# kkahatapitiya/Coarse-Fine-Networks

Hardware: AMD Instinct MI355X
Metric: clips/sec (fwd+bwd+SGD) x3d_fine X3D-M T=256x224x224 (higher is better)
Workload: dtype f32; 1 GPU; x3d_fine X3D-M train step (fwd+loss+bwd+SGD), 8x3x256x224x224 clips per GPU, random-init weights; clips_per_gpu=8, frames=256, parallelism=dp1, launch=eager

## Files before the change

coarse-fine-networks_amd/cfn_hip/ops.py:

```python
import torch
from torch.autograd import Function
from torch.autograd.function import once_differentiable

import ctypes
import threading

from . import call, call_try, check, query, ACT_NONE, ACT_RELU, ACT_SWISH, ACT_SIGMOID


_scratch_epoch = [0]


class _ZeroArena(object):
    CHUNK = 1 << 20

    def __init__(self):
        self.buf, self.off, self.epoch = {}, {}, _scratch_epoch[0]

    def take(self, numel, dev):
        if self.epoch != _scratch_epoch[0]:
            self.buf, self.off, self.epoch = {}, {}, _scratch_epoch[0]
        numel_al = (numel + 1) & ~1
        key = (dev.type, dev.index)
        if key not in self.buf or self.off[key] + numel_al > self.buf[key].numel():
            self.buf[key] = torch.zeros(max(self.CHUNK, numel_al), dtype=torch.float64, device=dev)
            self.off[key] = 0
        o = self.off[key]
        self.off[key] = o + numel_al
        return self.buf[key][o:o + numel]


class _GradCast(object):

    def __init__(self):
        self._reset()
        self.last_total = 0

    def _reset(self):
        self.cur, self.live, self.scheduled, self.seen, self.task = {}, [], False, set(), None

    def begin(self):
        tid = torch._C._current_graph_task_id()
        if tid != self.task:
            if self.live:
                self.flush()
            self._reset()
            self.task = tid

    def first_use(self, w):
        if id(w) in self.seen:
            return False
        self.seen.add(id(w))
        return True

    def take(self, numel, shape, dev):
        al = (numel + 3) & ~3
        key = (dev.type, dev.index)
        ch = self.cur.get(key)
        if ch is None or ch['off'] + al > ch['f64'].numel():
            size = max(int(self.last_total * 1.05) + 1024, al, 1 << 16)
            ch = {'f64': torch.zeros(size, dtype=torch.float64, device=dev),
                  'f32': torch.empty(size, dtype=torch.float32, device=dev), 'off': 0, 'done': 0}
            self.cur[key] = ch
            self.live.append(ch)
        o = ch['off']
        ch['off'] = o + al
        if not self.scheduled:
            torch.autograd.Variable._execution_engine.queue_callback(self._end_of_backward)
            self.scheduled = True
        return ch['f64'][o:o + numel], ch['f32'][o:o + numel].view(shape)

    def flush(self):
        for ch in self.live:
            if ch['off'] > ch['done']:
                ch['f32'][ch['done']:ch['off']].copy_(ch['f64'][ch['done']:ch['off']])
                ch['done'] = ch['off']

    def _end_of_backward(self):
        self.flush()
        self.last_total = max(sum(ch['off'] for ch in self.live), 1)
        self._reset()


class _PerThread(threading.local):

    def __init__(self):
        self.arena = _ZeroArena()
        self.gradcast = _GradCast()


_tls = _PerThread()
LAZY_GRAD_CAST = True


def _f64(n, c, dev):
    return _tls.arena.take(n * c, dev).view(n, c)


def _f64pair(n, c, dev):
    t = _tls.arena.take(2 * n * c, dev).view(2, n, c)
    return t, t[0], t[1]


def reset_scratch():
    _scratch_epoch[0] += 1


def flush_grad_casts():
    _tls.gradcast.flush()


def allow_lazy_grad_cast(params, ok=True):
    for p in params:
        p._cfn_lazy_grad_ok = bool(ok)


def _lazy_ok(w):
    if not LAZY_GRAD_CAST or w is None or not w.is_leaf or w.grad is not None or torch.is_grad_enabled():
        return False
    if not getattr(w, '_cfn_lazy_grad_ok', False):
        return False
    if w._backward_hooks:
        return False
    hooks = getattr(w, '_post_accumulate_grad_hooks', None)
    if hooks:
        from .dist import _BucketHook
        if not all(isinstance(h, _BucketHook) for h in hooks.values()):
            return False
    return True


def _lazy_ok_probe(w):
    with torch.no_grad():
        return _lazy_ok(w)


def _grad_owner(w):
    if w is not None and not w.is_leaf and w._is_view():
        base = w._base
        if base is not None and base.is_leaf and base.numel() == w.numel() and w.is_contiguous() and base.is_contiguous():
            return base
    return w


def _gw_buffers(w, rows, cols, dev):
    gc = _tls.gradcast
    owner = _grad_owner(w)
    if _lazy_ok(owner):
        gc.begin()
        if gc.first_use(owner):
            g64, g32 = gc.take(rows * cols, tuple(w.shape), dev)
            return g64.view(rows, cols), (lambda: g32)
        gc.flush()
    g64 = _f64(rows, cols, dev)
    return g64, (lambda: g64.float().view(tuple(w.shape)))


def _opt(t):
    return None if t is None else t.contiguous()


def _coef(t, rows=None, cols=None):
    if t is None:
        return None
    if rows is not None and t.numel() != rows * cols:
        raise RuntimeError('per-sample coefficients of %d x %d channels expected, got a tensor of shape %s' % (rows, cols, tuple(t.shape)))
    return t.to(torch.float64).contiguous()


class ShortcutToken(object):

    def __init__(self):
        self.acc, self.acc_stride, self.main_done = None, 1, False


class TailLink(object):

    def __init__(self):
        self.y_scale = self.res_scale = None
        self.done = False


def _bf(t):
    return t is not None and t.dtype in (torch.bfloat16, torch.float16)


def subsample_hw(x, s):
    N, C, T, H, W = x.shape
    out = torch.empty(N, C, T, (H - 1) // s + 1, (W - 1) // s + 1, dtype=x.dtype, device=x.device)
    call('cfn_subsample_hw' + _sfx(x), x, out, N * C * T, H, W, s)
    return out


class _PwConv(Function):

    @staticmethod
    def forward(ctx, x, A, B, w, act, stride, want_stats, token, role, tail=None, tail_role=None):
        x = check(x).contiguous()
        N, Cin, T, H, W = x.shape
        Cout = w.shape[0]
        Ho, Wo = (H - 1) // stride + 1, (W - 1) // stride + 1
        y = torch.empty(N, Cout, T, Ho, Wo, dtype=x.dtype, device=x.device)
        s = q = None
        if want_stats:
            s, q = _f64(N, Cout, x.device), _f64(N, Cout, x.device)
        w2 = w.reshape(Cout, Cin).contiguous()
        A, B = _coef(A, N, Cin), _coef(B, N, Cin)
        xs = None
        if _bf(x):
            xs = subsample_hw(x, stride) if stride > 1 else x
            call('cfn_pwconv_fwd' + _sfx(x), xs, A, B, act, w2, y, s, q, N, Cin, Cout, T * Ho * Wo)
        else:
            call('cfn_pwconv_fwd', x, A, B, act, w2, y, s, q, N, Cin, Cout, T, H, W, stride)
        ctx.save_for_backward(x, A, B, w2, y, xs if stride > 1 else None)
        ctx.meta = (act, stride, tuple(w.shape))
        ctx.wparam = w
        ctx.token, ctx.role = token, role
        ctx.tail, ctx.tail_role = tail, tail_role
        if not want_stats:
            return y, None, None
        return y, s, q

    @staticmethod
    @once_differentiable
    def backward(ctx, gy, gs, gq):
        x, A, B, w2, y, xs = ctx.saved_tensors
        act, stride, wshape = ctx.meta
        token, role = ctx.token, ctx.role
        N, Cin, T, H, W = x.shape
        Cout = w2.shape[0]
        gy = torch.zeros_like(y) if gy is None else gy.contiguous()
        gs, gq = _opt(gs), _opt(gq)
        gsc = None
        if ctx.tail is not None and ctx.tail.done:
            gsc = ctx.tail.y_scale if ctx.tail_role == 'y' else ctx.tail.res_scale
        if _bf(x):
            return _PwConv._backward_bf16(ctx, gy, gs, gq, gsc)
        gx = gA = gB = gw = None
        g64 = fin = None
        fused = False
        if ctx.needs_input_grad[0] or (A is not None and ctx.needs_input_grad[1]):
            if token is not None and role == 'short' and stride > 1 and not token.main_done:
                Ho, Wo = y.shape[3], y.shape[4]
                da = torch.empty(N, Cin, T, Ho, Wo, dtype=torch.float32, device=x.device)
                if ctx.needs_input_grad[3]:
                    g64, fin = _gw_buffers(ctx.wparam, Cout, Cin, x.device)
                    fused = call_try('cfn_pwconv_short_bwd', gy, y, gs, gq, gsc, w2, x, A, B, act, da, g64, N, Cin, Cout, T, H, W,
                                     stride)
                if not fused:
                    call('cfn_pwconv_bwd_data_acc', gy, y, gs, gq, w2, None, None, None, ACT_NONE, da, None, None, N, Cin, Cout, T,
                         Ho, Wo, 1, None, 1, gsc)
                token.acc, token.acc_stride = da, stride
            else:
                gx = torch.zeros_like(x) if stride != 1 else torch.empty_like(x)
                ab = a64 = b64 = None
                if A is not None:
                    ab, a64, b64 = _f64pair(N, Cin, x.device)
                acc, acc_stride = None, 1
                if token is not None and role == 'main':
                    if token.acc is not None:
                        acc, acc_stride, token.acc = token.acc, token.acc_stride, None
                    else:
                        token.main_done = True
                if stride == 1 and ctx.needs_input_grad[3]:
                    g64, fin = _gw_buffers(ctx.wparam, Cout, Cin, x.device)
                    fused = call_try('cfn_pwconv_bwd_fused', gy, y, gs, gq, w2, x, A, B, act, gx, a64, b64, g64, N, Cin, Cout,
                                     T, H, W, acc, acc_stride, gsc)
                if not fused:
                    call('cfn_pwconv_bwd_data_acc', gy, y, gs, gq, w2, x, A, B, act, gx, a64, b64, N, Cin, Cout, T, H, W, stride,
                         acc, acc_stride, gsc)
                if A is not None:
                    gA, gB = ab[0], ab[1]
        if ctx.needs_input_grad[3]:
            if g64 is None:
                g64, fin = _gw_buffers(ctx.wparam, Cout, Cin, x.device)
            if not fused:
                call('cfn_pwconv_bwd_weight', gy, y, gs, gq, x, A, B, act, g64, N, Cin, Cout, T, H, W, stride, gsc)
            gw = fin()
        return gx, gA, gB, gw, None, None, None, None, None, None, None

    @staticmethod
    def _backward_bf16(ctx, gy, gs, gq, gsc):
        x, A, B, w2, y, xs = ctx.saved_tensors
        act, stride, wshape = ctx.meta
        token, role = ctx.token, ctx.role
        N, Cin, T, H, W = x.shape
        Cout = w2.shape[0]
        Ho, Wo = y.shape[3], y.shape[4]
        xin = xs if stride > 1 else x
        gx = gA = gB = gw = None
        if ctx.needs_input_grad[0] or (A is not None and ctx.needs_input_grad[1]):
            if token is not None and role == 'short' and stride > 1 and not token.main_done:
                da = torch.empty(N, Cin, T, Ho, Wo, dtype=x.dtype, device=x.device)
                call('cfn_pwconv_bwd_data' + _sfx(gy), gy, y, gs, gq, w2, None, None, None, ACT_NONE, da, None, None, N, Cin, Cout, T,
                     Ho, Wo, None, 1, gsc)
                token.acc, token.acc_stride = da, stride
            else:
                ab = a64 = b64 = None
                if A is not None:
                    ab, a64, b64 = _f64pair(N, Cin, x.device)
                acc, acc_stride = None, 1
                if token is not None and role == 'main':
                    if token.acc is not None:
                        acc, acc_stride, token.acc = token.acc, token.acc_stride, None
                    else:
                        token.main_done = True
                gxc = torch.empty_like(xin)
                call('cfn_pwconv_bwd_data' + _sfx(gy), gy, y, gs, gq, w2, xin, A, B, act, gxc, a64, b64, N, Cin, Cout, T, Ho, Wo,
                     acc, acc_stride, gsc)
                if stride > 1:
                    gx = torch.zeros_like(x)
                    gx[:, :, :, ::stride, ::stride] = gxc
                else:
                    gx = gxc
                if A is not None:
                    gA, gB = ab[0], ab[1]
        if ctx.needs_input_grad[3]:
            g64, fin = _gw_buffers(ctx.wparam, Cout, Cin, x.device)
            call('cfn_pwconv_bwd_weight' + _sfx(gy), gy, y, gs, gq, xin, A, B, act, g64, N, Cin, Cout, T * Ho * Wo, gsc)
            gw = fin()
        return gx, gA, gB, gw, None, None, None, None, None, None, None


def pwconv(x, w, A=None, B=None, act=ACT_NONE, stride=1, stats=True, token=None, role=None, tail=None, tail_role=None):
    N, Cin, T, H, W = x.shape
    Ho, Wo = (H - 1) // stride + 1, (W - 1) // stride + 1
    es = x.element_size()
    lim = (1 << 31) if es == 4 else (1 << 30)
    span = max(Cin * H * W, w.shape[0] * H * W, w.shape[0] * Ho * Wo, Cin * Ho * Wo) * es
    needs_grad = torch.is_grad_enabled() and any(t is not None and t.requires_grad for t in (x, w, A, B))
    if span * T < lim or needs_grad or T == 1:
        return _PwConv.apply(x, A, B, w, act, stride, stats, token, role, tail, tail_role)
    step = max((lim - 1) // span, 1)
    odd_plane = es == 2 and (Ho * Wo) % 2 == 1
    if odd_plane:
        if 2 * span >= lim:
            raise RuntimeError('pwconv: two frames of %d x %d x %d bf16 elements exceed the 1 GiB buffer range the frame-range '
                               'chunking has to respect (odd plane: frames travel in pairs)' % (max(Cin, w.shape[0]), H, W))
        step = max(step & ~1, 2)
    y = torch.empty(N, w.shape[0], T, Ho, Wo, dtype=x.dtype, device=x.device)
    s = q = None
    t0 = 0
    while t0 < T:
        t1 = min(t0 + step, T)
        if odd_plane and (t1 - t0) % 2 and t1 - t0 > 1:
            t1 -= 1
        pad = odd_plane and (t1 - t0) % 2 == 1
        xc = x[:, :, t0:t1].contiguous()
        if pad:
            xc = torch.cat([xc, torch.zeros_like(xc)], 2)
        yc, sc, qc = _PwConv.apply(xc, A, B, w, act, stride, False if pad else stats, None, None)
        if pad:
            yc = yc[:, :, :1]
            if stats:
                sc, qc = yc.double().sum((2, 3, 4)), (yc.double() ** 2).sum((2, 3, 4))
        y[:, :, t0:t1] = yc
        if stats:
            s, q = (sc, qc) if s is None else (s + sc, q + qc)
        t0 = t1
    return y, s, q


def _sfx(t):
    return '_bf16' if t.dtype == torch.bfloat16 else ('_f16' if t.dtype == torch.float16 else '')


class _DwConv3d(Function):

    @staticmethod
    def forward(ctx, x, A, B, w, act, stride, want_stats):
        x = check(x).contiguous()
        N, C, T, H, W = x.shape
        Ho, Wo = (H + 2 - 3) // stride + 1, (W + 2 - 3) // stride + 1
        y = torch.empty(N, C, T, Ho, Wo, dtype=x.dtype, device=x.device)
        s = q = None
        if want_stats:
            s, q = _f64(N, C, x.device), _f64(N, C, x.device)
        w2 = w.reshape(C, 27).contiguous()
        A, B = _coef(A, N, C), _coef(B, N, C)
        call('cfn_dwconv3d_fwd' + _sfx(x), x, A, B, act, w2, y, s, q, N, C, T, H, W, stride)
        ctx.save_for_backward(x, A, B, w2, y)
        ctx.meta = (act, stride, tuple(w.shape))
        ctx.wparam = w
        if not want_stats:
            return y, None, None
        return y, s, q

    @staticmethod
    @once_differentiable
    def backward(ctx, gy, gs, gq):
        x, A, B, w2, y = ctx.saved_tensors
        act, stride, wshape = ctx.meta
        N, C, T, H, W = x.shape
        gy = torch.zeros_like(y) if gy is None else gy.contiguous()
        gs, gq = _opt(gs), _opt(gq)
        gx = gA = gB = gw = None
        want_x = ctx.needs_input_grad[0] or (A is not None and ctx.needs_input_grad[1])
        want_w = ctx.needs_input_grad[3]
        ab = a64 = b64 = g64 = fin = None
        if want_x:
            gx = torch.empty_like(x)
            if A is not None:
                ab, a64, b64 = _f64pair(N, C, x.device)
        if want_w:
            g64, fin = _gw_buffers(ctx.wparam, C, 27, x.device)
        sfx = _sfx(x)
        fused = want_x and want_w and stride == 1 and call_try('cfn_dwconv3d_bwd_fused' + sfx, gy, y, gs, gq, w2, x, A, B, act,
                                                             gx, a64, b64, g64, N, C, T, H, W)
        if not fused and want_x and want_w and stride == 2:
            fused = call_try('cfn_dwconv3d_bwd_fused_s2' + sfx, gy, y, gs, gq, w2, x, A, B, act, gx, a64, b64, g64, N, C, T, H, W)
        if not fused:
            if want_x:
                call('cfn_dwconv3d_bwd_data' + sfx, gy, y, gs, gq, w2, x, A, B, act, gx, a64, b64, N, C, T, H, W, stride)
            if want_w:
                call('cfn_dwconv3d_bwd_weight' + sfx, gy, y, gs, gq, x, A, B, act, g64, N, C, T, H, W, stride)
        if want_x and A is not None:
            gA, gB = ab[0], ab[1]
        if want_w:
            gw = fin()
        return gx, gA, gB, gw, None, None, None


def dwconv3d(x, w, A=None, B=None, act=ACT_NONE, stride=1, stats=True):
    return _DwConv3d.apply(x, A, B, w, act, stride, stats)


class _DwConvT5(Function):

    @staticmethod
    def forward(ctx, x, w, want_stats, out_dtype=None):
        x = check(x, torch.float32).contiguous()
        N, C, T, H, W = x.shape
        y = torch.empty_like(x, dtype=out_dtype or x.dtype)
        s = q = None
        if want_stats:
            s, q = _f64(N, C, x.device), _f64(N, C, x.device)
        w2 = w.reshape(C, 5).contiguous()
        call('cfn_dwconv_t5_fwd' + _sfx(y), x, w2, y, s, q, N, C, T, H * W)
        ctx.save_for_backward(x, w2, y)
        ctx.wshape = tuple(w.shape)
        ctx.wparam = w
        if not want_stats:
            return y, None, None
        return y, s, q

    @staticmethod
    @once_differentiable
    def backward(ctx, gy, gs, gq):
        x, w2, y = ctx.saved_tensors
        N, C, T, H, W = x.shape
        gy = torch.zeros_like(y) if gy is None else gy.contiguous()
        gs, gq = _opt(gs), _opt(gq)
        gx = gw = None
        want_x, want_w = ctx.needs_input_grad[0], ctx.needs_input_grad[1]
        if want_x:
            gx = torch.empty_like(x)
        if want_w:
            g64, fin = _gw_buffers(ctx.wparam, C, 5, x.device)
        fused = want_x and want_w and call_try('cfn_dwconv_t5_bwd_fused' + _sfx(y), gy, y, gs, gq, w2, x, gx, g64, N, C, T, H * W)
        if not fused:
            if want_x:
                call('cfn_dwconv_t5_bwd_data' + _sfx(y), gy, y, gs, gq, w2, gx, N, C, T, H * W)
            if want_w:
                call('cfn_dwconv_t5_bwd_weight' + _sfx(y), gy, y, gs, gq, x, g64, N, C, T, H * W)
        if want_w:
            gw = fin()
        return gx, gw, None, None


def dwconv_t5(x, w, stats=True, out_dtype=None):
    return _DwConvT5.apply(x, w, stats, out_dtype)


class _StemConv(Function):

    @staticmethod
    def forward(ctx, x, w):
        x = check(x).contiguous()
        N, Ci, T, H, W = x.shape
        Co = w.shape[0]
        Ho, Wo = (H + 2 - 3) // 2 + 1, (W + 2 - 3) // 2 + 1
        y = torch.empty(N, Co, T, Ho, Wo, dtype=torch.float32, device=x.device)
        w2 = w.reshape(Co, Ci * 9).contiguous()
        call('cfn_stem_conv_fwd', x, w2, y, N, Ci, Co, T, H, W)
        ctx.save_for_backward(x)
        ctx.wshape = tuple(w.shape)
        ctx.wparam = w
        return y

    @staticmethod
    @once_differentiable
    def backward(ctx, gy):
        (x,) = ctx.saved_tensors
        N, Ci, T, H, W = x.shape
        Co = ctx.wshape[0]
        gw = None
        if ctx.needs_input_grad[1]:
            g64, fin = _gw_buffers(ctx.wparam, Co, Ci * 9, x.device)
            call('cfn_stem_conv_bwd_weight', gy.contiguous(), x, g64, N, Ci, Co, T, H, W)
            gw = fin()
        return None, gw


def stem_conv(x, w):
    return _StemConv.apply(x, w)


from .u8clips import clip_lut


def _u8_args(frames, lengths, lut):
    if frames.dtype != torch.uint8 or frames.dim() != 5 or frames.shape[4] != 3:
        raise RuntimeError('uint8 frames of shape (N, T, H, W, 3) expected, got %s %s' % (frames.dtype, tuple(frames.shape)))
    if lut.dtype != torch.float32 or lut.numel() != 3 * 256:
        raise RuntimeError('a (3, 256) fp32 table expected (ops.clip_lut), got %s %s' % (lut.dtype, tuple(lut.shape)))
    if lengths is not None:
        if lengths.numel() != frames.shape[0]:
            raise RuntimeError('one length per clip expected: %d clips, lengths %s' % (frames.shape[0], tuple(lengths.shape)))
        lengths = lengths.to(torch.int32).contiguous()
    return frames.contiguous(), lengths, lut.contiguous()


def clip_u8_to_f32(frames, lut, lengths=None):
    frames, lengths, lut = _u8_args(frames, lengths, lut)
    N, T, H, W, _ = frames.shape
    x = torch.empty(N, 3, T, H, W, dtype=torch.float32, device=frames.device)
    call('cfn_clip_u8_to_f32', frames, lut, lengths, x, N, T, H, W)
    return x


class _StemConvU8(Function):

    @staticmethod
    def forward(ctx, frames, lengths, lut, w):
        frames, lengths, lut = _u8_args(frames, lengths, lut)
        N, T, H, W, Ci = frames.shape
        Co = w.shape[0]
        Ho, Wo = (H + 2 - 3) // 2 + 1, (W + 2 - 3) // 2 + 1
        y = torch.empty(N, Co, T, Ho, Wo, dtype=torch.float32, device=frames.device)
        w2 = w.reshape(Co, Ci * 9).contiguous()
        if not call_try('cfn_stem_conv_u8_fwd', frames, lut, lengths, w2, y, N, Ci, Co, T, H, W):
            call('cfn_stem_conv_fwd', clip_u8_to_f32(frames, lut, lengths), w2, y, N, Ci, Co, T, H, W)
        ctx.save_for_backward(frames, lengths, lut)
        ctx.wshape = tuple(w.shape)
        ctx.wparam = w
        return y

    @staticmethod
    @once_differentiable
    def backward(ctx, gy):
        frames, lengths, lut = ctx.saved_tensors
        N, T, H, W, Ci = frames.shape
        Co = ctx.wshape[0]
        gw = None
        if ctx.needs_input_grad[3]:
            g64, fin = _gw_buffers(ctx.wparam, Co, Ci * 9, frames.device)
            gy = gy.contiguous()
            if not call_try('cfn_stem_conv_u8_bwd_weight', gy, frames, lut, lengths, g64, N, Ci, Co, T, H, W):
                call('cfn_stem_conv_bwd_weight', gy, clip_u8_to_f32(frames, lut, lengths), g64, N, Ci, Co, T, H, W)
            gw = fin()
        return None, None, None, gw


def stem_conv_u8(frames, lengths, lut, w):
    return _StemConvU8.apply(frames, lengths, lut, w)


from . import u8aug

_AUG_TABLES = {}
_AUG_TABLES_MAX = 256


def aug_tables(box, size, device):
    cs = tuple(int(v) for v in box.detach().reshape(-1, 4)[:, 2].cpu().tolist())
    device = torch.device(device)
    key = (cs, int(size), device.type, device.index)
    hit = _AUG_TABLES.get(key)
    if hit is None:
        if any(c <= 0 or c > 4 * int(size) for c in cs):
            raise RuntimeError('crop_resize_flip_u8: crop extents %s into %d: 1 <= c <= 4 * size expected (the kernel takes tables of up '
                               'to %d taps; there is no CPU fallback)' % (sorted(set(cs)), size, u8aug.MAX_TAPS))
        bounds, coef = u8aug.batch_tables(cs, size)
        hit = (bounds.to(device), coef.to(device))
        if len(_AUG_TABLES) >= _AUG_TABLES_MAX:
            _AUG_TABLES.clear()
        _AUG_TABLES[key] = hit
    return hit


def crop_resize_flip_u8(frames, lengths, box, size, out=None, tables=None):
    if frames.dtype != torch.uint8 or frames.dim() != 5 or frames.shape[4] != 3:
        raise RuntimeError('uint8 frames of shape (N, T, Hs, Ws, 3) expected, got %s %s' % (frames.dtype, tuple(frames.shape)))
    N, T, Hs, Ws, _ = frames.shape
    S = int(size)
    if box.numel() != 4 * N:
        raise RuntimeError('one box (x1, y1, c, flip) per clip expected: %d clips, box %s' % (N, tuple(box.shape)))
    if lengths is not None:
        if lengths.numel() != N:
            raise RuntimeError('one length per clip expected: %d clips, lengths %s' % (N, tuple(lengths.shape)))
        lengths = lengths.to(torch.int32).contiguous()
    bounds, coef = tables if tables is not None else aug_tables(box, S, frames.device)
    if tuple(bounds.shape) != (N, S, 2) or coef.dim() != 3 or tuple(coef.shape[:2]) != (N, S):
        raise RuntimeError('tables of %d clips into %d expected, got bounds %s coef %s' % (N, S, tuple(bounds.shape), tuple(coef.shape)))
    box = box.reshape(N, 4).to(device=frames.device, dtype=torch.int32).contiguous()
    if out is None:
        out = torch.empty(N, T, S, S, 3, dtype=torch.uint8, device=frames.device)
    elif out.dtype != torch.uint8 or tuple(out.shape) != (N, T, S, S, 3) or not out.is_contiguous():
        raise RuntimeError('out: a contiguous uint8 tensor of shape %s expected, got %s %s' % ((N, T, S, S, 3), out.dtype, tuple(out.shape)))
    if not call_try('cfn_crop_resize_flip_u8', frames.contiguous(), lengths, box, bounds.contiguous(), coef.contiguous(), out, N, T, Hs, Ws,
                    S, int(coef.shape[2])):
        raise RuntimeError('crop_resize_flip_u8: %d taps into size %d is beyond what the kernel was built for (c <= 4 * size, size <= 312 '
                           'at 9 taps); there is no CPU fallback' % (int(coef.shape[2]), S))
    return out


AP_SORT_TILE = 8192
AP_FLAG_NONBINARY, AP_FLAG_OVERFLOW = 1, 2


def _ap_stores(scores, targets, count, what):
    for name, x in (('scores', scores), ('targets', targets), ('count', count)):
        if not torch.is_tensor(x) or not x.is_cuda:
            raise RuntimeError('%s: %s must be a device tensor; there is no CPU path' % (what, name))
    if scores.dtype != torch.float32 or scores.dim() != 2 or targets.dtype != torch.uint8 or tuple(targets.shape) != tuple(scores.shape):
        raise RuntimeError('%s: class-major stores expected, scores (K, cap) fp32 and targets (K, cap) uint8; got %s %s, %s %s'
                           % (what, scores.dtype, tuple(scores.shape), targets.dtype, tuple(targets.shape)))
    if count.dtype != torch.int32 or count.numel() != 1:
        raise RuntimeError('%s: count must be one int32 on the device, got %s %s' % (what, count.dtype, tuple(count.shape)))
    if scores.shape[0] < 1 or scores.shape[1] < 1:
        raise RuntimeError('%s: empty stores %s' % (what, tuple(scores.shape)))
    return int(scores.shape[0]), int(scores.shape[1])


def ap_append(probs, labels, valid, scores, targets, count, flags):
    K, cap = _ap_stores(scores, targets, count, 'ap_append')
    for name, x in (('probs', probs), ('labels', labels), ('flags', flags)):
        if not torch.is_tensor(x) or not x.is_cuda:
            raise RuntimeError('ap_append: %s must be a device tensor; there is no CPU path' % name)
    if probs.dim() != 3 or probs.shape[1] != K or tuple(labels.shape) != tuple(probs.shape):
        raise RuntimeError('ap_append: probs and labels (B, %d, TL) expected, got %s and %s' % (K, tuple(probs.shape), tuple(labels.shape)))
    if flags.dtype != torch.int32 or flags.numel() != 1:
        raise RuntimeError('ap_append: flags must be one int32 on the device')
    B, _, TL = probs.shape
    if valid is not None:
        if valid.numel() != B:
            raise RuntimeError('ap_append: one valid length per video expected: %d videos, valid %s' % (B, tuple(valid.shape)))
        valid = valid.to(torch.int32).contiguous()
    call('cfn_ap_append', probs.float().contiguous(), labels.float().contiguous(), valid, scores, targets, count, flags, B, K, TL, cap)


def ap_sort(scores, targets, count, out=None):
    K, cap = _ap_stores(scores, targets, count, 'ap_sort')
    if out is None:
        out = (torch.empty_like(scores), torch.empty_like(targets), torch.empty(K, cap, dtype=torch.int32, device=scores.device),
               torch.empty_like(targets))
    ss, st, tk, tt = out
    for x, ref, dt in ((ss, scores, torch.float32), (st, targets, torch.uint8), (tk, scores, torch.int32), (tt, targets, torch.uint8)):
        if tuple(x.shape) != tuple(ref.shape) or x.dtype != dt or x.device != ref.device:
            raise RuntimeError('ap_sort: out buffers of shape %s (fp32, uint8, int32, uint8) on %s expected' % (tuple(ref.shape), ref.device))
    call('cfn_ap_sort', scores, targets, count, ss, st, tk, tt, K, cap)
    return ss, st


def ap_reduce(sorted_targets, count):
    if not sorted_targets.is_cuda or not count.is_cuda:
        raise RuntimeError('ap_reduce: device tensors only; there is no CPU path')
    if sorted_targets.dtype != torch.uint8 or sorted_targets.dim() != 2 or count.dtype != torch.int32 or count.numel() != 1:
        raise RuntimeError('ap_reduce: sorted targets (K, cap) uint8 and one int32 count expected')
    K, cap = sorted_targets.shape
    ap = torch.empty(K, dtype=torch.float32, device=sorted_targets.device)
    call('cfn_ap_reduce', sorted_targets, count, ap, K, cap)
    return ap


def average_precision(scores, targets, count, out=None):
    _, st = ap_sort(scores, targets, count, out=out)
    return ap_reduce(st, count)


class _BnFold(Function):

    @staticmethod
    def forward(ctx, s, q, gamma, beta, w1, b1, w2, b2, bufs, cfg):
        training, N, C, S, count, eps, momentum, pool_count = cfg
        run_mean, run_var, nbt = bufs
        dev = run_mean.device
        Wd = w1.shape[0] if w1 is not None else 0
        Se = S if training else 1
        A = torch.empty(N, C, dtype=torch.float64, device=dev)
        B = torch.empty_like(A)
        mean = torch.empty(Se, C, dtype=torch.float64, device=dev)
        rstd = torch.empty_like(mean)
        A0 = B0 = gate = hbuf = pooled = None
        w1c = w2c = None
        if Wd:
            A0, B0, gate, pooled = (torch.empty(N, C, dtype=torch.float32, device=dev) for _ in range(4))
            hbuf = torch.empty(N, Wd, dtype=torch.float32, device=dev)
            w1c, w2c = w1.reshape(Wd, C).contiguous(), w2.reshape(C, Wd).contiguous()
        s, q = _opt(s), _opt(q)
        call('cfn_bn_fold_fwd', s, q, gamma, beta, run_mean, run_var, nbt if training else None, int(training), N, C, S,
             float(count), float(eps), float(momentum), w1c, b1, w2c, b2, Wd, float(pool_count), A, B, mean, rstd,
             A0, B0, gate, hbuf, pooled)
        ctx.save_for_backward(s, gamma, mean, rstd, A0, B0, gate, hbuf, pooled, w1c, w2c)
        ctx.cfg = (training, N, C, S, Wd, count, pool_count, None if w1 is None else tuple(w1.shape),
                   None if w2 is None else tuple(w2.shape))
        return A, B

    @staticmethod
    @once_differentiable
    def backward(ctx, gA, gB):
        s, gamma, mean, rstd, A0, B0, gate, hbuf, pooled, w1c, w2c = ctx.saved_tensors
        training, N, C, S, Wd, count, pool_count, w1s, w2s = ctx.cfg
        dev = mean.device
        gA = torch.zeros(N, C, dtype=torch.float64, device=dev) if gA is None else gA.contiguous()
        gB = torch.zeros(N, C, dtype=torch.float64, device=dev) if gB is None else gB.contiguous()
        gs = gq = None
        if training:
            gs = torch.empty(N, C, dtype=torch.float64, device=dev)
            gq = torch.empty_like(gs)
        elif Wd:
            gs = torch.empty(N, C, dtype=torch.float64, device=dev)
        gg = gbt = None
        if gamma is not None:
            gg, gbt = torch.empty(C, device=dev), torch.empty(C, device=dev)
        gw1 = gb1 = gw2 = gb2 = tA = tB = None
        if Wd:
            gw1, gb1 = torch.empty(Wd, C, device=dev), torch.empty(Wd, device=dev)
            gw2, gb2 = torch.empty(C, Wd, device=dev), torch.empty(C, device=dev)
            tA, tB = (torch.empty(N, C, dtype=torch.float64, device=dev) for _ in range(2))
        call('cfn_bn_fold_bwd', gA, gB, s, gamma, mean, rstd, A0, B0, gate, hbuf, pooled, w1c, w2c, int(training), N, C, S,
             Wd, float(count), float(pool_count), gs, gq, gg, gbt, gw1, gb1, gw2, gb2, tA, tB)
        if Wd:
            gw1, gw2 = gw1.view(w1s), gw2.view(w2s)
        return gs, gq, gg, gbt, gw1, gb1, gw2, gb2, None, None


def bn_fold(s, q, gamma, beta, bufs, training, N, C, S, count, eps, momentum, se=None, pool_count=1.0):
    w1, b1, w2, b2 = se if se is not None else (None, None, None, None)
    return _BnFold.apply(s, q, gamma, beta, w1, b1, w2, b2, bufs, (training, N, C, S, count, eps, momentum, pool_count))


class _BnAddRelu(Function):

    @staticmethod
    def forward(ctx, y, A, B, res, Ar, Br, split, link):
        y, res = check(y).contiguous(), check(res).contiguous()
        N, C = y.shape[:2]
        vol = y[0, 0].numel()
        if tuple(res.shape) != tuple(y.shape):
            raise RuntimeError('bn_add_relu: residual %s does not match y %s' % (tuple(res.shape), tuple(y.shape)))
        out = torch.empty_like(y)
        A, B, Ar, Br = _coef(A, N, C), _coef(B, N, C), _coef(Ar, N, C), _coef(Br, N, C)
        mask = None
        sfx = _sfx(y)
        if link is not None:
            words = query('cfn_bn_add_relu_mask_words' + sfx, N * C, vol)
            if words > 0:
                mask = torch.empty(words, dtype=torch.int32, device=y.device)
        call('cfn_bn_add_relu_fwd' + sfx, y, A, B, res, Ar, Br, out, mask, N * C, vol)
        ctx.link, ctx.has_mask = link, mask is not None
        ctx.save_for_backward(y, A, res, Ar, mask if mask is not None else out)
        if not split:
            return out
        alias = torch.empty(0, dtype=out.dtype, device=out.device).set_(out.untyped_storage(), out.storage_offset(),
                                                                         out.shape, out.stride())
        return out, alias

    @staticmethod
    @once_differentiable
    def backward(ctx, gout, gout2=None):
        y, A, res, Ar, out = ctx.saved_tensors
        N, C = y.shape[:2]
        vol = y[0, 0].numel()
        if gout is None:
            gout, gout2 = gout2, None
        if gout is None:
            gout = torch.zeros_like(y)
        gout2 = None if gout2 is None else gout2.contiguous()
        t3 = _tls.arena.take(3 * N * C, y.device).view(3, N, C)
        gA, gB = t3[0], t3[1]
        gAr = t3[2] if Ar is not None else None
        gBr = gB if Ar is not None else None
        link = ctx.link
        if link is not None:
            g = torch.empty_like(y)
            mask = out if ctx.has_mask else None
            call('cfn_bn_add_relu_bwd_g' + _sfx(y), gout.contiguous(), gout2, None if ctx.has_mask else out, mask, y,
                 res if Ar is not None else None, g, gA, gB, gAr, N * C, vol)
            link.y_scale, link.res_scale, link.done = A.detach(), (None if Ar is None else Ar.detach()), True
            g2 = torch.empty(0, dtype=g.dtype, device=g.device).set_(g.untyped_storage(), g.storage_offset(), g.shape, g.stride())
            return g, gA, gB, g2, gAr, gBr, None, None
        if _bf(y):
            g = torch.empty_like(y)
            call('cfn_bn_add_relu_bwd_g' + _sfx(y), gout.contiguous(), gout2, out, None, y, res if Ar is not None else None, g, gA, gB,
                 gAr, N * C, vol)
            shp = (N, C) + (1,) * (y.dim() - 2)
            gres = g if Ar is None else (g.float() * Ar.float().view(shp)).to(y.dtype)
            return (g.float() * A.float().view(shp)).to(y.dtype), gA, gB, gres, gAr, gBr, None, None
        gy, gres = torch.empty_like(y), torch.empty_like(res)
        call('cfn_bn_add_relu_bwd', gout.contiguous(), gout2, out, y, A, res, Ar, gy, gres, gA, gB, gAr, N * C, vol)
        return gy, gA, gB, gres, gAr, gBr, None, None


def bn_add_relu(y, A, B, res, Ar=None, Br=None, split=False, link=None):
    return _BnAddRelu.apply(y, A, B, res, Ar, Br, split, link)


class _AffineAct(Function):
    @staticmethod
    def forward(ctx, x, A, B, act):
        x = check(x).contiguous()
        N, C = x.shape[:2]
        out = torch.empty_like(x)
        A, B = _coef(A, N, C), _coef(B, N, C)
        call('cfn_affine_act_fwd', x, A, B, act, out, N * C, x[0, 0].numel())
        ctx.save_for_backward(x, A, B)
        ctx.act = act
        return out

    @staticmethod
    @once_differentiable
    def backward(ctx, gout):
        x, A, B = ctx.saved_tensors
        N, C = x.shape[:2]
        gx = torch.empty_like(x)
        a64, b64 = _f64(N, C, x.device), _f64(N, C, x.device)
        call('cfn_affine_act_bwd', gout.contiguous(), x, A, B, ctx.act, gx, a64, b64, N * C, x[0, 0].numel())
        return gx, a64, b64, None


def affine_act(x, A, B, act=ACT_NONE):
    return _AffineAct.apply(x, A, B, act)


class _ChannelStats(Function):

    @staticmethod
    def forward(ctx, x):
        x = check(x).contiguous()
        N, C = x.shape[:2]
        s, q = _f64(N, C, x.device), _f64(N, C, x.device)
        call('cfn_channel_stats', x, s, q, N * C, x[0, 0].numel())
        ctx.save_for_backward(x)
        return s, q

    @staticmethod
    @once_differentiable
    def backward(ctx, gs, gq):
        (x,) = ctx.saved_tensors
        N, C = x.shape[:2]
        gx = torch.zeros_like(x)
        shp = (N, C) + (1,) * (x.dim() - 2)
        if gs is not None:
            gx = gx + gs.float().view(shp)
        if gq is not None:
            gx = gx + 2.0 * gq.float().view(shp) * x
        return gx


def channel_stats(x):
    return _ChannelStats.apply(x)


class _PoolHW(Function):

    @staticmethod
    def forward(ctx, x, A, B, act, OH, OW):
        x = check(x).contiguous()
        N, C, T, H, W = x.shape
        out = torch.empty(N, C, T, OH, OW, dtype=torch.float32, device=x.device)
        A, B = _coef(A, N, C), _coef(B, N, C)
        call('cfn_pool_hw_fwd' + _sfx(x), x, A, B, act, out, N * C, T, H, W, OH, OW)
        ctx.save_for_backward(x, A, B)
        ctx.meta = (act, OH, OW)
        return out

    @staticmethod
    @once_differentiable
    def backward(ctx, gout):
        x, A, B = ctx.saved_tensors
        act, OH, OW = ctx.meta
        N, C, T, H, W = x.shape
        gx = torch.empty_like(x)
        a64 = b64 = None
        if A is not None:
            a64, b64 = _f64(N, C, x.device), _f64(N, C, x.device)
        call('cfn_pool_hw_bwd' + _sfx(x), gout.contiguous(), x, A, B, act, gx, a64, b64, N * C, T, H, W, OH, OW)
        if A is None:
            return gx, None, None, None, None, None
        return gx, a64, b64, None, None, None


def pool_hw(x, OH, OW, A=None, B=None, act=ACT_NONE):
    return _PoolHW.apply(x, A, B, act, OH, OW)


class _Film(Function):

    @staticmethod
    def forward(ctx, x, m, c, f):
        x, m, c = check(x).contiguous(), check(m).contiguous(), check(c).contiguous()
        N, C, T, H, W = x.shape
        want = (N, C, T, H // f if f > 0 else -1, W // f if f > 0 else -1)
        if f <= 0 or H % f or W % f or tuple(m.shape) != want or tuple(c.shape) != want:
            raise RuntimeError('film: coefficients %s / %s do not tile x %s with %d x %d blocks (expected %s)'
                               % (tuple(m.shape), tuple(c.shape), tuple(x.shape), f, f, want))
        out = torch.empty_like(x)
        call('cfn_film_fwd', x, m, c, out, N * C, T, H, W, f)
        ctx.save_for_backward(x, m)
        ctx.f = f
        return out

    @staticmethod
    @once_differentiable
    def backward(ctx, g):
        x, m = ctx.saved_tensors
        N, C, T, H, W = x.shape
        gx, gm, gc = torch.empty_like(x), torch.empty_like(m), torch.empty_like(m)
        call('cfn_film_bwd', g.contiguous(), x, m, gx, gm, gc, N * C, T, H, W, ctx.f)
        return gx, gm, gc, None


def film(x, m, c, f):
    return _Film.apply(x, m, c, f)


class _TimeSample(Function):

    @staticmethod
    def forward(ctx, x, cdf):
        x, cdf = check(x).contiguous(), check(cdf).contiguous()
        B, C, Tin = x.shape[:3]
        K = cdf.shape[1]
        P = x[0, 0, 0].numel()
        out = torch.empty((B, C, K) + tuple(x.shape[3:]), dtype=torch.float32, device=x.device)
        call('cfn_time_sample_fwd', x, cdf, out, B, C, Tin, K, P)
        ctx.save_for_backward(x, cdf)
        return out

    @staticmethod
    @once_differentiable
    def backward(ctx, g):
        x, cdf = ctx.saved_tensors
        B, C, Tin = x.shape[:3]
        K = cdf.shape[1]
        P = x[0, 0, 0].numel()
        gx = torch.empty_like(x) if ctx.needs_input_grad[0] else None
        g64 = torch.zeros(B, K, dtype=torch.float64, device=x.device) if ctx.needs_input_grad[1] else None
        call('cfn_time_sample_bwd', g.contiguous(), x, cdf, gx, g64, B, C, Tin, K, P)
        return gx, (g64.float() if g64 is not None else None)


def time_sample(x, cdf):
    return _TimeSample.apply(x, cdf)


class _TimePool(Function):

    @staticmethod
    def forward(ctx, x, mode, R):
        x = check(x, torch.float32).contiguous()
        B, C, T = x.shape[:3]
        P = x[0, 0, 0].numel()
        out = torch.empty((B, C, T // R) + tuple(x.shape[3:]), dtype=torch.float32, device=x.device)
        call('cfn_time_pool_fwd', x, out, mode, B * C, T, R, P)
        ctx.save_for_backward(x)
        ctx.meta = (mode, R)
        return out

    @staticmethod
    @once_differentiable
    def backward(ctx, g):
        (x,) = ctx.saved_tensors
        mode, R = ctx.meta
        B, C, T = x.shape[:3]
        gx = torch.empty_like(x)
        call('cfn_time_pool_bwd', g.contiguous(), x, gx, mode, B * C, T, R, x[0, 0, 0].numel())
        return gx, None, None


def time_pool(x, mode, R=4):
    return _TimePool.apply(x, {'avg': 0, 'max': 1}[mode], R)


def grid_time_index(cdf, Tin):
    cdf = check(cdf).contiguous()
    i0 = torch.empty(cdf.shape, dtype=torch.int32, device=cdf.device)
    w1 = torch.empty(cdf.shape, dtype=torch.float32, device=cdf.device)
    call('cfn_grid_time_index', cdf, cdf.numel(), Tin, i0, w1)
    return i0, w1


class _Interp1d(Function):
    @staticmethod
    def forward(ctx, x, y, xnew):
        x, y, xnew = check(x).contiguous(), check(y).contiguous(), check(xnew).contiguous()
        B = max(x.shape[0], y.shape[0], xnew.shape[0])
        N, Pq = x.shape[1], xnew.shape[1]
        rows = (int(x.shape[0] > 1), int(y.shape[0] > 1), int(xnew.shape[0] > 1))
        ynew = torch.empty(B, Pq, dtype=torch.float32, device=x.device)
        ind = torch.empty(B, Pq, dtype=torch.int64, device=x.device)
        call('cfn_interp1d_fwd', x, y, xnew, ynew, ind, B, N, Pq, *rows)
        ctx.save_for_backward(x, y, xnew, ind)
        ctx.rows = rows
        ctx.mark_non_differentiable(ind)
        return ynew, ind

    @staticmethod
    @once_differentiable
    def backward(ctx, g, _gind):
        x, y, xnew, ind = ctx.saved_tensors
        B, Pq = ind.shape
        N = x.shape[1]
        gx = torch.zeros_like(x) if ctx.needs_input_grad[0] else None
        gy = torch.zeros_like(y) if ctx.needs_input_grad[1] else None
        gq = torch.zeros_like(xnew) if ctx.needs_input_grad[2] else None
        call('cfn_interp1d_bwd', g.contiguous(), x, y, xnew, ind, gx, gy, gq, B, N, Pq, *ctx.rows)
        return gx, gy, gq


def interp1d(x, y, xnew):
    return _Interp1d.apply(x, y, xnew)


class _TimeResize(Function):

    @staticmethod
    def forward(ctx, x, L, align_corners):
        x = check(x).contiguous()
        BC = x.shape[0] * x.shape[1]
        Kin = x.shape[2]
        P = x[0, 0, 0].numel()
        out = torch.empty(tuple(x.shape[:2]) + (L,) + tuple(x.shape[3:]), dtype=torch.float32, device=x.device)
        call('cfn_time_resize_fwd', x, out, BC, Kin, L, P, int(bool(align_corners)))
        ctx.meta = (tuple(x.shape), L, int(bool(align_corners)))
        return out

    @staticmethod
    @once_differentiable
    def backward(ctx, g):
        shape, L, ac = ctx.meta
        gx = torch.empty(shape, dtype=torch.float32, device=g.device)
        P = 1
        for d in shape[3:]:
            P *= d
        call('cfn_time_resize_bwd', g.contiguous(), gx, shape[0] * shape[1], shape[2], L, P, ac)
        return gx, None, None


def time_resize(x, L, align_corners=True):
    return _TimeResize.apply(x, L, align_corners)


def _detloss_args(logits, labels, masks, crops):
    for name, v in (('logits', logits), ('labels', labels), ('masks', masks)):
        if not v.is_cuda or v.dtype != torch.float32:
            raise RuntimeError('detection_loss: %s must be a device fp32 tensor, got %s on %s (there is no CPU path)' % (name, v.dtype, v.device))
        if v.device != logits.device:
            raise RuntimeError('detection_loss: %s lives on %s, the logits on %s' % (name, v.device, logits.device))
    crops = int(crops)
    if logits.dim() != 3 or labels.dim() != 3 or masks.dim() != 2 or crops < 1:
        raise RuntimeError('detection_loss: logits (B*crops, C, T), labels (B, C, TL), masks (B, TL), crops >= 1')
    B, C, TL = labels.shape
    if logits.shape[0] != B * crops or logits.shape[1] != C or tuple(masks.shape) != (B, TL) or 0 in logits.shape or 0 in labels.shape:
        raise RuntimeError('detection_loss: logits %s, labels %s, masks %s do not belong together at %d crop(s)'
                           % (tuple(logits.shape), tuple(labels.shape), tuple(masks.shape), crops))
    return logits.contiguous(), labels.contiguous(), masks.contiguous(), B, C, logits.shape[2], TL


def detection_loss_fwd(logits, labels, masks, align_corners=True, crops=1, norm=None, world=1.0, want_probs=True):
    logits, labels, masks, B, C, T, TL = _detloss_args(logits, labels, masks, crops)
    dev = logits.device
    if norm is not None:
        if not norm.is_cuda or norm.device != dev or norm.numel() != 1:
            raise RuntimeError('detection_loss: norm must be a one-element tensor on the device of the logits')
        norm = norm.detach().to(torch.float32).reshape(1)
    cls = torch.empty((), dtype=torch.float32, device=dev)
    loc = torch.empty((), dtype=torch.float32, device=dev)
    probs = torch.empty(B, C, TL, dtype=torch.float32, device=dev) if want_probs else None
    jstar = torch.empty(B * C, dtype=torch.int32, device=dev)
    ymax = torch.empty(B * C, dtype=torch.float32, device=dev)
    rows = torch.empty(2 * B * C, dtype=torch.float64, device=dev)
    norm_used = torch.empty(1, dtype=torch.float64, device=dev)
    call('cfn_detloss_fwd', logits, labels, masks, norm, float(world), probs, cls, loc, jstar, ymax, rows, norm_used, B, C, T, TL, int(crops),
         int(bool(align_corners)))
    return cls, loc, probs, jstar, ymax, norm_used


def detection_loss_bwd(g_cls, g_loc, logits, labels, masks, jstar, ymax, norm_used, align_corners=True, crops=1, world=1.0):
    logits, labels, masks, B, C, T, TL = _detloss_args(logits, labels, masks, crops)
    if jstar.numel() != B * C or ymax.numel() != B * C or norm_used.numel() != 1:
        raise RuntimeError('detection_loss_bwd: jstar / ymax / norm_used are not the ones the forward returned for these shapes')
    g_cls, g_loc = (g.detach().to(torch.float32).reshape(1) for g in (g_cls, g_loc))
    gx = torch.empty_like(logits)
    call('cfn_detloss_bwd', g_cls, g_loc, logits, labels, masks, jstar.contiguous(), ymax.contiguous(), norm_used, float(world), gx, B, C, T, TL,
         int(crops), int(bool(align_corners)))
    return gx


class _DetectionLoss(Function):

    @staticmethod
    def forward(ctx, logits, labels, masks, align_corners, crops, norm, world, want_probs):
        cls, loc, probs, jstar, ymax, norm_used = detection_loss_fwd(logits, labels, masks, align_corners, crops, norm, world, want_probs)
        ctx.save_for_backward(logits, labels, masks, jstar, ymax, norm_used)
        ctx.meta = (bool(align_corners), int(crops), float(world))
        if probs is not None:
            ctx.mark_non_differentiable(probs)
        return cls, loc, probs

    @staticmethod
    @once_differentiable
    def backward(ctx, g_cls, g_loc, _g_probs):
        gx = detection_loss_bwd(g_cls, g_loc, *ctx.saved_tensors, *ctx.meta) if ctx.needs_input_grad[0] else None
        return gx, None, None, None, None, None, None, None


def detection_loss(logits, labels, masks, align_corners, crops=1, norm=None, world=1.0, want_probs=True):
    return _DetectionLoss.apply(logits, labels, masks, align_corners, crops, norm, world, want_probs)


def _geom(kernel, stride, padding):
    return (ctypes.c_int * 9)(*(tuple(kernel) + tuple(stride) + tuple(padding)))


class _ConvDense(Function):

    @staticmethod
    def forward(ctx, x, A, B, w, act, kernel, stride, padding, want_stats):
        x = check(x).contiguous()
        N, Ci, T, H, W = x.shape
        Co = w.shape[0]
        g = _geom(kernel, stride, padding)
        To = (T + 2 * padding[0] - kernel[0]) // stride[0] + 1
        Ho = (H + 2 * padding[1] - kernel[1]) // stride[1] + 1
        Wo = (W + 2 * padding[2] - kernel[2]) // stride[2] + 1
        y = torch.empty(N, Co, To, Ho, Wo, dtype=torch.float32, device=x.device)
        s = q = None
        if want_stats:
            s, q = _f64(N, Co, x.device), _f64(N, Co, x.device)
        w2 = w.reshape(Co, -1).contiguous()
        A, B = _coef(A, N, Ci), _coef(B, N, Ci)
        call('cfn_conv3d_dense_fwd', x, A, B, act, w2, y, s, q, N, Ci, Co, T, H, W, g)
        ctx.save_for_backward(x, A, B, w2, y)
        ctx.meta = (act, tuple(kernel), tuple(stride), tuple(padding), tuple(w.shape))
        ctx.wparam = w
        if not want_stats:
            return y, None, None
        return y, s, q

    @staticmethod
    @once_differentiable
    def backward(ctx, gy, gs, gq):
        x, A, B, w2, y = ctx.saved_tensors
        act, kernel, stride, padding, wshape = ctx.meta
        N, Ci, T, H, W = x.shape
        Co = w2.shape[0]
        g = _geom(kernel, stride, padding)
        gy = torch.zeros_like(y) if gy is None else gy.contiguous()
        gs, gq = _opt(gs), _opt(gq)
        gx = gA = gB = gw = None
        if ctx.needs_input_grad[0] or (A is not None and ctx.needs_input_grad[1]):
            gx = torch.empty_like(x)
            ab = a64 = b64 = None
            if A is not None:
                ab, a64, b64 = _f64pair(N, Ci, x.device)
            call('cfn_conv3d_dense_bwd_data', gy, y, gs, gq, w2, x, A, B, act, gx, a64, b64, N, Ci, Co, T, H, W, g)
            if A is not None:
                gA, gB = ab[0], ab[1]
        if ctx.needs_input_grad[3]:
            g64, fin = _gw_buffers(ctx.wparam, Co, w2.shape[1], x.device)
            call('cfn_conv3d_dense_bwd_weight', gy, y, gs, gq, x, A, B, act, g64, N, Ci, Co, T, H, W, g)
            gw = fin()
        return gx, gA, gB, gw, None, None, None, None, None


def conv3d_dense(x, w, kernel, stride, padding, A=None, B=None, act=ACT_NONE, stats=True):
    return _ConvDense.apply(x, A, B, w, act, kernel, stride, padding, stats)


class _FusionGather(Function):

    @staticmethod
    def forward(ctx, x, at_raw, at_bias, GX, mask, crops):
        x, at_raw, GX, mask = check(x).contiguous(), check(at_raw).contiguous(), check(GX).contiguous(), check(mask).contiguous()
        B, C, Tf, P = x.shape
        K = GX.shape[2]
        if GX.shape[0] != B * crops or GX.shape[1] != Tf or tuple(mask.shape) != (B, Tf) or tuple(at_raw.shape) != (B, Tf, P):
            raise RuntimeError('fusion_gather: inconsistent shapes x %s at %s GX %s mask %s crops %d'
                               % (tuple(x.shape), tuple(at_raw.shape), tuple(GX.shape), tuple(mask.shape), crops))
        z = torch.empty(B * crops, C, K, P, dtype=torch.float32, device=x.device)
        den = torch.empty(B * crops, K, P, dtype=torch.float32, device=x.device)
        call('cfn_fusion_gather_fwd', x, at_raw, at_bias, GX, mask, z, den, B, crops, C, Tf, K, P)
        ctx.save_for_backward(x, at_raw, at_bias, GX, mask, z, den)
        ctx.crops = crops
        return z

    @staticmethod
    @once_differentiable
    def backward(ctx, gz):
        x, at_raw, at_bias, GX, mask, z, den = ctx.saved_tensors
        B, C, Tf, P = x.shape
        K, crops = GX.shape[2], ctx.crops
        need = ctx.needs_input_grad
        gx = torch.empty_like(x) if need[0] else None
        want_at = need[1] or (at_bias is not None and need[2])
        gat = torch.empty_like(at_raw) if want_at else None
        gGX = torch.empty_like(GX) if need[3] else None
        dw = torch.empty(B * crops, Tf, K, P, dtype=torch.float32, device=x.device)
        call('cfn_fusion_gather_bwd', gz.contiguous(), z, den, x, at_raw, at_bias, GX, mask, gx, gat, gGX, dw, B, crops, C, Tf, K, P)
        gb = gat.sum().view(at_bias.shape) if (at_bias is not None and need[2]) else None
        return gx, (gat if need[1] else None), gb, gGX, None, None


def fusion_gather(x, at_raw, at_bias, GX, mask, crops=1):
    return _FusionGather.apply(x, at_raw, at_bias, GX, mask, crops)


class _GaussAlign(Function):

    @staticmethod
    def forward(ctx, meta, mask, gx, tx, ratio, crops, K):
        meta, mask = meta.contiguous(), check(mask).contiguous()
        if meta.dtype != torch.int64:
            meta = meta.to(torch.int64)
        B, Tf = mask.shape
        if gx is not None:
            gx = check(gx).contiguous()
        GX = torch.empty(B * crops, Tf, K, dtype=torch.float32, device=mask.device)
        call('cfn_gauss_align_fwd', meta, mask, gx, float(tx), float(ratio), GX, B, crops, Tf, K)
        ctx.save_for_backward(meta, mask, gx)
        ctx.cfg = (float(tx), float(ratio), crops, K)
        return GX

    @staticmethod
    @once_differentiable
    def backward(ctx, gGX):
        meta, mask, gx = ctx.saved_tensors
        tx, ratio, crops, K = ctx.cfg
        ggx = None
        if gx is not None and ctx.needs_input_grad[2]:
            B, Tf = mask.shape
            ggx = torch.empty_like(gx)
            call('cfn_gauss_align_bwd', gGX.contiguous(), meta, mask, gx, tx, ratio, ggx, B, crops, Tf, K)
        return None, None, ggx, None, None, None, None


def gauss_align(meta, mask, gx, tx, ratio, crops, K):
    return _GaussAlign.apply(meta, mask, gx, 1.0 if tx is None else tx, ratio, crops, K)


class _GridCdf(Function):

    @staticmethod
    def forward(ctx, g, bias):
        g = check(g).contiguous()
        B, Kin = g.shape
        cdf = torch.empty(B, Kin + 1, dtype=torch.float32, device=g.device)
        call('cfn_grid_cdf_fwd', g, bias, cdf, B, Kin)
        ctx.save_for_backward(g, bias)
        return cdf

    @staticmethod
    @once_differentiable
    def backward(ctx, gcdf):
        g, bias = ctx.saved_tensors
        B, Kin = g.shape
        gg = torch.empty_like(g)
        call('cfn_grid_cdf_bwd', gcdf.contiguous(), g, bias, gg, B, Kin)
        gb = gg.sum().view(bias.shape) if (bias is not None and ctx.needs_input_grad[1]) else None
        return gg, gb


def grid_cdf(g, bias=None):
    return _GridCdf.apply(g, bias)


FEAT_POSITIONS = 49


def _feat_channels(channels, what):
    channels = tuple(int(c) for c in channels)
    if len(channels) != 5 or any(c <= 0 or c % 8 for c in channels):
        raise RuntimeError('%s: five channel counts that are positive multiples of 8 expected, got %s' % (what, channels))
    return channels


def _feat_sfx(dtype, what):
    if dtype not in (torch.float16, torch.bfloat16):
        raise RuntimeError('%s: fp16 or bf16 data expected, got %s' % (what, dtype))
    return '_f16' if dtype == torch.float16 else '_bf16'


def feat_unpack(data, offsets, lengths, channels, t_max, out=None):
    channels = _feat_channels(channels, 'feat_unpack')
    sfx = _feat_sfx(data.dtype, 'feat_unpack')
    t_max = int(t_max)
    if data.dim() != 1 or not data.is_contiguous():
        raise RuntimeError('feat_unpack: a flat contiguous buffer expected, got %s' % (tuple(data.shape),))
    if offsets.dtype != torch.int64 or offsets.dim() != 2 or offsets.shape[1] != 5 or offsets.shape[0] < 1:
        raise RuntimeError('feat_unpack: offsets (B, 5) int64 expected, got %s %s' % (offsets.dtype, tuple(offsets.shape)))
    B = int(offsets.shape[0])
    if lengths.dtype != torch.int32 or lengths.numel() != B:
        raise RuntimeError('feat_unpack: lengths (%d,) int32 expected, got %s %s' % (B, lengths.dtype, tuple(lengths.shape)))
    if t_max < 1:
        raise RuntimeError('feat_unpack: t_max >= 1 expected, got %d' % t_max)
    if out is None:
        out = [torch.empty(B, c, t_max, 7, 7, dtype=torch.float32, device=data.device) for c in channels]
    else:
        out = list(out)
        if len(out) != 5:
            raise RuntimeError('feat_unpack: out: five maps expected, got %d' % len(out))
        for y, c in zip(out, channels):
            if y.dtype != torch.float32 or tuple(y.shape) != (B, c, t_max, 7, 7) or not y.is_contiguous():
                raise RuntimeError('feat_unpack: out: five contiguous fp32 maps (%d, C_k, %d, 7, 7) with C_k = %s expected, got %s %s'
                                   % (B, t_max, channels, y.dtype, tuple(y.shape)))
    call('cfn_feat_unpack' + sfx, data, offsets.contiguous(), lengths.contiguous(), *out, B, t_max, *channels, int(data.numel()))
    return out


def feat_pack(feat, dtype, out=None):
    sfx = _feat_sfx(dtype, 'feat_pack')
    xs = []
    for x in feat:
        if x.dim() == 5 and x.shape[0] == 1:
            x = x[0]
        if x.dtype != torch.float32 or x.dim() != 4 or x.shape[2] * x.shape[3] != FEAT_POSITIONS:
            raise RuntimeError('feat_pack: fp32 maps (C, T, 7, 7) expected, got %s %s' % (x.dtype, tuple(x.shape)))
        xs.append(x.contiguous())
    if len(xs) != 5 or any(x.shape[1] != xs[0].shape[1] for x in xs):
        raise RuntimeError('feat_pack: five maps of one frame count expected, got %s' % [tuple(x.shape) for x in xs])
    channels = _feat_channels([x.shape[0] for x in xs], 'feat_pack')
    T = int(xs[0].shape[1])
    n = T * sum(channels) * FEAT_POSITIONS
    if out is None:
        out = torch.empty(n, dtype=dtype, device=xs[0].device)
    elif out.dtype != dtype or out.dim() != 1 or out.numel() != n or not out.is_contiguous():
        raise RuntimeError('feat_pack: out: a flat %s tensor of %d elements expected, got %s %s' % (dtype, n, out.dtype, tuple(out.shape)))
    call('cfn_feat_pack' + sfx, *xs, out, T, *channels)
    return out


def jpeg_workspace_bytes(rows, slots, lanes, blocks_max):
    n = int(query('cfn_jpeg_workspace_bytes', int(rows), int(slots), int(lanes), int(blocks_max)))
    if n < 0:
        raise RuntimeError('jpeg_decode_u8: bad sizes (%d frames, %d slots, %d lanes, %d blocks)' % (rows, slots, lanes, blocks_max))
    return n


def jpeg_decode_u8(jpeg_clips, out=None, status=None, workspace=None):
    jc = jpeg_clips
    if not (hasattr(jc, '_fields') and jc._fields[:6] == ('data', 'frames', 'tables', 'geom', 'lengths', 'box')):
        raise RuntimeError('jpeg_decode_u8: a JpegClips batch expected, got %s' % type(jc).__name__)
    data, frames, tables = jc.data, jc.frames, jc.tables
    geom, lengths = jc.geom.reshape(-1, 4), jc.lengths.reshape(-1)
    T, H, W, lanes, blocks_max = (int(d) for d in jc.dims)
    if data.dtype != torch.uint8 or data.dim() != 1 or data.numel() < 1:
        raise RuntimeError('jpeg_decode_u8: data: a flat uint8 buffer expected, got %s %s' % (data.dtype, tuple(data.shape)))
    if frames.dim() != 2 or frames.shape[1] != 8 or frames.shape[0] < 1:
        raise RuntimeError('jpeg_decode_u8: frames (R, 8) int32 expected, got %s %s' % (frames.dtype, tuple(frames.shape)))
    if tables.dim() != 2 or tables.shape[1] != 3456 or tables.shape[0] < 1:
        raise RuntimeError('jpeg_decode_u8: tables (S, 3456) int32 expected, got %s %s' % (tables.dtype, tuple(tables.shape)))
    N, R = int(lengths.numel()), int(frames.shape[0])
    if geom.shape[0] != N:
        raise RuntimeError('jpeg_decode_u8: one geometry per clip expected: %d clips, geom %s' % (N, tuple(jc.geom.shape)))
    dev = data.device
    if out is None:
        out = torch.empty(N, T, H, W, 3, dtype=torch.uint8, device=dev)
    elif out.dtype != torch.uint8 or out.numel() != N * T * H * W * 3 or tuple(out.shape[-4:]) != (T, H, W, 3) or not out.is_contiguous():
        raise RuntimeError('jpeg_decode_u8: out: a contiguous uint8 tensor (..., %d, %d, %d, 3) of %d clips expected, got %s %s'
                           % (T, H, W, N, out.dtype, tuple(out.shape)))
    if status is None:
        status = torch.empty(R, dtype=torch.int32, device=dev)
    elif status.dtype != torch.int32 or status.numel() != R or not status.is_contiguous():
        raise RuntimeError('jpeg_decode_u8: status: %d contiguous int32 words expected, got %s %s' % (R, status.dtype, tuple(status.shape)))
    need = jpeg_workspace_bytes(R, N * T, lanes, blocks_max)
    if workspace is None:
        workspace = torch.empty(need, dtype=torch.uint8, device=dev)
    elif workspace.dtype != torch.uint8 or workspace.numel() < need or not workspace.is_contiguous():
        raise RuntimeError('jpeg_decode_u8: workspace: a contiguous uint8 buffer of at least %d bytes expected, got %s %s'
                           % (need, workspace.dtype, tuple(workspace.shape)))
    call('cfn_jpeg_decode_u8', data.contiguous(), frames.contiguous(), tables.contiguous(), geom.contiguous(), lengths.contiguous(), out, status,
         workspace, int(workspace.numel()), int(data.numel()), R, int(tables.shape[0]), N, T, H, W, lanes, blocks_max)
    return out.view(N, T, H, W, 3)
```

coarse-fine-networks_amd/csrc/bnfold.hip:

```cpp
#include "cfn_common.h"
#include <stdlib.h>

struct BnFoldArgs {
    const double* s; const double* q;
    const float* gamma; const float* beta;
    float* run_mean; float* run_var;
    long* nbt;
    int training, N, C, S, Wd;
    int stage;
    double count, pool_count, eps, momentum;
    const float* w1; const float* b1; const float* w2; const float* b2;
    double* A; double* B;
    double* mean; double* rstd;
    float* A0; float* B0; float* gate; float* hbuf; float* pooled;
};

#define BNF_NB 8

__device__ __forceinline__ void bnf_stage_se(const float* w1, const float* w2, float* w1s, float* w2s, int C, int Wd) {
    for (int e = threadIdx.x; e < C * Wd; e += blockDim.x) {
        w1s[e] = w1[e];
        const int c = e / Wd, j = e - c * Wd;
        w2s[c * (Wd + 1) + j] = w2[e];
    }
}

__global__ __launch_bounds__(1024) void bn_fold_fwd_kernel(const BnFoldArgs a) {
    const int tid = threadIdx.x, nthr = blockDim.x, N = a.N, C = a.C, S = a.training ? a.S : 1, G = N / S, Wd = a.Wd;
    extern __shared__ float sh[];
    const bool st = Wd > 0 && a.stage;
    float* sp = sh + (st ? Wd * C + C * (Wd + 1) : 0);
    float* shh = sp + BNF_NB * C;
    const float* w1s = st ? sh : a.w1;
    const float* w2s = st ? sh + Wd * C : a.w2;
    const int w2p = st ? Wd + 1 : Wd;
    if (st) bnf_stage_se(a.w1, a.w2, sh, sh + Wd * C, C, Wd);
    const bool ps = Wd > 0 && gridDim.x > 1;
    const int gown = ps ? (int)(blockIdx.x % S) : 0;
    const int gtid = Wd > 0 ? tid : (int)(blockIdx.x * blockDim.x) + tid, gn = Wd > 0 ? nthr : (int)(gridDim.x * blockDim.x);
    for (int e = ps ? gown * C + tid : gtid; e < (ps ? (gown + 1) * C : S * C); e += gn) {
        const bool wr = !ps || (int)blockIdx.x == gown;
        const int g = e / C, c = e - g * C;
        double mean, var;
        if (a.training) {
            double ss = 0.0, qq = 0.0;
            for (int i = 0; i < G; ++i) { ss += a.s[(long)(i * S + g) * C + c]; qq += a.q[(long)(i * S + g) * C + c]; }
            const double cnt = a.count * G;
            mean = ss / cnt;
            var = qq / cnt - mean * mean;
            if (var < 0.0) var = 0.0;
            const double unb = var * (cnt / (cnt > 1.0 ? cnt - 1.0 : 1.0));
            if (wr) {
                a.run_mean[e] = (float)((1.0 - a.momentum) * (double)a.run_mean[e] + a.momentum * mean);
                a.run_var[e] = (float)((1.0 - a.momentum) * (double)a.run_var[e] + a.momentum * unb);
            }
        } else {
            mean = (double)a.run_mean[c];
            var = (double)a.run_var[c];
        }
        const double rstd = 1.0 / sqrt(var + a.eps);
        if (wr) { a.mean[e] = mean; a.rstd[e] = rstd; }
        const double ga = a.gamma ? (double)a.gamma[c] : 1.0, be = a.beta ? (double)a.beta[c] : 0.0;
        const float av = (float)(ga * rstd), bv = (float)(be - mean * ga * rstd);
        for (int i = 0; i < G; ++i) {
            if (ps && i * S + g != (int)blockIdx.x) continue;
            const long o = (long)(i * S + g) * C + c;
            if (Wd > 0) { a.A0[o] = av; a.B0[o] = bv; } else { a.A[o] = av; a.B[o] = bv; }
        }
    }
    if (a.training && a.nbt && gtid == 0 && (!ps || blockIdx.x == 0)) a.nbt[0] += 1;
    if (Wd <= 0) return;
    __syncthreads();
    const int wave = tid >> 6, lane = tid & 63, nwaves = nthr >> 6;
    for (int n0 = ps ? (int)blockIdx.x : 0; n0 < (ps ? (int)blockIdx.x + 1 : N); n0 += BNF_NB) {
        const int nb = ps ? 1 : min(BNF_NB, N - n0);
        for (int e = tid; e < nb * C; e += nthr) {
            const long o = (long)n0 * C + e;
            const float pv = (float)(a.s[o] / a.pool_count) * a.A0[o] + a.B0[o];
            sp[e] = pv;
            a.pooled[o] = pv;
        }
        __syncthreads();
        for (int p = wave; p < nb * Wd; p += nwaves) {
            const int nl = p / Wd, j = p - nl * Wd;
            float acc = 0.0f;
            for (int c = lane; c < C; c += 64) acc = fmaf(w1s[j * C + c], sp[nl * C + c], acc);
            acc = cfn_wave_sum(acc);
            if (lane == 0) {
                acc = fmaxf(acc + a.b1[j], 0.0f);
                shh[p] = acc;
                a.hbuf[(long)(n0 + nl) * Wd + j] = acc;
            }
        }
        __syncthreads();
        for (int e = tid; e < nb * C; e += nthr) {
            const int nl = e / C, c = e - nl * C;
            float acc = a.b2[c];
            for (int j = 0; j < Wd; ++j) acc = fmaf(w2s[c * w2p + j], shh[nl * Wd + j], acc);
            const float gt = 1.0f / (1.0f + expf(-acc));
            const long o = (long)n0 * C + e;
            a.gate[o] = gt;
            a.A[o] = a.A0[o] * gt;
            a.B[o] = a.B0[o] * gt;
        }
        __syncthreads();
    }
}

struct BnFoldBwdArgs {
    const double* gA; const double* gB;
    const double* s;
    const float* gamma;
    const double* mean; const double* rstd;
    const float* A0; const float* B0; const float* gate; const float* hbuf; const float* pooled;
    const float* w1; const float* w2;
    int training, N, C, S, Wd;
    int stage;
    double count, pool_count;
    double* gs; double* gq;
    float* ggamma; float* gbeta;
    float* gw1; float* gb1; float* gw2; float* gb2;
    double* tA; double* tB;
};

__global__ __launch_bounds__(1024) void bn_fold_bwd_kernel(const BnFoldBwdArgs a) {
    const int tid = threadIdx.x, nthr = blockDim.x, N = a.N, C = a.C, S = a.training ? a.S : 1, G = N / S, Wd = a.Wd;
    extern __shared__ float sh[];
    if (Wd > 0) {
        const bool st = a.stage != 0;
        const float* w1s = st ? sh : a.w1;
        const float* w2s = st ? sh + Wd * C : a.w2;
        const int w2p = st ? Wd + 1 : Wd;
        float* gz2 = sh + (st ? Wd * C + C * (Wd + 1) : 0);
        float* pl = gz2 + BNF_NB * C;
        float* gz1 = pl + BNF_NB * C;
        float* shh = gz1 + BNF_NB * Wd;
        if (st) bnf_stage_se(a.w1, a.w2, sh, sh + Wd * C, C, Wd);
        const int wave = tid >> 6, lane = tid & 63, nwaves = nthr >> 6;
        for (int n0 = 0; n0 < N; n0 += BNF_NB) {
            const int nb = min(BNF_NB, N - n0);
            const bool first = n0 == 0;
            for (int e = tid; e < nb * Wd; e += nthr) shh[e] = a.hbuf[(long)n0 * Wd + e];
            for (int e = tid; e < nb * C; e += nthr) {
                const long o = (long)n0 * C + e;
                const float gt = a.gate[o];
                const float ggate = a.gA[o] * a.A0[o] + a.gB[o] * a.B0[o];
                gz2[e] = ggate * gt * (1.0f - gt);
                pl[e] = a.pooled[o];
                a.tA[o] = a.gA[o] * gt;
                a.tB[o] = a.gB[o] * gt;
            }
            __syncthreads();
            for (int e = tid; e < C * Wd; e += nthr) {
                const int c = e / Wd, j = e - c * Wd;
                float acc = 0.0f;
                for (int nl = 0; nl < nb; ++nl) acc = fmaf(gz2[nl * C + c], shh[nl * Wd + j], acc);
                a.gw2[e] = first ? acc : a.gw2[e] + acc;
            }
            for (int c = tid; c < C; c += nthr) {
                float acc = 0.0f;
                for (int nl = 0; nl < nb; ++nl) acc += gz2[nl * C + c];
                a.gb2[c] = first ? acc : a.gb2[c] + acc;
            }
            for (int p = wave; p < nb * Wd; p += nwaves) {
                const int nl = p / Wd, j = p - nl * Wd;
                float acc = 0.0f;
                for (int c = lane; c < C; c += 64) acc = fmaf(gz2[nl * C + c], w2s[c * w2p + j], acc);
                acc = cfn_wave_sum(acc);
                if (lane == 0) gz1[p] = shh[p] > 0.0f ? acc : 0.0f;
            }
            __syncthreads();
            for (int e = tid; e < Wd * C; e += nthr) {
                const int j = e / C, c = e - j * C;
                float acc = 0.0f;
                for (int nl = 0; nl < nb; ++nl) acc = fmaf(gz1[nl * Wd + j], pl[nl * C + c], acc);
                a.gw1[e] = first ? acc : a.gw1[e] + acc;
            }
            for (int j = tid; j < Wd; j += nthr) {
                float acc = 0.0f;
                for (int nl = 0; nl < nb; ++nl) acc += gz1[nl * Wd + j];
                a.gb1[j] = first ? acc : a.gb1[j] + acc;
            }
            for (int e = tid; e < nb * C; e += nthr) {
                const int nl = e / C, c = e - nl * C;
                float gp = 0.0f;
                for (int j = 0; j < Wd; ++j) gp = fmaf(gz1[nl * Wd + j], w1s[j * C + c], gp);
                const long o = (long)n0 * C + e;
                const float sm = (float)(a.s[o] / a.pool_count);
                a.tA[o] += gp * sm;
                a.tB[o] += gp;
                if (a.gs) a.gs[o] = (double)(gp * a.A0[o]) / a.pool_count;
            }
            __syncthreads();
        }
    }
    const double* dA = Wd > 0 ? a.tA : a.gA;
    const double* dB = Wd > 0 ? a.tB : a.gB;
    const int gtid = Wd > 0 ? tid : (int)(blockIdx.x * blockDim.x) + tid, gn = Wd > 0 ? nthr : (int)(gridDim.x * blockDim.x);
    for (int c = gtid; c < C; c += gn) {
        double ggam = 0.0, gbet = 0.0;
        for (int g = 0; g < S; ++g) {
            double ga = 0.0, gb = 0.0;
            for (int i = 0; i < G; ++i) { ga += dA[(long)(i * S + g) * C + c]; gb += dB[(long)(i * S + g) * C + c]; }
            const double mean = a.mean[g * C + c], rstd = a.rstd[g * C + c];
            const double gam = a.gamma ? (double)a.gamma[c] : 1.0;
            ggam += (ga - gb * mean) * rstd;
            gbet += gb;
            if (a.training && a.gs) {
                const double cnt = a.count * G;
                const double g_rstd = (ga - gb * mean) * gam;
                const double g_var = g_rstd * (-0.5 * rstd * rstd * rstd);
                const double g_mean = -gb * gam * rstd - 2.0 * mean * g_var;
                for (int i = 0; i < G; ++i) {
                    const long o = (long)(i * S + g) * C + c;
                    a.gs[o] = (Wd > 0 ? a.gs[o] : 0.0) + g_mean / cnt;
                    a.gq[o] = g_var / cnt;
                }
            }
        }
        if (a.ggamma) { a.ggamma[c] = (float)ggam; a.gbeta[c] = (float)gbet; }
    }
}

extern "C" int cfn_bn_fold_fwd(const double* s, const double* q, const float* gamma, const float* beta, float* run_mean,
                               float* run_var, long* nbt, int training, int N, int C, int S, double count, double eps,
                               double momentum, const float* w1, const float* b1, const float* w2, const float* b2, int Wd,
                               double pool_count, double* A, double* B, double* mean, double* rstd, float* A0, float* B0,
                               float* gate, float* hbuf, float* pooled, void* stream) {
    CFN_REQUIRE(A && B && mean && rstd && run_mean && run_var, "cfn_bn_fold_fwd: null tensor");
    CFN_REQUIRE(!training || (s && q), "cfn_bn_fold_fwd: training needs sum / sumsq");
    CFN_REQUIRE(N > 0 && C > 0 && S > 0, "cfn_bn_fold_fwd: bad sizes");
    CFN_REQUIRE(!training || N % S == 0, "cfn_bn_fold_fwd: batch %d not divisible by %d splits", N, S);
    CFN_REQUIRE(Wd <= 0 || (w1 && b1 && w2 && b2 && s && A0 && B0 && gate && hbuf && pooled), "cfn_bn_fold_fwd: SE needs its tensors");
    const size_t lds_small = Wd > 0 ? BNF_NB * (size_t)(C + Wd) * sizeof(float) : 0;
    const size_t lds_full = Wd > 0 ? lds_small + ((size_t)Wd * C + (size_t)C * (Wd + 1)) * sizeof(float) : 0;
    const int stage = lds_full <= 150 * 1024;
    const size_t lds = stage ? lds_full : lds_small;
    BnFoldArgs a = {s, q, gamma, beta, run_mean, run_var, nbt, training, N, C, S, Wd, stage, count, pool_count, eps, momentum,
                    w1, b1, w2, b2, A, B, mean, rstd, A0, B0, gate, hbuf, pooled};
    CFN_REQUIRE(lds <= 150 * 1024, "cfn_bn_fold_fwd: per-sample SE tables (C=%d, width=%d) exceed LDS", C, Wd);
    if (lds > 48 * 1024) (void)hipFuncSetAttribute((const void*)bn_fold_fwd_kernel, hipFuncAttributeMaxDynamicSharedMemorySize, (int)lds);
    const int Se = training ? S : 1;
    static const int per_sample = getenv("CFN_BNFOLD_PS") ? atoi(getenv("CFN_BNFOLD_PS")) : 1;
    hipLaunchKernelGGL(bn_fold_fwd_kernel, dim3(Wd > 0 ? (per_sample ? N : 1) : cfn_cdiv((long)Se * C, 64)), dim3(Wd > 0 ? 1024 : 64), lds, (hipStream_t)stream, a);
    return cfn_check_launch("bn_fold_fwd");
}

extern "C" int cfn_bn_fold_bwd(const double* gA, const double* gB, const double* s, const float* gamma, const double* mean,
                               const double* rstd, const float* A0, const float* B0, const float* gate, const float* hbuf,
                               const float* pooled, const float* w1, const float* w2, int training, int N, int C, int S,
                               int Wd, double count, double pool_count, double* gs, double* gq, float* ggamma, float* gbeta,
                               float* gw1, float* gb1, float* gw2, float* gb2, double* tA, double* tB, void* stream) {
    CFN_REQUIRE(gA && gB && mean && rstd, "cfn_bn_fold_bwd: null tensor");
    CFN_REQUIRE(Wd <= 0 || (s && A0 && B0 && gate && hbuf && pooled && w1 && w2 && gw1 && gb1 && gw2 && gb2 && tA && tB),
                "cfn_bn_fold_bwd: SE needs its tensors");
    CFN_REQUIRE(!training || ((gs == nullptr) == (gq == nullptr)), "cfn_bn_fold_bwd: gs/gq mismatch");
    const size_t lds_small = Wd > 0 ? 2 * BNF_NB * (size_t)(C + Wd) * sizeof(float) : 0;
    const size_t lds_full = Wd > 0 ? lds_small + ((size_t)Wd * C + (size_t)C * (Wd + 1)) * sizeof(float) : 0;
    const int stage = lds_full <= 150 * 1024;
    const size_t lds = stage ? lds_full : lds_small;
    BnFoldBwdArgs a = {gA, gB, s, gamma, mean, rstd, A0, B0, gate, hbuf, pooled, w1, w2, training, N, C, S, Wd, stage, count,
                       pool_count, gs, gq, ggamma, gbeta, gw1, gb1, gw2, gb2, tA, tB};
    CFN_REQUIRE(lds <= 150 * 1024, "cfn_bn_fold_bwd: per-sample SE tables (C=%d, width=%d) exceed LDS", C, Wd);
    if (lds > 48 * 1024) (void)hipFuncSetAttribute((const void*)bn_fold_bwd_kernel, hipFuncAttributeMaxDynamicSharedMemorySize, (int)lds);
    hipLaunchKernelGGL(bn_fold_bwd_kernel, dim3(Wd > 0 ? 1 : cfn_cdiv(C, 64)), dim3(Wd > 0 ? 1024 : 64), lds, (hipStream_t)stream, a);
    return cfn_check_launch("bn_fold_bwd");
}
```

coarse-fine-networks_amd/csrc/cfn_common.h:

```cpp
#pragma once
#include <hip/hip_runtime.h>
#include <stdint.h>
#include <stdio.h>
#include <stdarg.h>

#define CFN_OK 0
#define CFN_ERR_ARG 1
#define CFN_ERR_LAUNCH 2
#define CFN_ERR_UNSUPPORTED 3

enum { CFN_ACT_NONE = 0, CFN_ACT_RELU = 1, CFN_ACT_SWISH = 2, CFN_ACT_SIGMOID = 3 };

extern "C" const char* cfn_last_error(void);
int cfn_fail(int code, const char* fmt, ...);
int cfn_check_launch(const char* what);

#define CFN_REQUIRE(cond, ...) \
    do { if (!(cond)) return cfn_fail(CFN_ERR_ARG, __VA_ARGS__); } while (0)

enum { CFN_K_DWCONV_FWD = 0, CFN_K_DWCONV_BWD = 1, CFN_K_PWCONV_FWD = 2, CFN_K_PWCONV_BWD = 3,
       CFN_K_GRIDPOOL = 4, CFN_K_ELEMWISE = 5, CFN_K_STEM = 6, CFN_K_FUSION = 7, CFN_K_PWCONV_WGRAD = 8,
       CFN_K_DWCONV_WGRAD = 9, CFN_K_DENSE_FWD = 10, CFN_K_GRIDPOOL_BWD = 11, CFN_K_COUNT = 12 };
struct CfnProfScope {
    int fam; hipStream_t s; hipEvent_t e0; bool on;
    CfnProfScope(int family, hipStream_t stream, double bytes);
    ~CfnProfScope();
};

struct CfnDetState { unsigned long long* keys; unsigned long long* vals; unsigned long long* count; unsigned long long cap; };
static __constant__ CfnDetState cfn_det_dev;
int cfn_det_register(void (*set)(const CfnDetState*));
static void cfn_det_tu_set(const CfnDetState* st) {
    if (hipMemcpyToSymbol(HIP_SYMBOL(cfn_det_dev), st, sizeof(*st)) != hipSuccess) (void)hipGetLastError();
}
static const int cfn_det_tu_registered = cfn_det_register(&cfn_det_tu_set);
__device__ __forceinline__ unsigned long long* cfn_det_keys() { return cfn_det_dev.keys; }
__device__ __forceinline__ void cfn_add64(double* p, double v, unsigned long long* keys);
__device__ __forceinline__ void cfn_add64(double* p, double v) { cfn_add64(p, v, cfn_det_dev.keys); }
__device__ __forceinline__ void cfn_add64(double* p, double v, unsigned long long* const keys) {
    if (__builtin_expect(keys != nullptr, 0)) {
        const unsigned long long i = atomicAdd(cfn_det_dev.count, 1ull);
        if (i < cfn_det_dev.cap) { keys[i] = (unsigned long long)(uintptr_t)p; cfn_det_dev.vals[i] = __builtin_bit_cast(unsigned long long, v); }
    } else {
        atomicAdd(p, v);
    }
}

static inline int cfn_cdiv(long a, long b) { return (int)((a + b - 1) / b); }

static inline bool cfn_split_nc(long NC, unsigned& gy, unsigned& gz) {
    gy = (unsigned)NC; gz = 1;
    if (NC <= 65535) return NC > 0;
    for (long d = 65535; d >= 1; --d)
        if (NC % d == 0) { gy = (unsigned)d; gz = (unsigned)(NC / d); return gz <= 65535; }
    return false;
}
static inline bool cfn_split_nc_ok(long NC) { unsigned a, b; return cfn_split_nc(NC, a, b); }

__device__ __forceinline__ int cfn_uni(int v) { return __builtin_amdgcn_readfirstlane(v); }
__device__ __forceinline__ unsigned cfn_uni(unsigned v) { return (unsigned)__builtin_amdgcn_readfirstlane((int)v); }
__device__ __forceinline__ long cfn_uni(long v) {
    const unsigned lo = cfn_uni((unsigned)v), hi = cfn_uni((unsigned)((unsigned long)v >> 32));
    return (long)(((unsigned long)hi << 32) | lo);
}
__device__ __forceinline__ float cfn_uni(float v) { return __builtin_bit_cast(float, __builtin_amdgcn_readfirstlane(__builtin_bit_cast(int, v))); }
template <class T> __device__ __forceinline__ T* cfn_uni(T* p) { return (T*)cfn_uni((long)p); }

template <class T> __device__ __forceinline__ __amdgpu_buffer_rsrc_t cfn_rsrc(T* p, unsigned bytes) {
    return __builtin_amdgcn_make_buffer_rsrc((void*)cfn_uni((long)p), 0, cfn_uni(bytes), 0x00020000);
}

__device__ __forceinline__ void cfn_bst128(unsigned __attribute__((ext_vector_type(4))) data, __amdgpu_buffer_rsrc_t r, int vo, int so) {
    __builtin_amdgcn_raw_buffer_store_b128(data, r, vo, so, 0);
    asm volatile("s_nop 1" : "+v"(data));
}

__device__ __forceinline__ float cfn_sigmoid(float v) { return __builtin_amdgcn_rcpf(1.0f + __expf(-v)); }

template <int ACT>
__device__ __forceinline__ float cfn_act(float z) {
    if (ACT == CFN_ACT_RELU) return fmaxf(z, 0.0f);
    if (ACT == CFN_ACT_SWISH) return z * cfn_sigmoid(z);
    return z;
}
template <int ACT>
__device__ __forceinline__ float cfn_act_grad(float z) {
    if (ACT == CFN_ACT_RELU) return z > 0.0f ? 1.0f : 0.0f;
    if (ACT == CFN_ACT_SWISH) { float s = cfn_sigmoid(z); return s * (1.0f + z * (1.0f - s)); }
    return 1.0f;
}
__device__ __forceinline__ float cfn_act_rt(float z, int act) {
    if (act == CFN_ACT_RELU) return fmaxf(z, 0.0f);
    if (act == CFN_ACT_SWISH) return z * cfn_sigmoid(z);
    if (act == CFN_ACT_SIGMOID) return cfn_sigmoid(z);
    return z;
}
__device__ __forceinline__ float cfn_act_grad_rt(float z, int act) {
    if (act == CFN_ACT_RELU) return z > 0.0f ? 1.0f : 0.0f;
    if (act == CFN_ACT_SWISH) { float s = cfn_sigmoid(z); return s * (1.0f + z * (1.0f - s)); }
    if (act == CFN_ACT_SIGMOID) { float s = cfn_sigmoid(z); return s * (1.0f - s); }
    return 1.0f;
}

__device__ __forceinline__ float cfn_settle(float v) {
    float o;
    asm volatile("v_mov_b32 %0, %1" : "=v"(o) : "v"(v));
    return o;
}
__device__ __forceinline__ float2 cfn_settle(float2 v) { return float2{cfn_settle(v.x), cfn_settle(v.y)}; }
__device__ __forceinline__ float4 cfn_settle3(float4 v) { return float4{cfn_settle(v.x), cfn_settle(v.y), cfn_settle(v.z), 0.0f}; }

__device__ __forceinline__ float cfn_wave_sum(float v) {
#pragma unroll
    for (int o = 32; o > 0; o >>= 1) v += __shfl_xor(v, o, 64);
    return v;
}
__device__ __forceinline__ double cfn_wave_sum_d(double v) {
#pragma unroll
    for (int o = 32; o > 0; o >>= 1) v += __shfl_xor(v, o, 64);
    return v;
}

__device__ __forceinline__ unsigned cfn_xcd_remap(unsigned b, unsigned total) {
    const unsigned q = total >> 3, r = total & 7u;
    const unsigned xcd = b & 7u, i = b >> 3;
#ifdef CFN_XCD_REVERSE
    return total - 1u - (xcd * q + (xcd < r ? xcd : r) + i);
#else
    return xcd * q + (xcd < r ? xcd : r) + i;
#endif
}
```

coarse-fine-networks_amd/csrc/elementwise.hip:

```cpp
#include "cfn_common.h"
#include <stdlib.h>

typedef float __attribute__((ext_vector_type(4))) f4v;

template <int NV>
__device__ __forceinline__ void block_sum(float (&v)[NV], float* sh ) {
#pragma unroll
    for (int i = 0; i < NV; ++i) v[i] = cfn_wave_sum(v[i]);
    const int wave = threadIdx.x >> 6;
    if ((threadIdx.x & 63) == 0)
#pragma unroll
        for (int i = 0; i < NV; ++i) sh[i * 4 + wave] = v[i];
    __syncthreads();
    if (threadIdx.x == 0)
#pragma unroll
        for (int i = 0; i < NV; ++i) v[i] = sh[i * 4] + sh[i * 4 + 1] + sh[i * 4 + 2] + sh[i * 4 + 3];
}

#define EW_ITEMS 8

template <int VEC>
__global__ __launch_bounds__(256) void bn_add_relu_fwd_kernel(const float* __restrict__ y, const double* __restrict__ A,
                                                              const double* __restrict__ B, const float* __restrict__ res,
                                                              const double* __restrict__ Ar, const double* __restrict__ Br,
                                                              float* __restrict__ out, unsigned* __restrict__ mask, long vol) {
    const long nc = blockIdx.y + (long)blockIdx.z * gridDim.y;
    const float a = A[nc], b = B[nc] + (Br ? Br[nc] : 0.0f), ar = Ar ? Ar[nc] : 1.0f;
    const long base = nc * vol;
    long i = ((long)blockIdx.x * 256 * EW_ITEMS + threadIdx.x) * VEC;
    unsigned mw = 0;
#pragma unroll
    for (int k = 0; k < EW_ITEMS; ++k, i += 256 * VEC) {
        if (i >= vol) break;
        if (VEC == 4) {
            const f4v yv = *reinterpret_cast<const f4v*>(y + base + i);
            const f4v rv = *reinterpret_cast<const f4v*>(res + base + i);
            f4v o;
            o.x = fmaxf(fmaf(yv.x, a, fmaf(rv.x, ar, b)), 0.f); o.y = fmaxf(fmaf(yv.y, a, fmaf(rv.y, ar, b)), 0.f);
            o.z = fmaxf(fmaf(yv.z, a, fmaf(rv.z, ar, b)), 0.f); o.w = fmaxf(fmaf(yv.w, a, fmaf(rv.w, ar, b)), 0.f);
            *reinterpret_cast<f4v*>(out + base + i) = o;
            mw |= ((o.x > 0.f ? 1u : 0u) | (o.y > 0.f ? 2u : 0u) | (o.z > 0.f ? 4u : 0u) | (o.w > 0.f ? 8u : 0u)) << (4 * k);
        } else {
            out[base + i] = fmaxf(fmaf(y[base + i], a, fmaf(res[base + i], ar, b)), 0.f);
        }
    }
    if (VEC == 4 && mask) mask[(nc * gridDim.x + blockIdx.x) * 256 + threadIdx.x] = mw;
}

template <int VEC>
__global__ __launch_bounds__(256) void bn_add_relu_bwd_g_kernel(const float* __restrict__ gout, const float* __restrict__ gout2,
                                                                const float* __restrict__ out, const unsigned* __restrict__ mask,
                                                                const float* __restrict__ y, const float* __restrict__ res,
                                                                float* __restrict__ g_out, double* __restrict__ gA,
                                                                double* __restrict__ gB, double* __restrict__ gAr, long vol) {
    __shared__ float sh[12];
    const long nc = blockIdx.y + (long)blockIdx.z * gridDim.y;
    const long base = nc * vol;
    float acc[3] = {0.f, 0.f, 0.f};
    long i = ((long)blockIdx.x * 256 * EW_ITEMS + threadIdx.x) * VEC;
    const unsigned mw = (VEC == 4 && mask) ? mask[(nc * gridDim.x + blockIdx.x) * 256 + threadIdx.x] : 0u;
#pragma unroll
    for (int k = 0; k < EW_ITEMS; ++k, i += 256 * VEC) {
        if (i >= vol) break;
        if (VEC == 4) {
            f4v go = *reinterpret_cast<const f4v*>(gout + base + i);
            if (gout2) go += *reinterpret_cast<const f4v*>(gout2 + base + i);
            const f4v yv = *reinterpret_cast<const f4v*>(y + base + i);
            unsigned m4;
            if (mask) m4 = (mw >> (4 * k)) & 15u;
            else {
                const f4v ov = *reinterpret_cast<const f4v*>(out + base + i);
                m4 = (ov.x > 0.f ? 1u : 0u) | (ov.y > 0.f ? 2u : 0u) | (ov.z > 0.f ? 4u : 0u) | (ov.w > 0.f ? 8u : 0u);
            }
            f4v g;
            g.x = (m4 & 1u) ? go.x : 0.f; g.y = (m4 & 2u) ? go.y : 0.f;
            g.z = (m4 & 4u) ? go.z : 0.f; g.w = (m4 & 8u) ? go.w : 0.f;
            acc[0] += g.x * yv.x + g.y * yv.y + g.z * yv.z + g.w * yv.w;
            acc[1] += g.x + g.y + g.z + g.w;
            if (gAr) {
                const f4v rv = *reinterpret_cast<const f4v*>(res + base + i);
                acc[2] += g.x * rv.x + g.y * rv.y + g.z * rv.z + g.w * rv.w;
            }
            *reinterpret_cast<f4v*>(g_out + base + i) = g;
        } else {
            const float g = out[base + i] > 0.f ? gout[base + i] + (gout2 ? gout2[base + i] : 0.f) : 0.f;
            acc[0] = fmaf(g, y[base + i], acc[0]);
            acc[1] += g;
            if (gAr) acc[2] = fmaf(g, res[base + i], acc[2]);
            g_out[base + i] = g;
        }
    }
    block_sum<3>(acc, sh);
    if (threadIdx.x == 0) {
        cfn_add64(&gA[nc], (double)acc[0]);
        cfn_add64(&gB[nc], (double)acc[1]);
        if (gAr) cfn_add64(&gAr[nc], (double)acc[2]);
    }
}

struct EwFlatArgs {
    const float* y; const double* A; const double* B; const float* res; const double* Ar; const double* Br; float* out; unsigned* mask;
    const float* gout; const float* gout2; const float* outr; const unsigned* maskr; float* g; double* gA; double* gB; double* gAr;
    long vol; unsigned nchunks;
};

__global__ __launch_bounds__(256) void bn_add_relu_fwd_flat_kernel(const EwFlatArgs a) {
    constexpr int OOB = 0x7ffffff0;
    const unsigned L = cfn_xcd_remap(blockIdx.x, gridDim.x);
    const long nc = cfn_uni((int)(L / a.nchunks));
    const unsigned chunk = cfn_uni(L - (unsigned)nc * a.nchunks);
    const float ca = a.A[nc], cb = a.B[nc] + (a.Br ? a.Br[nc] : 0.0f), car = a.Ar ? a.Ar[nc] : 1.0f;
    const unsigned bytes = (unsigned)(a.vol * 4);
    __amdgpu_buffer_rsrc_t ry = cfn_rsrc(a.y + nc * a.vol, bytes), rr = cfn_rsrc(a.res + nc * a.vol, bytes), ro = cfn_rsrc(a.out + nc * a.vol, bytes);
    const long i0 = ((long)chunk * 256 * EW_ITEMS + threadIdx.x) * 4;
    f4v yv[EW_ITEMS], rv[EW_ITEMS];
    int off[EW_ITEMS];
#pragma unroll
    for (int k = 0; k < EW_ITEMS; ++k) {
        const long i = i0 + (long)k * 1024;
        off[k] = i < a.vol ? (int)(i * 4) : OOB;
        yv[k] = __builtin_bit_cast(f4v, __builtin_amdgcn_raw_buffer_load_b128(ry, off[k], 0, 0));
        rv[k] = __builtin_bit_cast(f4v, __builtin_amdgcn_raw_buffer_load_b128(rr, off[k], 0, 0));
    }
    unsigned mw = 0;
#pragma unroll
    for (int k = 0; k < EW_ITEMS; ++k) {
        f4v o;
        o.x = fmaxf(fmaf(yv[k].x, ca, fmaf(rv[k].x, car, cb)), 0.f); o.y = fmaxf(fmaf(yv[k].y, ca, fmaf(rv[k].y, car, cb)), 0.f);
        o.z = fmaxf(fmaf(yv[k].z, ca, fmaf(rv[k].z, car, cb)), 0.f); o.w = fmaxf(fmaf(yv[k].w, ca, fmaf(rv[k].w, car, cb)), 0.f);
        cfn_bst128(__builtin_bit_cast(unsigned __attribute__((ext_vector_type(4))), o), ro, off[k], 0);
        if (off[k] != OOB) mw |= ((o.x > 0.f ? 1u : 0u) | (o.y > 0.f ? 2u : 0u) | (o.z > 0.f ? 4u : 0u) | (o.w > 0.f ? 8u : 0u)) << (4 * k);
    }
    if (a.mask) a.mask[((unsigned long)nc * a.nchunks + chunk) * 256 + threadIdx.x] = mw;
}

__global__ __launch_bounds__(256) void bn_add_relu_bwd_g_flat_kernel(const EwFlatArgs a) {
    constexpr int OOB = 0x7ffffff0;
    __shared__ float sh[12];
    const unsigned L = cfn_xcd_remap(blockIdx.x, gridDim.x);
    const long nc = cfn_uni((int)(L / a.nchunks));
    const unsigned chunk = cfn_uni(L - (unsigned)nc * a.nchunks);
    const unsigned bytes = (unsigned)(a.vol * 4);
    const bool has2 = a.gout2 != nullptr, hasm = a.maskr != nullptr, hasr = a.gAr != nullptr;
    __amdgpu_buffer_rsrc_t rg = cfn_rsrc(a.gout + nc * a.vol, bytes), rg2 = cfn_rsrc((has2 ? a.gout2 : a.gout) + nc * a.vol, has2 ? bytes : 0u);
    __amdgpu_buffer_rsrc_t ry = cfn_rsrc(a.y + nc * a.vol, bytes), ro = cfn_rsrc((hasm ? a.gout : a.outr) + nc * a.vol, bytes);
    __amdgpu_buffer_rsrc_t rr = cfn_rsrc((hasr ? a.res : a.gout) + nc * a.vol, bytes), rd = cfn_rsrc(a.g + nc * a.vol, bytes);
    const long i0 = ((long)chunk * 256 * EW_ITEMS + threadIdx.x) * 4;
    const unsigned mw = hasm ? a.maskr[((unsigned long)nc * a.nchunks + chunk) * 256 + threadIdx.x] : 0u;
    f4v go[EW_ITEMS], g2v[EW_ITEMS], yv[EW_ITEMS];
    int off[EW_ITEMS];
#pragma unroll
    for (int k = 0; k < EW_ITEMS; ++k) {
        const long i = i0 + (long)k * 1024;
        off[k] = i < a.vol ? (int)(i * 4) : OOB;
        go[k] = __builtin_bit_cast(f4v, __builtin_amdgcn_raw_buffer_load_b128(rg, off[k], 0, 0));
        g2v[k] = __builtin_bit_cast(f4v, __builtin_amdgcn_raw_buffer_load_b128(rg2, off[k], 0, 0));
        yv[k] = __builtin_bit_cast(f4v, __builtin_amdgcn_raw_buffer_load_b128(ry, off[k], 0, 0));
    }
    float acc[3] = {0.f, 0.f, 0.f};
#pragma unroll
    for (int k = 0; k < EW_ITEMS; ++k) {
        f4v ov, rv;
        const f4v g2 = g2v[k];
        if (!hasm) ov = __builtin_bit_cast(f4v, __builtin_amdgcn_raw_buffer_load_b128(ro, off[k], 0, 0));
        if (hasr) rv = __builtin_bit_cast(f4v, __builtin_amdgcn_raw_buffer_load_b128(rr, off[k], 0, 0));
        const f4v gs = go[k] + g2;
        unsigned m4;
        if (hasm) m4 = (mw >> (4 * k)) & 15u;
        else m4 = (ov.x > 0.f ? 1u : 0u) | (ov.y > 0.f ? 2u : 0u) | (ov.z > 0.f ? 4u : 0u) | (ov.w > 0.f ? 8u : 0u);
        f4v g;
        g.x = (m4 & 1u) ? gs.x : 0.f; g.y = (m4 & 2u) ? gs.y : 0.f;
        g.z = (m4 & 4u) ? gs.z : 0.f; g.w = (m4 & 8u) ? gs.w : 0.f;
        acc[0] += g.x * yv[k].x + g.y * yv[k].y + g.z * yv[k].z + g.w * yv[k].w;
        acc[1] += g.x + g.y + g.z + g.w;
        if (hasr) acc[2] += g.x * rv.x + g.y * rv.y + g.z * rv.z + g.w * rv.w;
        cfn_bst128(__builtin_bit_cast(unsigned __attribute__((ext_vector_type(4))), g), rd, off[k], 0);
    }
    block_sum<3>(acc, sh);
    if (threadIdx.x == 0) {
        cfn_add64(&a.gA[nc], (double)acc[0]);
        cfn_add64(&a.gB[nc], (double)acc[1]);
        if (hasr) cfn_add64(&a.gAr[nc], (double)acc[2]);
    }
}

template <int VEC>
__global__ __launch_bounds__(256) void bn_add_relu_bwd_kernel(const float* __restrict__ gout, const float* __restrict__ gout2,
                                                              const float* __restrict__ out,
                                                              const float* __restrict__ y, const double* __restrict__ A,
                                                              const float* __restrict__ res, const double* __restrict__ Ar,
                                                              float* __restrict__ gy, float* __restrict__ gres,
                                                              double* __restrict__ gA, double* __restrict__ gB,
                                                              double* __restrict__ gAr, long vol) {
    __shared__ float sh[12];
    const long nc = blockIdx.y + (long)blockIdx.z * gridDim.y;
    const float a = A[nc], ar = Ar ? Ar[nc] : 1.0f;
    const long base = nc * vol;
    float acc[3] = {0.f, 0.f, 0.f};
    long i = ((long)blockIdx.x * 256 * EW_ITEMS + threadIdx.x) * VEC;
#pragma unroll
    for (int k = 0; k < EW_ITEMS; ++k, i += 256 * VEC) {
        if (i >= vol) break;
        if (VEC == 4) {
            f4v go = *reinterpret_cast<const f4v*>(gout + base + i);
            if (gout2) go += *reinterpret_cast<const f4v*>(gout2 + base + i);
            const f4v ov = *reinterpret_cast<const f4v*>(out + base + i);
            const f4v yv = *reinterpret_cast<const f4v*>(y + base + i);
            f4v g;
            g.x = ov.x > 0.f ? go.x : 0.f; g.y = ov.y > 0.f ? go.y : 0.f;
            g.z = ov.z > 0.f ? go.z : 0.f; g.w = ov.w > 0.f ? go.w : 0.f;
            acc[0] += g.x * yv.x + g.y * yv.y + g.z * yv.z + g.w * yv.w;
            acc[1] += g.x + g.y + g.z + g.w;
            if (Ar) {
                const f4v rv = *reinterpret_cast<const f4v*>(res + base + i);
                acc[2] += g.x * rv.x + g.y * rv.y + g.z * rv.z + g.w * rv.w;
            }
            *reinterpret_cast<f4v*>(gy + base + i) = g * a;
            *reinterpret_cast<f4v*>(gres + base + i) = g * ar;
        } else {
            const float g = out[base + i] > 0.f ? gout[base + i] + (gout2 ? gout2[base + i] : 0.f) : 0.f;
            acc[0] = fmaf(g, y[base + i], acc[0]);
            acc[1] += g;
            if (Ar) acc[2] = fmaf(g, res[base + i], acc[2]);
            gy[base + i] = g * a;
            gres[base + i] = g * ar;
        }
    }
    block_sum<3>(acc, sh);
    if (threadIdx.x == 0) {
        cfn_add64(&gA[nc], (double)acc[0]);
        cfn_add64(&gB[nc], (double)acc[1]);
        if (gAr) cfn_add64(&gAr[nc], (double)acc[2]);
    }
}

template <int VEC>
__global__ __launch_bounds__(256) void affine_act_fwd_kernel(const float* __restrict__ x, const double* __restrict__ A,
                                                             const double* __restrict__ B, int act, float* __restrict__ out,
                                                             long vol) {
    const long nc = blockIdx.y + (long)blockIdx.z * gridDim.y;
    const float a = A[nc], b = B[nc];
    const long base = nc * vol;
    long i = ((long)blockIdx.x * 256 * EW_ITEMS + threadIdx.x) * VEC;
#pragma unroll
    for (int k = 0; k < EW_ITEMS; ++k, i += 256 * VEC) {
        if (i >= vol) break;
        if (VEC == 4) {
            const f4v v = *reinterpret_cast<const f4v*>(x + base + i);
            f4v o;
            o.x = cfn_act_rt(fmaf(v.x, a, b), act); o.y = cfn_act_rt(fmaf(v.y, a, b), act);
            o.z = cfn_act_rt(fmaf(v.z, a, b), act); o.w = cfn_act_rt(fmaf(v.w, a, b), act);
            *reinterpret_cast<f4v*>(out + base + i) = o;
        } else {
            out[base + i] = cfn_act_rt(fmaf(x[base + i], a, b), act);
        }
    }
}

template <int VEC>
__global__ __launch_bounds__(256) void affine_act_bwd_kernel(const float* __restrict__ gout, const float* __restrict__ x,
                                                             const double* __restrict__ A, const double* __restrict__ B, int act,
                                                             float* __restrict__ gx, double* __restrict__ gA,
                                                             double* __restrict__ gB, long vol) {
    __shared__ float sh[8];
    const long nc = blockIdx.y + (long)blockIdx.z * gridDim.y;
    const float a = A[nc], b = B[nc];
    const long base = nc * vol;
    float acc[2] = {0.f, 0.f};
    long i = ((long)blockIdx.x * 256 * EW_ITEMS + threadIdx.x) * VEC;
#pragma unroll
    for (int k = 0; k < EW_ITEMS; ++k, i += 256 * VEC) {
        if (i >= vol) break;
#pragma unroll
        for (int u = 0; u < VEC; ++u) {
            const float xv = x[base + i + u];
            const float dz = gout[base + i + u] * cfn_act_grad_rt(fmaf(xv, a, b), act);
            acc[0] = fmaf(dz, xv, acc[0]);
            acc[1] += dz;
            gx[base + i + u] = dz * a;
        }
    }
    block_sum<2>(acc, sh);
    if (threadIdx.x == 0) { cfn_add64(&gA[nc], (double)acc[0]); cfn_add64(&gB[nc], (double)acc[1]); }
}

template <int VEC>
__global__ __launch_bounds__(256) void channel_stats_kernel(const float* __restrict__ x, double* __restrict__ sum,
                                                            double* __restrict__ sumsq, long vol) {
    __shared__ float sh[8];
    const long nc = blockIdx.y + (long)blockIdx.z * gridDim.y;
    const long base = nc * vol;
    float acc[2] = {0.f, 0.f};
    long i = ((long)blockIdx.x * 256 * EW_ITEMS + threadIdx.x) * VEC;
#pragma unroll
    for (int k = 0; k < EW_ITEMS; ++k, i += 256 * VEC) {
        if (i >= vol) break;
        if (VEC == 4) {
            const f4v v = *reinterpret_cast<const f4v*>(x + base + i);
            acc[0] += v.x + v.y + v.z + v.w;
            acc[1] += v.x * v.x + v.y * v.y + v.z * v.z + v.w * v.w;
        } else {
            const float v = x[base + i];
            acc[0] += v;
            acc[1] = fmaf(v, v, acc[1]);
        }
    }
    block_sum<2>(acc, sh);
    if (threadIdx.x == 0) { cfn_add64(&sum[nc], (double)acc[0]); cfn_add64(&sumsq[nc], (double)acc[1]); }
}

__device__ __forceinline__ int ap_start(int o, int O, int S) { return (o * S) / O; }
__device__ __forceinline__ int ap_end(int o, int O, int S) { return ((o + 1) * S + O - 1) / O; }

__global__ __launch_bounds__(256) void pool_hw_fwd_kernel(const float* __restrict__ x, const double* __restrict__ A,
                                                          const double* __restrict__ B, int act, float* __restrict__ out,
                                                          int T, int H, int W, int OH, int OW) {
    const long nc = blockIdx.y + (long)blockIdx.z * gridDim.y;
    const long ovol = (long)T * OH * OW;
    const long o = (long)blockIdx.x * 256 + threadIdx.x;
    if (o >= ovol) return;
    const float a = A ? A[nc] : 1.0f, b = A ? B[nc] : 0.0f;
    const int ow = (int)(o % OW), oh = (int)((o / OW) % OH), t = (int)(o / ((long)OW * OH));
    const int h0 = ap_start(oh, OH, H), h1 = ap_end(oh, OH, H), w0 = ap_start(ow, OW, W), w1 = ap_end(ow, OW, W);
    const float* p = x + (nc * T + t) * (long)H * W;
    float s = 0.f;
    for (int i = h0; i < h1; ++i)
        for (int j = w0; j < w1; ++j) s += cfn_act_rt(fmaf(p[i * W + j], a, b), act);
    out[nc * ovol + o] = s / (float)((h1 - h0) * (w1 - w0));
}

__global__ __launch_bounds__(256) void pool_hw_bwd_kernel(const float* __restrict__ gout, const float* __restrict__ x,
                                                          const double* __restrict__ A, const double* __restrict__ B, int act,
                                                          float* __restrict__ gx, double* __restrict__ gA,
                                                          double* __restrict__ gB, int T, int H, int W, int OH, int OW) {
    __shared__ float sh[8];
    const long nc = blockIdx.y + (long)blockIdx.z * gridDim.y;
    const long vol = (long)T * H * W;
    const long i = (long)blockIdx.x * 256 + threadIdx.x;
    float acc[2] = {0.f, 0.f};
    if (i < vol) {
        const float a = A ? A[nc] : 1.0f, b = A ? B[nc] : 0.0f;
        const int w = (int)(i % W), h = (int)((i / W) % H), t = (int)(i / ((long)W * H));
        const float* gp = gout + (nc * T + t) * (long)OH * OW;
        float g = 0.f;
        for (int oh = 0; oh < OH; ++oh) {
            const int hs = ap_start(oh, OH, H), he = ap_end(oh, OH, H);
            if (h < hs || h >= he) continue;
            for (int ow = 0; ow < OW; ++ow) {
                const int ws = ap_start(ow, OW, W), we = ap_end(ow, OW, W);
                if (w >= ws && w < we) g += gp[oh * OW + ow] / (float)((he - hs) * (we - ws));
            }
        }
        const float xv = x[nc * vol + i];
        const float dz = g * cfn_act_grad_rt(fmaf(xv, a, b), act);
        acc[0] = dz * xv;
        acc[1] = dz;
        gx[nc * vol + i] = dz * a;
    }
    if (gA) {
        block_sum<2>(acc, sh);
        if (threadIdx.x == 0) { cfn_add64(&gA[nc], (double)acc[0]); cfn_add64(&gB[nc], (double)acc[1]); }
    }
}

__global__ __launch_bounds__(256) void pool_hw1_fwd_kernel(const float* __restrict__ x, const double* __restrict__ A,
                                                           const double* __restrict__ B, int act, float* __restrict__ out,
                                                           int T, int HW) {
    const long nc = blockIdx.y + (long)blockIdx.z * gridDim.y;
    const int lane = threadIdx.x & 63, wv = threadIdx.x >> 6;
    const float a = A ? (float)A[nc] : 1.0f, b = A ? (float)B[nc] : 0.0f;
    const float inv = 1.0f / (float)HW;
    const float* p = x + nc * (long)T * HW;
    for (int t0 = (blockIdx.x * 4 + wv) * 8; t0 < T; t0 += gridDim.x * 32) {
        float v[8];
#pragma unroll
        for (int u = 0; u < 8; ++u) v[u] = (lane < HW && t0 + u < T) ? p[(long)(t0 + u) * HW + lane] : 0.0f;
#pragma unroll
        for (int u = 0; u < 8; ++u) {
            float s = (lane < HW && t0 + u < T) ? cfn_act_rt(fmaf(v[u], a, b), act) : 0.0f;
            s = cfn_wave_sum(s);
            if (lane == 0 && t0 + u < T) out[nc * T + t0 + u] = s * inv;
        }
    }
}

__global__ __launch_bounds__(256) void pool_hw1_bwd_kernel(const float* __restrict__ gout, const float* __restrict__ x,
                                                           const double* __restrict__ A, const double* __restrict__ B, int act,
                                                           float* __restrict__ gx, double* __restrict__ gA,
                                                           double* __restrict__ gB, int T, int HW) {
    __shared__ float sh[8];
    const long nc = blockIdx.y + (long)blockIdx.z * gridDim.y;
    const float a = A ? (float)A[nc] : 1.0f, b = A ? (float)B[nc] : 0.0f;
    const float inv = 1.0f / (float)HW;
    const long vol = (long)T * HW;
    const float* xp = x + nc * vol;
    const float* gp = gout + nc * T;
    float* op = gx + nc * vol;
    float acc[2] = {0.f, 0.f};
    for (long i = threadIdx.x; i < vol; i += 256) {
        const int t = (int)(i / HW);
        const float xv = xp[i];
        const float dz = gp[t] * inv * cfn_act_grad_rt(fmaf(xv, a, b), act);
        acc[0] = fmaf(dz, xv, acc[0]);
        acc[1] += dz;
        op[i] = dz * a;
    }
    if (gA) {
        block_sum<2>(acc, sh);
        if (threadIdx.x == 0) { cfn_add64(&gA[nc], (double)acc[0]); cfn_add64(&gB[nc], (double)acc[1]); }
    }
}

__global__ __launch_bounds__(256) void film_fwd_kernel(const float* __restrict__ x, const float* __restrict__ m,
                                                       const float* __restrict__ c, float* __restrict__ out, int T, int H,
                                                       int W, int f) {
    const long nc = blockIdx.y + (long)blockIdx.z * gridDim.y;
    const long vol = (long)T * H * W;
    const long i = (long)blockIdx.x * 256 + threadIdx.x;
    if (i >= vol) return;
    const int Hs = H / f, Ws = W / f;
    const int w = (int)(i % W), h = (int)((i / W) % H), t = (int)(i / ((long)W * H));
    const long s = (nc * T + t) * (long)Hs * Ws + (long)(h / f) * Ws + w / f;
    out[nc * vol + i] = fmaf(x[nc * vol + i], m[s], c[s]);
}

__global__ __launch_bounds__(256) void film_bwd_kernel(const float* __restrict__ g, const float* __restrict__ x,
                                                       const float* __restrict__ m, float* __restrict__ gx,
                                                       float* __restrict__ gm, float* __restrict__ gc, int T, int H, int W,
                                                       int f) {
    const long nc = blockIdx.y + (long)blockIdx.z * gridDim.y;
    const int Hs = H / f, Ws = W / f;
    const long svol = (long)T * Hs * Ws;
    const long s = (long)blockIdx.x * 256 + threadIdx.x;
    if (s >= svol) return;
    const int ws = (int)(s % Ws), hs = (int)((s / Ws) % Hs), t = (int)(s / ((long)Ws * Hs));
    const long base = (nc * T + t) * (long)H * W + (long)hs * f * W + ws * f;
    const float mv = m[nc * svol + s];
    float a0 = 0.f, a1 = 0.f;
    for (int i = 0; i < f; ++i)
        for (int j = 0; j < f; ++j) {
            const float gv = g[base + i * W + j];
            a0 = fmaf(gv, x[base + i * W + j], a0);
            a1 += gv;
            gx[base + i * W + j] = gv * mv;
        }
    gm[nc * svol + s] = a0;
    gc[nc * svol + s] = a1;
}

static inline dim3 ew_grid(long vol, long NC, int vec) { unsigned gy, gz; cfn_split_nc(NC, gy, gz); return dim3(cfn_cdiv(vol, 256L * EW_ITEMS * vec), gy, gz); }
static inline dim3 nc_grid(long xblocks, long NC) { unsigned gy, gz; cfn_split_nc(NC, gy, gz); return dim3((unsigned)xblocks, gy, gz); }
static inline bool ew_vec4(long vol, const void* p0, const void* p1 = nullptr, const void* p2 = nullptr,
                           const void* p3 = nullptr, const void* p4 = nullptr, const void* p5 = nullptr) {
    auto al = [](const void* p) { return p == nullptr || ((uintptr_t)p & 15) == 0; };
    return vol % 4 == 0 && al(p0) && al(p1) && al(p2) && al(p3) && al(p4) && al(p5);
}
static inline bool ew_flat_ok(long vol, long NC) {
    return vol * 4 < 0x7ffffff0L && NC * (long)cfn_cdiv(vol, 256L * EW_ITEMS * 4) < 0x7fffffffL && NC < 0x7fffffffL;
}
#define CFN_NC_CHECK(NC) CFN_REQUIRE((NC) > 0 && cfn_split_nc_ok(NC), "N*C = %ld has no grid factorisation", (long)(NC))

extern "C" long cfn_bn_add_relu_mask_words(long NC, long vol) {
    if (NC <= 0 || vol <= 0 || vol % 4 != 0) return 0;
    return NC * (long)cfn_cdiv(vol, 256L * EW_ITEMS * 4) * 256;
}

extern "C" int cfn_bn_add_relu_fwd(const float* y, const double* A, const double* B, const float* res, const double* Ar,
                                   const double* Br, float* out, int* mask, long NC, long vol, void* stream) {
    CFN_REQUIRE(y && A && B && res && out, "cfn_bn_add_relu_fwd: null tensor");
    CFN_REQUIRE((Ar == nullptr) == (Br == nullptr), "cfn_bn_add_relu_fwd: Ar/Br mismatch");
    CFN_NC_CHECK(NC);
    hipStream_t st = (hipStream_t)stream;
    CfnProfScope prof(CFN_K_ELEMWISE, st, 12.0 * NC * vol);
    const bool v4 = ew_vec4(vol, y, res, out);
    CFN_REQUIRE(mask == nullptr || v4, "cfn_bn_add_relu_fwd: the bit mask needs vol %% 4 == 0 and 16-byte aligned tensors");
    if (v4 && ew_flat_ok(vol, NC)) {
        EwFlatArgs a = {};
        a.y = y; a.A = A; a.B = B; a.res = res; a.Ar = Ar; a.Br = Br; a.out = out; a.mask = (unsigned*)mask; a.vol = vol;
        a.nchunks = (unsigned)cfn_cdiv(vol, 256L * EW_ITEMS * 4);
        hipLaunchKernelGGL(bn_add_relu_fwd_flat_kernel, dim3((unsigned)(NC * a.nchunks)), dim3(256), 0, st, a);
    } else if (v4) hipLaunchKernelGGL(bn_add_relu_fwd_kernel<4>, ew_grid(vol, NC, 4), dim3(256), 0, st, y, A, B, res, Ar, Br, out, (unsigned*)mask, vol);
    else hipLaunchKernelGGL(bn_add_relu_fwd_kernel<1>, ew_grid(vol, NC, 1), dim3(256), 0, st, y, A, B, res, Ar, Br, out, (unsigned*)nullptr, vol);
    return cfn_check_launch("bn_add_relu_fwd");
}

extern "C" int cfn_bn_add_relu_bwd_g(const float* gout, const float* gout2, const float* out, const int* mask, const float* y,
                                     const float* res, float* g, double* gA, double* gB, double* gAr, long NC, long vol,
                                     void* stream) {
    CFN_REQUIRE(gout && y && g && gA && gB, "cfn_bn_add_relu_bwd_g: null tensor");
    CFN_REQUIRE((out != nullptr) != (mask != nullptr), "cfn_bn_add_relu_bwd_g: exactly one of out / mask");
    CFN_REQUIRE(gAr == nullptr || res != nullptr, "cfn_bn_add_relu_bwd_g: gAr needs res");
    CFN_NC_CHECK(NC);
    hipStream_t st = (hipStream_t)stream;
    CfnProfScope prof(CFN_K_ELEMWISE, st, (12.0 + (gout2 ? 4.0 : 0.0) + (out ? 4.0 : 0.125) + (gAr ? 4.0 : 0.0)) * NC * vol);
    const bool v4 = ew_vec4(vol, gout, out, y, gAr ? res : nullptr, g) && (((uintptr_t)gout2) & 15) == 0;
    CFN_REQUIRE(mask == nullptr || v4, "cfn_bn_add_relu_bwd_g: the bit mask needs vol %% 4 == 0 and 16-byte aligned tensors");
    if (v4 && ew_flat_ok(vol, NC)) {
        EwFlatArgs a = {};
        a.gout = gout; a.gout2 = gout2; a.outr = out; a.maskr = (const unsigned*)mask; a.y = y; a.res = res; a.g = g; a.gA = gA; a.gB = gB; a.gAr = gAr;
        a.vol = vol; a.nchunks = (unsigned)cfn_cdiv(vol, 256L * EW_ITEMS * 4);
        hipLaunchKernelGGL(bn_add_relu_bwd_g_flat_kernel, dim3((unsigned)(NC * a.nchunks)), dim3(256), 0, st, a);
    } else if (v4)
        hipLaunchKernelGGL(bn_add_relu_bwd_g_kernel<4>, ew_grid(vol, NC, 4), dim3(256), 0, st, gout, gout2, out, (const unsigned*)mask, y, res, g, gA, gB, gAr, vol);
    else
        hipLaunchKernelGGL(bn_add_relu_bwd_g_kernel<1>, ew_grid(vol, NC, 1), dim3(256), 0, st, gout, gout2, out, (const unsigned*)nullptr, y, res, g, gA, gB, gAr, vol);
    return cfn_check_launch("bn_add_relu_bwd_g");
}

extern "C" int cfn_bn_add_relu_bwd(const float* gout, const float* gout2, const float* out, const float* y, const double* A, const float* res,
                                   const double* Ar, float* gy, float* gres, double* gA, double* gB, double* gAr, long NC,
                                   long vol, void* stream) {
    CFN_REQUIRE(gout && out && y && A && gy && gres && gA && gB, "cfn_bn_add_relu_bwd: null tensor");
    CFN_REQUIRE(Ar == nullptr || (res != nullptr && gAr != nullptr), "cfn_bn_add_relu_bwd: Ar needs res and gAr");
    CFN_NC_CHECK(NC);
    hipStream_t st = (hipStream_t)stream;
    CfnProfScope prof(CFN_K_ELEMWISE, st, ((Ar ? 24.0 : 20.0) + (gout2 ? 4.0 : 0.0)) * NC * vol);
    if (ew_vec4(vol, gout, out, y, res, gy, gres) && (((uintptr_t)gout2) & 15) == 0)
        hipLaunchKernelGGL(bn_add_relu_bwd_kernel<4>, ew_grid(vol, NC, 4), dim3(256), 0, st, gout, gout2, out, y, A, res, Ar, gy, gres, gA, gB, gAr, vol);
    else
        hipLaunchKernelGGL(bn_add_relu_bwd_kernel<1>, ew_grid(vol, NC, 1), dim3(256), 0, st, gout, gout2, out, y, A, res, Ar, gy, gres, gA, gB, gAr, vol);
    return cfn_check_launch("bn_add_relu_bwd");
}

extern "C" int cfn_affine_act_fwd(const float* x, const double* A, const double* B, int act, float* out, long NC, long vol,
                                  void* stream) {
    CFN_REQUIRE(x && A && B && out, "cfn_affine_act_fwd: null tensor");
    CFN_NC_CHECK(NC);
    hipStream_t st = (hipStream_t)stream;
    CfnProfScope prof(CFN_K_ELEMWISE, st, 8.0 * NC * vol);
    if (ew_vec4(vol, x, out)) hipLaunchKernelGGL(affine_act_fwd_kernel<4>, ew_grid(vol, NC, 4), dim3(256), 0, st, x, A, B, act, out, vol);
    else hipLaunchKernelGGL(affine_act_fwd_kernel<1>, ew_grid(vol, NC, 1), dim3(256), 0, st, x, A, B, act, out, vol);
    return cfn_check_launch("affine_act_fwd");
}

extern "C" int cfn_affine_act_bwd(const float* gout, const float* x, const double* A, const double* B, int act, float* gx,
                                  double* gA, double* gB, long NC, long vol, void* stream) {
    CFN_REQUIRE(gout && x && A && B && gx && gA && gB, "cfn_affine_act_bwd: null tensor");
    CFN_NC_CHECK(NC);
    hipStream_t st = (hipStream_t)stream;
    CfnProfScope prof(CFN_K_ELEMWISE, st, 12.0 * NC * vol);
    if (vol % 4 == 0) hipLaunchKernelGGL(affine_act_bwd_kernel<4>, ew_grid(vol, NC, 4), dim3(256), 0, st, gout, x, A, B, act, gx, gA, gB, vol);
    else hipLaunchKernelGGL(affine_act_bwd_kernel<1>, ew_grid(vol, NC, 1), dim3(256), 0, st, gout, x, A, B, act, gx, gA, gB, vol);
    return cfn_check_launch("affine_act_bwd");
}

extern "C" int cfn_channel_stats(const float* x, double* sum, double* sumsq, long NC, long vol, void* stream) {
    CFN_REQUIRE(x && sum && sumsq, "cfn_channel_stats: null tensor");
    CFN_NC_CHECK(NC);
    hipStream_t st = (hipStream_t)stream;
    CfnProfScope prof(CFN_K_ELEMWISE, st, 4.0 * NC * vol);
    if (ew_vec4(vol, x)) hipLaunchKernelGGL(channel_stats_kernel<4>, ew_grid(vol, NC, 4), dim3(256), 0, st, x, sum, sumsq, vol);
    else hipLaunchKernelGGL(channel_stats_kernel<1>, ew_grid(vol, NC, 1), dim3(256), 0, st, x, sum, sumsq, vol);
    return cfn_check_launch("channel_stats");
}

extern "C" int cfn_pool_hw_fwd(const float* x, const double* A, const double* B, int act, float* out, long NC, int T, int H,
                               int W, int OH, int OW, void* stream) {
    CFN_REQUIRE(x && out, "cfn_pool_hw_fwd: null tensor");
    CFN_REQUIRE((A == nullptr) == (B == nullptr), "cfn_pool_hw_fwd: A/B mismatch");
    CFN_REQUIRE(OH > 0 && OW > 0 && OH <= 64 && OW <= 64, "cfn_pool_hw_fwd: bad output size %dx%d", OH, OW);
    CFN_NC_CHECK(NC);
    hipStream_t st = (hipStream_t)stream;
    const long ovol = (long)T * OH * OW;
    if (OH == 1 && OW == 1 && H * W <= 64) {
        hipLaunchKernelGGL(pool_hw1_fwd_kernel, nc_grid(cfn_cdiv(T, 32) < 16 ? cfn_cdiv(T, 32) : 16, NC), dim3(256), 0, st, x, A, B, act, out, T, H * W);
        return cfn_check_launch("pool_hw_fwd(global mean)");
    }
    hipLaunchKernelGGL(pool_hw_fwd_kernel, nc_grid(cfn_cdiv(ovol, 256), NC), dim3(256), 0, st, x, A, B, act, out, T, H, W, OH, OW);
    return cfn_check_launch("pool_hw_fwd");
}

extern "C" int cfn_pool_hw_bwd(const float* gout, const float* x, const double* A, const double* B, int act, float* gx,
                               double* gA, double* gB, long NC, int T, int H, int W, int OH, int OW, void* stream) {
    CFN_REQUIRE(gout && x && gx, "cfn_pool_hw_bwd: null tensor");
    CFN_REQUIRE((A == nullptr) == (B == nullptr), "cfn_pool_hw_bwd: A/B mismatch");
    CFN_REQUIRE(A == nullptr || (gA && gB), "cfn_pool_hw_bwd: prologue needs gA, gB");
    CFN_REQUIRE(OH > 0 && OW > 0 && OH <= 64 && OW <= 64, "cfn_pool_hw_bwd: bad output size %dx%d", OH, OW);
    CFN_NC_CHECK(NC);
    hipStream_t st = (hipStream_t)stream;
    const long vol = (long)T * H * W;
    if (OH == 1 && OW == 1 && H * W <= 64) {
        hipLaunchKernelGGL(pool_hw1_bwd_kernel, nc_grid(1, NC), dim3(256), 0, st, gout, x, A, B, act, gx,
                           A ? gA : nullptr, A ? gB : nullptr, T, H * W);
        return cfn_check_launch("pool_hw_bwd(global mean)");
    }
    hipLaunchKernelGGL(pool_hw_bwd_kernel, nc_grid(cfn_cdiv(vol, 256), NC), dim3(256), 0, st, gout, x, A, B, act, gx,
                       A ? gA : nullptr, A ? gB : nullptr, T, H, W, OH, OW);
    return cfn_check_launch("pool_hw_bwd");
}

extern "C" int cfn_film_fwd(const float* x, const float* m, const float* c, float* out, long NC, int T, int H, int W, int f,
                            void* stream) {
    CFN_REQUIRE(x && m && c && out, "cfn_film_fwd: null tensor");
    CFN_REQUIRE(f > 0 && H % f == 0 && W % f == 0, "cfn_film_fwd: factor %d does not tile %dx%d", f, H, W);
    CFN_NC_CHECK(NC);
    hipStream_t st = (hipStream_t)stream;
    const long vol = (long)T * H * W;
    CfnProfScope prof(CFN_K_FUSION, st, 8.0 * NC * vol);
    hipLaunchKernelGGL(film_fwd_kernel, nc_grid(cfn_cdiv(vol, 256), NC), dim3(256), 0, st, x, m, c, out, T, H, W, f);
    return cfn_check_launch("film_fwd");
}

extern "C" int cfn_film_bwd(const float* g, const float* x, const float* m, float* gx, float* gm, float* gc, long NC, int T,
                            int H, int W, int f, void* stream) {
    CFN_REQUIRE(g && x && m && gx && gm && gc, "cfn_film_bwd: null tensor");
    CFN_REQUIRE(f > 0 && H % f == 0 && W % f == 0, "cfn_film_bwd: factor %d does not tile %dx%d", f, H, W);
    CFN_NC_CHECK(NC);
    hipStream_t st = (hipStream_t)stream;
    const long svol = (long)T * (H / f) * (W / f);
    CfnProfScope prof(CFN_K_FUSION, st, 12.0 * NC * T * H * W);
    hipLaunchKernelGGL(film_bwd_kernel, nc_grid(cfn_cdiv(svol, 256), NC), dim3(256), 0, st, g, x, m, gx, gm, gc, T, H, W, f);
    return cfn_check_launch("film_bwd");
}
```

coarse-fine-networks_amd/x3d_fine.py:

```python
import os

import torch
import torch.nn as nn
import torch.nn.functional as F

from cfn_hip import ops, ACT_NONE, ACT_RELU, ACT_SWISH
from cfn_hip.u8clips import U8Clips

USE_TORCH_OPS = os.environ.get('CFN_USE_TORCH_OPS', '0') == '1'


class Deferred(object):
    __slots__ = ('raw', 'A', 'B', 'act')

    def __init__(self, raw, A, B, act):
        self.raw, self.A, self.B, self.act = raw, A, B, act

    @property
    def shape(self):
        return self.raw.shape

    def materialize(self):
        return ops.affine_act(self.raw, self.A, self.B, self.act)


def _unpack(x):
    if isinstance(x, Deferred):
        return x.raw, x.A, x.B, x.act
    return x, None, None, ACT_NONE


class SubBatchNorm3d(nn.Module):

    def __init__(self, num_splits, **args):
        super(SubBatchNorm3d, self).__init__()
        self.num_splits = num_splits
        self.num_features = args['num_features']
        self.eps = args.get('eps', 1e-5)
        self.momentum = args.get('momentum', 0.1)
        if args.get('affine', True):
            self.affine = True
            self.weight = nn.Parameter(torch.ones(self.num_features))
            self.bias = nn.Parameter(torch.zeros(self.num_features))
        else:
            self.affine = False
        self.bn = nn.BatchNorm3d(self.num_features, eps=self.eps, momentum=self.momentum, affine=False)
        self.split_bn = nn.BatchNorm3d(self.num_features * self.num_splits, eps=self.eps, momentum=self.momentum,
                                       affine=False)

    def aggregate_stats(self):
        if self.split_bn.track_running_stats:
            n = self.num_splits
            means = self.split_bn.running_mean.view(n, -1)
            mean = means.sum(0) / n
            var = self.split_bn.running_var.view(n, -1).sum(0) / n + ((means - mean) ** 2).sum(0) / n
            self.bn.running_mean.data = mean.detach()
            self.bn.running_var.data = var.detach()

    def fold(self, s, q, count, n, se=None):
        if self.training:
            bufs = (self.split_bn.running_mean, self.split_bn.running_var, self.split_bn.num_batches_tracked)
        else:
            bufs = (self.bn.running_mean, self.bn.running_var, self.bn.num_batches_tracked)
        gamma, beta = (self.weight, self.bias) if self.affine else (None, None)
        return ops.bn_fold(s, q, gamma, beta, bufs, self.training, n, self.num_features, self.num_splits, count, self.eps,
                           self.momentum, se=se, pool_count=count)

    def fold_op(self, s, q, count, n, se=None):
        tr = self.training
        bn = self.split_bn if tr else self.bn
        gamma, beta = (self.weight, self.bias) if self.affine else (None, None)
        w1, b1, w2, b2 = se if se is not None else (None, None, None, None)
        out = torch.ops.cfn.bn_fold(s, q, gamma, beta, bn.running_mean, bn.running_var, bn.num_batches_tracked, tr, n,
                                    self.num_features, self.num_splits, float(count), self.eps, self.momentum, w1, b1, w2, b2, float(count))
        if tr:
            with torch.no_grad():
                bn.running_mean.copy_(out[9])
                bn.running_var.copy_(out[10])
                bn.num_batches_tracked.copy_(out[11])
        return out[0], out[1]

    def forward(self, x):
        n = x.shape[0]
        s = q = None
        if self.training:
            s, q = ops.channel_stats(x)
        A, B = self.fold(s, q, x[0, 0].numel(), n)
        return ops.affine_act(x, A, B, ACT_NONE)


class Swish(nn.Module):

    def forward(self, x):
        n, c = x.shape[:2]
        one = torch.ones(n, c, device=x.device)
        return ops.affine_act(x, one, torch.zeros_like(one), ACT_SWISH)


def conv3x3x3(in_planes, out_planes, stride=1, t_downsample=False):
    return nn.Conv3d(in_planes, out_planes, kernel_size=3, stride=stride if t_downsample else (1, stride, stride), padding=1,
                     bias=False, groups=in_planes)


def conv1x1x1(in_planes, out_planes, stride=1, t_downsample=False):
    return nn.Conv3d(in_planes, out_planes, kernel_size=1, stride=stride if t_downsample else (1, stride, stride), bias=False)


def _every(x, s):
    return x if s == 1 else x[:, :, ::s].contiguous()


def _count(y):
    return y.shape[2] * y.shape[3] * y.shape[4]


class Bottleneck(nn.Module):

    def __init__(self, in_planes, planes, stride=1, downsample=None, index=0, base_bn_splits=8, t_downsample=False):
        super(Bottleneck, self).__init__()
        self.index = index
        self.base_bn_splits = base_bn_splits
        self.conv1 = conv1x1x1(in_planes, planes[0])
        self.bn1 = SubBatchNorm3d(num_splits=base_bn_splits, num_features=planes[0], affine=True)
        self.conv2 = conv3x3x3(planes[0], planes[0], stride, t_downsample=t_downsample)
        self.bn2 = SubBatchNorm3d(num_splits=base_bn_splits, num_features=planes[0], affine=True)
        self.conv3 = conv1x1x1(planes[0], planes[1], t_downsample=t_downsample)
        self.bn3 = SubBatchNorm3d(num_splits=base_bn_splits, num_features=planes[1], affine=True)
        self.swish = Swish()
        self.relu = nn.ReLU(inplace=True)
        if self.index % 2 == 0:
            width = self.round_width(planes[0])
            self.global_pool = nn.AdaptiveAvgPool3d((1, 1, 1))
            self.fc1 = nn.Conv3d(planes[0], width, kernel_size=1, stride=1)
            self.fc2 = nn.Conv3d(width, planes[0], kernel_size=1, stride=1)
            self.sigmoid = nn.Sigmoid()
        self.downsample = downsample
        self.stride = stride
        self.t_stride = stride if t_downsample else 1
        self.split_out = False

    def round_width(self, width, multiplier=0.0625, min_width=8, divisor=8):
        if not multiplier:
            return width
        width *= multiplier
        min_width = min_width or divisor
        width_out = max(min_width, int(width + divisor / 2) // divisor * divisor)
        if width_out < 0.9 * width:
            width_out += divisor
        return int(width_out)

    def _forward_torch_ops(self, x):
        import cfn_hip.torchlib
        T = torch.ops.cfn
        if isinstance(x, tuple):
            x = x[0]
        if isinstance(x, Deferred):
            x = x.materialize()
        if self.t_stride != 1 or (self.downsample is not None and not isinstance(self.downsample, nn.Sequential)):
            raise NotImplementedError('CFN_USE_TORCH_OPS: t_downsample / shortcut type A run on the default path only')
        n = x.shape[0]
        has_se = self.index % 2 == 0
        y1, s1, q1 = T.pwconv(x, self.conv1.weight, None, None, ACT_NONE, 1)
        A1, B1 = self.bn1.fold_op(s1, q1, _count(y1), n)
        y2, s2, q2 = T.dwconv3d(y1, self.conv2.weight, A1, B1, ACT_RELU, self.stride)
        se = (self.fc1.weight, self.fc1.bias, self.fc2.weight, self.fc2.bias) if has_se else None
        A2, B2 = self.bn2.fold_op(s2, q2, _count(y2), n, se=se)
        y3, s3, q3 = T.pwconv(y2, self.conv3.weight, A2, B2, ACT_SWISH, 1)
        A3, B3 = self.bn3.fold_op(s3, q3, _count(y3), n)
        if self.downsample is not None:
            yd, sd, qd = T.pwconv(x, self.downsample[0].weight, None, None, ACT_NONE, self.stride)
            Ad, Bd = self.downsample[1].fold_op(sd, qd, _count(yd), n)
            return T.bn_add_relu(y3, A3, B3, yd, Ad, Bd)
        return T.bn_add_relu(y3, A3, B3, x)

    def forward(self, x):
        if USE_TORCH_OPS:
            return self._forward_torch_ops(x)
        x, x_res = x if isinstance(x, tuple) else (x, x)
        xr, xa, xb, xact = _unpack(x)
        n = xr.shape[0]
        tr = self.training
        has_se = self.index % 2 == 0

        ts = self.t_stride
        tok = ops.ShortcutToken() if (isinstance(self.downsample, nn.Sequential) and self.stride > 1 and ts == 1) else None
        y1, s1, q1 = ops.pwconv(xr, self.conv1.weight, xa, xb, xact, 1, stats=tr, token=tok, role='main')
        A1, B1 = self.bn1.fold(s1, q1, _count(y1), n)
        if ts == 1:
            y2, s2, q2 = ops.dwconv3d(y1, self.conv2.weight, A1, B1, ACT_RELU, self.stride, stats=tr or has_se)
        else:
            y2f, _, _ = ops.dwconv3d(y1, self.conv2.weight, A1, B1, ACT_RELU, self.stride, stats=False)
            y2 = _every(y2f, ts)
            s2, q2 = ops.channel_stats(y2) if (tr or has_se) else (None, None)
        se = (self.fc1.weight, self.fc1.bias, self.fc2.weight, self.fc2.bias) if has_se else None
        A2, B2 = self.bn2.fold(s2, q2, _count(y2), n, se=se)
        link = ops.TailLink() if torch.is_grad_enabled() else None
        y3, s3, q3 = ops.pwconv(y2, self.conv3.weight, A2, B2, ACT_SWISH, 1, stats=tr, tail=link, tail_role='y')
        A3, B3 = self.bn3.fold(s3, q3, _count(y3), n)

        if self.downsample is not None:
            if not isinstance(self.downsample, nn.Sequential):
                _, planes_out, s_ = self.downsample
                xm = x_res.materialize() if isinstance(x_res, Deferred) else x_res
                res = xm.detach()[:, :, ::s_, ::s_, ::s_]
                if planes_out > res.shape[1]:
                    res = torch.cat([res, res.new_zeros((res.shape[0], planes_out - res.shape[1]) + tuple(res.shape[2:]))], dim=1)
                return ops.bn_add_relu(y3, A3, B3, res.contiguous(), split=self.split_out, link=link)
            yd, sd, qd = ops.pwconv(_every(xr, ts), self.downsample[0].weight, xa, xb, xact, self.stride, stats=tr, token=tok, role='short',
                                    tail=link, tail_role='res')
            Ad, Bd = self.downsample[1].fold(sd, qd, _count(yd), n)
            return ops.bn_add_relu(y3, A3, B3, yd, Ad, Bd, split=self.split_out, link=link)
        res = x_res.materialize() if isinstance(x_res, Deferred) else x_res
        return ops.bn_add_relu(y3, A3, B3, res, split=self.split_out, link=link)


class ResNet(nn.Module):

    def __init__(self, block, layers, block_inplanes, n_input_channels=3, conv1_t_size=7, conv1_t_stride=1,
                 shortcut_type='B', widen_factor=1.0, dropout=0.5, n_classes=400, base_bn_splits=8, task='class',
                 extract_feat=False, global_tower=False, t_downsample=False, aux_losses=None, _skip_module_init=False,
                 act_dtype=None):
        if not _skip_module_init:
            super(ResNet, self).__init__()
        block_inplanes = [(int(x * widen_factor), int(y * widen_factor)) for x, y in block_inplanes]
        self.index = 0
        self.base_bn_splits = base_bn_splits
        self.task = task
        self.extract_feat = extract_feat
        self.global_tower = global_tower
        self.t_downsample = t_downsample
        self.act_dtype = {None: torch.float32, 'f32': torch.float32, 'fp32': torch.float32, torch.float32: torch.float32,
                          'bf16': torch.bfloat16, torch.bfloat16: torch.bfloat16,
                          'fp16': torch.float16, 'f16': torch.float16, torch.float16: torch.float16}[act_dtype]
        self.in_planes = block_inplanes[0][1]

        self.conv1_s = nn.Conv3d(n_input_channels, self.in_planes, kernel_size=(1, 3, 3), stride=(1, 2, 2),
                                 padding=(0, 1, 1), bias=False)
        self.conv1_t = nn.Conv3d(self.in_planes, self.in_planes, kernel_size=(5, 1, 1), stride=(1, 1, 1),
                                 padding=(2, 0, 0), bias=False, groups=self.in_planes)
        self.bn1 = SubBatchNorm3d(num_splits=base_bn_splits, num_features=self.in_planes, affine=True)
        self.relu = nn.ReLU(inplace=True)
        self.layer1 = self._make_layer(block, block_inplanes[0], layers[0], shortcut_type, stride=2)
        self.layer2 = self._make_layer(block, block_inplanes[1], layers[1], shortcut_type, stride=2)
        self.layer3 = self._make_layer(block, block_inplanes[2], layers[2], shortcut_type, stride=2)
        self.layer4 = self._make_layer(block, block_inplanes[3], layers[3], shortcut_type, stride=2)
        self.conv5 = nn.Conv3d(block_inplanes[3][1], block_inplanes[3][0], kernel_size=(1, 1, 1), stride=(1, 1, 1),
                               padding=(0, 0, 0), bias=False)
        self.bn5 = SubBatchNorm3d(num_splits=base_bn_splits, num_features=block_inplanes[3][0], affine=True)
        if task == 'class':
            self.avgpool = nn.AdaptiveAvgPool3d((1, 1, 1))
        elif task == 'loc':
            self.avgpool = nn.AdaptiveAvgPool3d((None, 1, 1))
        self.fc1 = nn.Conv3d(block_inplanes[3][0], 2048, bias=False, kernel_size=1, stride=1)
        self.fc2 = nn.Linear(2048, n_classes)
        self.dropout = nn.Dropout(dropout)

        for m in self.modules():
            if isinstance(m, nn.Conv3d):
                nn.init.kaiming_normal_(m.weight, mode='fan_out', nonlinearity='relu')

    def _make_layer(self, block, planes, blocks, shortcut_type, stride=1):
        downsample = None
        if stride != 1 or self.in_planes != planes[1]:
            if shortcut_type == 'A':
                downsample = ('A', planes[1], stride)
            else:
                downsample = nn.Sequential(
                    conv1x1x1(self.in_planes, planes[1], stride, t_downsample=self.t_downsample),
                    SubBatchNorm3d(num_splits=self.base_bn_splits, num_features=planes[1], affine=True))
        layers = [block(in_planes=self.in_planes, planes=planes, stride=stride, downsample=downsample,
                        index=self.index, base_bn_splits=self.base_bn_splits, t_downsample=self.t_downsample)]
        self.in_planes = planes[1]
        self.index += 1
        for _ in range(1, blocks):
            layers.append(block(self.in_planes, planes, index=self.index, base_bn_splits=self.base_bn_splits,
                                t_downsample=self.t_downsample))
            self.index += 1
        self.index = 0
        for blk in layers[:-1]:
            blk.split_out = True
        return nn.Sequential(*layers)

    def replace_logits(self, n_classes):
        self.fc2 = nn.Linear(2048, n_classes).to(self.fc1.weight.device)

    def update_bn_splits_long_cycle(self, long_cycle_bn_scale):
        for m in self.modules():
            if isinstance(m, SubBatchNorm3d):
                m.num_splits = self.base_bn_splits * long_cycle_bn_scale
                m.split_bn = nn.BatchNorm3d(num_features=m.num_features * m.num_splits, affine=False).to(m.weight.device)
        return self.base_bn_splits * long_cycle_bn_scale

    def aggregate_sub_bn_stats(self):
        count = 0
        for m in self.modules():
            if isinstance(m, SubBatchNorm3d):
                m.aggregate_stats()
                count += 1
        return count

    def set_input_norm(self, mean, std, norm_value=255):
        lut = ops.clip_lut(mean, std, norm_value).to(self.conv1_s.weight.device)
        self.register_buffer('input_lut', lut, persistent=False)
        return self

    def _conv1_s(self, x):
        if not isinstance(x, U8Clips):
            return ops.stem_conv(x, self.conv1_s.weight)
        lut = getattr(self, 'input_lut', None)
        if lut is None:
            raise RuntimeError('the model was handed uint8 frames (U8Clips) but does not know how to normalise them: call '
                               'set_input_norm(mean, std) first (e.g. CHARADES_MEAN / CHARADES_STD)')
        if x.frames.dim() != 5:
            raise RuntimeError('U8Clips of shape (N, T, H, W, 3) expected (flatten_crops() a collated batch), got %s'
                               % (tuple(x.frames.shape),))
        return ops.stem_conv_u8(x.frames, x.lengths, lut, self.conv1_s.weight)

    def _stem(self, x):
        y = self._conv1_s(x)
        y, s, q = ops.dwconv_t5(y, self.conv1_t.weight, stats=self.training, out_dtype=self.act_dtype)
        A, B = self.bn1.fold(s, q, _count(y), y.shape[0])
        return Deferred(y, A, B, ACT_RELU)

    def _head(self, x):
        n = x.shape[0]
        y5, s5, q5 = ops.pwconv(x, self.conv5.weight, stats=self.training)
        A5, B5 = self.bn5.fold(s5, q5, _count(y5), n)
        if self.task == 'class':
            pooled = ops.pool_hw(y5, 1, 1, A5, B5, ACT_RELU).mean(dim=2, keepdim=True)
        else:
            pooled = ops.pool_hw(y5, 1, 1, A5, B5, ACT_RELU)
        if self.extract_feat:
            return pooled
        f1, _, _ = ops.pwconv(pooled, self.fc1.weight, stats=False)
        one = torch.ones(n, f1.shape[1], device=f1.device)
        z = ops.affine_act(f1, one, torch.zeros_like(one), ACT_RELU)
        z = self.dropout(z)
        out, _, _ = ops.pwconv(z, self.fc2.weight.view(self.fc2.weight.shape[0], -1, 1, 1, 1), stats=False)
        out = out.squeeze(4).squeeze(3) + self.fc2.bias.view(1, -1, 1)
        return out

    def forward(self, inp):
        x, masks = inp
        x = self._stem(x)
        feat_g = {}
        for i, layer in enumerate((self.layer1, self.layer2, self.layer3, self.layer4), start=1):
            x = layer(x)
            if self.global_tower:
                feat_g['layer%d' % i] = ops.pool_hw(x, 7, 7)
        if self.global_tower:
            n = x.shape[0]
            y5, s5, q5 = ops.pwconv(x, self.conv5.weight, stats=self.training)
            A5, B5 = self.bn5.fold(s5, q5, _count(y5), n)
            feat_g['conv5'] = ops.pool_hw(y5, 7, 7, A5, B5, ACT_RELU)
            return feat_g, masks
        return self._head(x)


def replace_logits(self, n_classes):
    self.fc2 = nn.Linear(2048, n_classes)


def get_inplanes(version):
    planes = {'S': [(54, 24), (108, 48), (216, 96), (432, 192)],
              'M': [(54, 24), (108, 48), (216, 96), (432, 192)],
              'XL': [(72, 32), (162, 72), (306, 136), (630, 280)]}
    return planes[version]


def get_blocks(version):
    blocks = {'S': [3, 5, 11, 7], 'M': [3, 5, 11, 7], 'XL': [5, 10, 25, 15]}
    return blocks[version]


def generate_model(x3d_version, **kwargs):
    return ResNet(Bottleneck, get_blocks(x3d_version), get_inplanes(x3d_version), **kwargs)
```

include/cfn_hip.h:

```cpp
#ifndef CFN_HIP_H
#define CFN_HIP_H
#ifdef __cplusplus
extern "C" {
#endif

const char* cfn_last_error(void);
const char* cfn_version(void);
int cfn_device_info(int* cus, int* lds_per_cu, char* name, int name_len);

int cfn_prof_enable(int family, int on);
int cfn_prof_collect(int family, double* total_ms, long* launches, double* total_bytes);

int cfn_dwconv3d_fwd(const float* x, const double* A, const double* B, int act, const float* w, float* y, double* sum,
                     double* sumsq, int N, int C, int T, int Hi, int Wi, int stride, void* stream);
int cfn_dwconv3d_bwd_data(const float* gy, const float* y, const double* gsum, const double* gsumsq, const float* w,
                          const float* x, const double* A, const double* B, int act, float* gx, double* gA, double* gB,
                          int N, int C, int T, int Hi, int Wi, int stride, void* stream);
int cfn_dwconv3d_bwd_weight(const float* gy, const float* y, const double* gsum, const double* gsumsq, const float* x,
                            const double* A, const double* B, int act, double* gw, int N, int C, int T, int Hi, int Wi,
                            int stride, void* stream);
int cfn_dwconv3d_bwd_fused(const float* gy, const float* y, const double* gsum, const double* gsumsq, const float* w,
                           const float* x, const double* A, const double* B, int act, float* gx, double* gA, double* gB,
                           double* gw, int N, int C, int T, int H, int W, void* stream);
int cfn_dwconv3d_bwd_fused_s2(const float* gy, const float* y, const double* gsum, const double* gsumsq, const float* w,
                              const float* x, const double* A, const double* B, int act, float* gx, double* gA, double* gB,
                              double* gw, int N, int C, int T, int H, int W, void* stream);

int cfn_dwconv_t5_fwd(const float* x, const float* w, float* y, double* sum, double* sumsq, int N, int C, int T,
                      long plane, void* stream);
int cfn_dwconv_t5_bwd_data(const float* gy, const float* y, const double* gsum, const double* gsumsq, const float* w,
                           float* gx, int N, int C, int T, long plane, void* stream);
int cfn_dwconv_t5_bwd_weight(const float* gy, const float* y, const double* gsum, const double* gsumsq, const float* x,
                             double* gw, int N, int C, int T, long plane, void* stream);
int cfn_dwconv_t5_bwd_fused(const float* gy, const float* y, const double* gsum, const double* gsumsq, const float* w,
                            const float* x, float* gx, double* gw, int N, int C, int T, long plane, void* stream);

int cfn_pwconv_fwd(const float* x, const double* A, const double* B, int act, const float* w, float* y, double* sum,
                   double* sumsq, int N, int Cin, int Cout, int T, int Hi, int Wi, int stride, void* stream);
int cfn_pwconv_bwd_data(const float* gy, const float* y, const double* gsum, const double* gsumsq, const float* w,
                        const float* x, const double* A, const double* B, int act, float* gx, double* gA, double* gB, int N,
                        int Cin, int Cout, int T, int Hi, int Wi, int stride, void* stream);
int cfn_pwconv_bwd_data_acc(const float* gy, const float* y, const double* gsum, const double* gsumsq, const float* w,
                        const float* x, const double* A, const double* B, int act, float* gx, double* gA, double* gB, int N,
                        int Cin, int Cout, int T, int Hi, int Wi, int stride, const float* acc, int acc_stride,
                        const double* gscale, void* stream);
int cfn_pwconv_bwd_weight(const float* gy, const float* y, const double* gsum, const double* gsumsq, const float* x,
                          const double* A, const double* B, int act, double* gw, int N, int Cin, int Cout, int T, int Hi,
                          int Wi, int stride, const double* gscale, void* stream);

int cfn_pw_split_terms(int terms);

int cfn_deterministic(int on);

int cfn_pwconv_bwd_fused(const float* gy, const float* y, const double* gsum, const double* gsumsq, const float* w,
                         const float* x, const double* A, const double* B, int act, float* gx, double* gA, double* gB,
                         double* gw, int N, int Cin, int Cout, int T, int Hi, int Wi, const float* acc, int acc_stride,
                         const double* gscale, void* stream);

int cfn_pwconv_short_bwd(const float* gy, const float* y, const double* gsum, const double* gsumsq, const double* gscale,
                         const float* w, const float* x, const double* A, const double* B, int act, float* da, double* gw,
                         int N, int Cin, int Cout, int T, int Hi, int Wi, int stride, void* stream);

int cfn_stem_conv_fwd(const float* x, const float* w, float* y, int N, int Cimg, int Cout, int T, int Hi, int Wi,
                      void* stream);
int cfn_stem_conv_bwd_weight(const float* gy, const float* x, double* gw, int N, int Cimg, int Cout, int T, int Hi, int Wi,
                             void* stream);

int cfn_clip_u8_to_f32(const unsigned char* frames, const float* lut, const int* lengths, float* x, int N, int T, int H, int W,
                       void* stream);
int cfn_stem_conv_u8_fwd(const unsigned char* frames, const float* lut, const int* lengths, const float* w, float* y, int N,
                         int Cimg, int Cout, int T, int Hi, int Wi, void* stream);
int cfn_stem_conv_u8_bwd_weight(const float* gy, const unsigned char* frames, const float* lut, const int* lengths, double* gw,
                                int N, int Cimg, int Cout, int T, int Hi, int Wi, void* stream);

int cfn_bn_fold_fwd(const double* s, const double* q, const float* gamma, const float* beta, float* run_mean, float* run_var,
                    long* nbt, int training, int N, int C, int S, double count, double eps, double momentum, const float* w1,
                    const float* b1, const float* w2, const float* b2, int Wd, double pool_count, double* A, double* B,
                    double* mean, double* rstd, float* A0, float* B0, float* gate, float* hbuf, float* pooled, void* stream);
int cfn_bn_fold_bwd(const double* gA, const double* gB, const double* s, const float* gamma, const double* mean,
                    const double* rstd, const float* A0, const float* B0, const float* gate, const float* hbuf,
                    const float* pooled, const float* w1, const float* w2, int training, int N, int C, int S, int Wd,
                    double count, double pool_count, double* gs, double* gq, float* ggamma, float* gbeta, float* gw1,
                    float* gb1, float* gw2, float* gb2, double* tA, double* tB, void* stream);

int cfn_conv3d_dense_fwd(const float* x, const double* A, const double* B, int act, const float* w, float* y, double* sum,
                         double* sumsq, int N, int Cin, int Cout, int T, int Hi, int Wi, const int* geom, void* stream);
int cfn_conv3d_dense_bwd_data(const float* gy, const float* y, const double* gsum, const double* gsumsq, const float* w,
                              const float* x, const double* A, const double* B, int act, float* gx, double* gA, double* gB,
                              int N, int Cin, int Cout, int T, int Hi, int Wi, const int* geom, void* stream);
int cfn_conv3d_dense_bwd_weight(const float* gy, const float* y, const double* gsum, const double* gsumsq, const float* x,
                                const double* A, const double* B, int act, double* gw, int N, int Cin, int Cout, int T, int Hi,
                                int Wi, const int* geom, void* stream);

int cfn_gauss_align_fwd(const long* meta, const float* mask, const float* gx, double tx, double ratio, float* GX, int B, int crops,
                        int Tf, int K, void* stream);
int cfn_gauss_align_bwd(const float* gGX, const long* meta, const float* mask, const float* gx, double tx, double ratio,
                        float* ggx, int B, int crops, int Tf, int K, void* stream);

int cfn_fusion_gather_fwd(const float* x, const float* at_raw, const float* at_bias, const float* GX, const float* mask, float* z,
                          float* den, int B, int crops, int C, int Tf, int K, int P, void* stream);
int cfn_fusion_gather_bwd(const float* gz, const float* z, const float* den, const float* x, const float* at_raw,
                          const float* at_bias, const float* GX, const float* mask, float* gx, float* gat, float* gGX, float* dw,
                          int B, int crops, int C, int Tf, int K, int P, void* stream);

int cfn_bn_add_relu_fwd(const float* y, const double* A, const double* B, const float* res, const double* Ar, const double* Br,
                        float* out, int* mask, long NC, long vol, void* stream);
int cfn_bn_add_relu_bwd(const float* gout, const float* gout2, const float* out, const float* y, const double* A, const float* res,
                        const double* Ar, float* gy, float* gres, double* gA, double* gB, double* gAr, long NC, long vol,
                        void* stream);
long cfn_bn_add_relu_mask_words(long NC, long vol);
int cfn_bn_add_relu_bwd_g(const float* gout, const float* gout2, const float* out, const int* mask, const float* y,
                          const float* res, float* g, double* gA, double* gB, double* gAr, long NC, long vol, void* stream);

int cfn_affine_act_fwd(const float* x, const double* A, const double* B, int act, float* out, long NC, long vol, void* stream);
int cfn_affine_act_bwd(const float* gout, const float* x, const double* A, const double* B, int act, float* gx, double* gA,
                       double* gB, long NC, long vol, void* stream);
int cfn_channel_stats(const float* x, double* sum, double* sumsq, long NC, long vol, void* stream);

int cfn_pool_hw_fwd(const float* x, const double* A, const double* B, int act, float* out, long NC, int T, int H, int W, int OH,
                    int OW, void* stream);
int cfn_pool_hw_bwd(const float* gout, const float* x, const double* A, const double* B, int act, float* gx, double* gA,
                    double* gB, long NC, int T, int H, int W, int OH, int OW, void* stream);

int cfn_film_fwd(const float* x, const float* m, const float* c, float* out, long NC, int T, int H, int W, int f,
                 void* stream);
int cfn_film_bwd(const float* g, const float* x, const float* m, float* gx, float* gm, float* gc, long NC, int T, int H,
                 int W, int f, void* stream);

int cfn_grid_time_index(const float* cdf, int n, int Tin, int* i0, float* w1, void* stream);
int cfn_grid_cdf_fwd(const float* g, const float* bias, float* cdf, int B, int Kin, void* stream);
int cfn_grid_cdf_bwd(const float* gcdf, const float* g, const float* bias, float* gg, int B, int Kin, void* stream);
int cfn_time_sample_fwd(const float* x, const float* cdf, float* out, int B, int C, int Tin, int K, long P, void* stream);
int cfn_time_sample_bwd(const float* g, const float* x, const float* cdf, float* gx, double* gcdf, int B, int C, int Tin,
                        int K, long P, void* stream);

int cfn_time_pool_fwd(const float* x, float* out, int mode, long BC, int Tin, int R, long P, void* stream);
int cfn_time_pool_bwd(const float* g, const float* x, float* gx, int mode, long BC, int Tin, int R, long P, void* stream);

int cfn_interp1d_fwd(const float* x, const float* y, const float* xnew, float* ynew, long* ind, int B, int N, int Pq,
                     int xrow, int yrow, int qrow, void* stream);
int cfn_interp1d_bwd(const float* g, const float* x, const float* y, const float* xnew, const long* ind, float* gx, float* gy,
                     float* gq, int B, int N, int Pq, int xrow, int yrow, int qrow, void* stream);

int cfn_time_resize_fwd(const float* x, float* out, long BC, int Kin, int Lout, long P, int align_corners, void* stream);
int cfn_time_resize_bwd(const float* g, float* gx, long BC, int Kin, int Lout, long P, int align_corners, void* stream);

int cfn_detloss_fwd(const float* logits, const float* labels, const float* masks, const float* norm, double world, float* probs,
                    float* cls, float* loc, int* jstar, float* ymax, double* rows, double* norm_used, int B, int C, int T, int TL,
                    int n, int align_corners, void* stream);
int cfn_detloss_bwd(const float* g_cls, const float* g_loc, const float* logits, const float* labels, const float* masks,
                    const int* jstar, const float* ymax, const double* norm_used, double world, float* gx, int B, int C, int T,
                    int TL, int n, int align_corners, void* stream);

int cfn_pwconv_fwd_bf16(const unsigned short* x, const double* A, const double* B, int act, const float* w, unsigned short* y,
                        double* sum, double* sumsq, int N, int Cin, int Cout, long Q, void* stream);
int cfn_pwconv_bwd_data_bf16(const unsigned short* gy, const unsigned short* y, const double* gsum, const double* gsumsq,
                             const float* w, const unsigned short* x, const double* A, const double* B, int act,
                             unsigned short* gx, double* gA, double* gB, int N, int Cin, int Cout, int T, int H, int W,
                             const unsigned short* acc, int acc_stride, const double* gscale, void* stream);
int cfn_pwconv_bwd_weight_bf16(const unsigned short* gy, const unsigned short* y, const double* gsum, const double* gsumsq,
                               const unsigned short* x, const double* A, const double* B, int act, double* gw, int N, int Cin,
                               int Cout, long Q, const double* gscale, void* stream);
int cfn_subsample_hw_bf16(const unsigned short* x, unsigned short* out, long planes, int H, int W, int s, void* stream);

int cfn_dwconv3d_fwd_bf16(const unsigned short* x, const double* A, const double* B, int act, const float* w, unsigned short* y,
                          double* sum, double* sumsq, int N, int C, int T, int Hi, int Wi, int stride, void* stream);
int cfn_dwconv3d_bwd_data_bf16(const unsigned short* gy, const unsigned short* y, const double* gsum, const double* gsumsq,
                               const float* w, const unsigned short* x, const double* A, const double* B, int act,
                               unsigned short* gx, double* gA, double* gB, int N, int C, int T, int Hi, int Wi, int stride,
                               void* stream);
int cfn_dwconv3d_bwd_weight_bf16(const unsigned short* gy, const unsigned short* y, const double* gsum, const double* gsumsq,
                                 const unsigned short* x, const double* A, const double* B, int act, double* gw, int N, int C,
                                 int T, int Hi, int Wi, int stride, void* stream);
int cfn_dwconv3d_bwd_fused_bf16(const unsigned short* gy, const unsigned short* y, const double* gsum, const double* gsumsq,
                                const float* w, const unsigned short* x, const double* A, const double* B, int act,
                                unsigned short* gx, double* gA, double* gB, double* gw, int N, int C, int T, int H, int W,
                                void* stream);
int cfn_dwconv3d_bwd_fused_s2_bf16(const unsigned short* gy, const unsigned short* y, const double* gsum, const double* gsumsq,
                                   const float* w, const unsigned short* x, const double* A, const double* B, int act,
                                   unsigned short* gx, double* gA, double* gB, double* gw, int N, int C, int T, int H, int W,
                                   void* stream);

int cfn_dwconv_t5_fwd_bf16(const float* x, const float* w, unsigned short* y, double* sum, double* sumsq, int N, int C, int T,
                           long plane, void* stream);
int cfn_dwconv_t5_bwd_data_bf16(const unsigned short* gy, const unsigned short* y, const double* gsum, const double* gsumsq,
                                const float* w, float* gx, int N, int C, int T, long plane, void* stream);
int cfn_dwconv_t5_bwd_weight_bf16(const unsigned short* gy, const unsigned short* y, const double* gsum, const double* gsumsq,
                                  const float* x, double* gw, int N, int C, int T, long plane, void* stream);
int cfn_dwconv_t5_bwd_fused_bf16(const unsigned short* gy, const unsigned short* y, const double* gsum, const double* gsumsq,
                                 const float* w, const float* x, float* gx, double* gw, int N, int C, int T, long plane,
                                 void* stream);

long cfn_bn_add_relu_mask_words_bf16(long NC, long vol);
int cfn_bn_add_relu_fwd_bf16(const unsigned short* y, const double* A, const double* B, const unsigned short* res,
                             const double* Ar, const double* Br, unsigned short* out, int* mask, long NC, long vol, void* stream);
int cfn_bn_add_relu_bwd_g_bf16(const unsigned short* gout, const unsigned short* gout2, const unsigned short* out, const int* mask,
                               const unsigned short* y, const unsigned short* res, unsigned short* g, double* gA, double* gB,
                               double* gAr, long NC, long vol, void* stream);
int cfn_pool_hw_fwd_bf16(const unsigned short* x, const double* A, const double* B, int act, float* out, long NC, int T, int H,
                         int W, int OH, int OW, void* stream);
int cfn_pool_hw_bwd_bf16(const float* gout, const unsigned short* x, const double* A, const double* B, int act,
                         unsigned short* gx, double* gA, double* gB, long NC, int T, int H, int W, int OH, int OW, void* stream);

int cfn_pwconv_fwd_f16(const unsigned short* x, const double* A, const double* B, int act, const float* w, unsigned short* y,
                        double* sum, double* sumsq, int N, int Cin, int Cout, long Q, void* stream);
int cfn_pwconv_bwd_data_f16(const unsigned short* gy, const unsigned short* y, const double* gsum, const double* gsumsq,
                             const float* w, const unsigned short* x, const double* A, const double* B, int act,
                             unsigned short* gx, double* gA, double* gB, int N, int Cin, int Cout, int T, int H, int W,
                             const unsigned short* acc, int acc_stride, const double* gscale, void* stream);
int cfn_pwconv_bwd_weight_f16(const unsigned short* gy, const unsigned short* y, const double* gsum, const double* gsumsq,
                               const unsigned short* x, const double* A, const double* B, int act, double* gw, int N, int Cin,
                               int Cout, long Q, const double* gscale, void* stream);
int cfn_subsample_hw_f16(const unsigned short* x, unsigned short* out, long planes, int H, int W, int s, void* stream);

int cfn_dwconv3d_fwd_f16(const unsigned short* x, const double* A, const double* B, int act, const float* w, unsigned short* y,
                          double* sum, double* sumsq, int N, int C, int T, int Hi, int Wi, int stride, void* stream);
int cfn_dwconv3d_bwd_data_f16(const unsigned short* gy, const unsigned short* y, const double* gsum, const double* gsumsq,
                               const float* w, const unsigned short* x, const double* A, const double* B, int act,
                               unsigned short* gx, double* gA, double* gB, int N, int C, int T, int Hi, int Wi, int stride,
                               void* stream);
int cfn_dwconv3d_bwd_weight_f16(const unsigned short* gy, const unsigned short* y, const double* gsum, const double* gsumsq,
                                 const unsigned short* x, const double* A, const double* B, int act, double* gw, int N, int C,
                                 int T, int Hi, int Wi, int stride, void* stream);
int cfn_dwconv3d_bwd_fused_f16(const unsigned short* gy, const unsigned short* y, const double* gsum, const double* gsumsq,
                                const float* w, const unsigned short* x, const double* A, const double* B, int act,
                                unsigned short* gx, double* gA, double* gB, double* gw, int N, int C, int T, int H, int W,
                                void* stream);
int cfn_dwconv3d_bwd_fused_s2_f16(const unsigned short* gy, const unsigned short* y, const double* gsum, const double* gsumsq,
                                   const float* w, const unsigned short* x, const double* A, const double* B, int act,
                                   unsigned short* gx, double* gA, double* gB, double* gw, int N, int C, int T, int H, int W,
                                   void* stream);

int cfn_dwconv_t5_fwd_f16(const float* x, const float* w, unsigned short* y, double* sum, double* sumsq, int N, int C, int T,
                           long plane, void* stream);
int cfn_dwconv_t5_bwd_data_f16(const unsigned short* gy, const unsigned short* y, const double* gsum, const double* gsumsq,
                                const float* w, float* gx, int N, int C, int T, long plane, void* stream);
int cfn_dwconv_t5_bwd_weight_f16(const unsigned short* gy, const unsigned short* y, const double* gsum, const double* gsumsq,
                                  const float* x, double* gw, int N, int C, int T, long plane, void* stream);
int cfn_dwconv_t5_bwd_fused_f16(const unsigned short* gy, const unsigned short* y, const double* gsum, const double* gsumsq,
                                 const float* w, const float* x, float* gx, double* gw, int N, int C, int T, long plane,
                                 void* stream);

long cfn_bn_add_relu_mask_words_f16(long NC, long vol);
int cfn_bn_add_relu_fwd_f16(const unsigned short* y, const double* A, const double* B, const unsigned short* res,
                             const double* Ar, const double* Br, unsigned short* out, int* mask, long NC, long vol, void* stream);
int cfn_bn_add_relu_bwd_g_f16(const unsigned short* gout, const unsigned short* gout2, const unsigned short* out, const int* mask,
                               const unsigned short* y, const unsigned short* res, unsigned short* g, double* gA, double* gB,
                               double* gAr, long NC, long vol, void* stream);
int cfn_pool_hw_fwd_f16(const unsigned short* x, const double* A, const double* B, int act, float* out, long NC, int T, int H,
                         int W, int OH, int OW, void* stream);
int cfn_pool_hw_bwd_f16(const float* gout, const unsigned short* x, const double* A, const double* B, int act,
                         unsigned short* gx, double* gA, double* gB, long NC, int T, int H, int W, int OH, int OW, void* stream);

int cfn_crop_resize_flip_u8(const unsigned char* src, const int* lengths, const int* box, const int* bounds, const int* coef,
                            unsigned char* dst, int N, int T, int Hs, int Ws, int S, int K, void* stream);

int cfn_ap_append(const float* probs, const float* labels, const int* valid, float* scores, unsigned char* targets, int* count,
                  int* flags, int B, int K, int TL, long cap, void* stream);
int cfn_ap_sort(const float* scores, const unsigned char* targets, const int* count, float* sorted_scores,
                unsigned char* sorted_targets, int* tmp_keys, unsigned char* tmp_targets, int K, long cap, void* stream);
int cfn_ap_reduce(const unsigned char* sorted_targets, const int* count, float* ap, int K, long cap, void* stream);
int cfn_ap_sort_tile(void);

int cfn_feat_unpack_f16(const unsigned short* data, const long* offsets, const int* lengths, float* out0, float* out1, float* out2,
                        float* out3, float* out4, int B, int t_max, int c0, int c1, int c2, int c3, int c4, long total, void* stream);
int cfn_feat_unpack_bf16(const unsigned short* data, const long* offsets, const int* lengths, float* out0, float* out1, float* out2,
                         float* out3, float* out4, int B, int t_max, int c0, int c1, int c2, int c3, int c4, long total, void* stream);
int cfn_feat_pack_f16(const float* x0, const float* x1, const float* x2, const float* x3, const float* x4, unsigned short* dst, int T,
                      int c0, int c1, int c2, int c3, int c4, void* stream);
int cfn_feat_pack_bf16(const float* x0, const float* x1, const float* x2, const float* x3, const float* x4, unsigned short* dst, int T,
                       int c0, int c1, int c2, int c3, int c4, void* stream);

long cfn_jpeg_workspace_bytes(int rows, long slots, int lanes, int blocks_max);
int cfn_jpeg_decode_u8(const unsigned char* data, const int* frames, const int* tables, const int* geom, const int* lengths,
                       unsigned char* out, int* status, void* ws, long ws_bytes, long data_bytes, int rows, int sets, int N,
                       int Tmax, int Hmax, int Wmax, int lanes, int blocks_max, void* stream);

#ifdef __cplusplus
}
#endif
#endif
```

Measured before the change: 106.9 clips/s.

## Fuse BN fold with bottleneck add-ReLU tail in forward and backward

Adds a bn_tail op that computes the BN fold (mean/rstd, running stats, A/B coefficients) inside the elementwise add-ReLU kernel in forward. In backward it folds the BN-fold adjoint into the add-ReLU gradient kernel using per-channel tickets, so the last block finishes the channel reduction. This removes separate small fold launches per bottleneck block. The SE fold backward is also split across several workgroups by channel, and the SE weight staging now uses float4 loads. The trade is extra kernel complexity, atomic ticket ordering, and double work where fold stats are recomputed per chunk.

```diff
diff --git a/coarse-fine-networks_amd/cfn_hip/ops.py b/coarse-fine-networks_amd/cfn_hip/ops.py
--- a/coarse-fine-networks_amd/cfn_hip/ops.py
+++ b/coarse-fine-networks_amd/cfn_hip/ops.py
@@ -91,6 +91,7 @@
 
 _tls = _PerThread()
 LAZY_GRAD_CAST = True
+FUSED_BN_TAIL = True
 
 
 def _f64(n, c, dev):
@@ -807,6 +808,100 @@
     return _BnAddRelu.apply(y, A, B, res, Ar, Br, split, link)
 
 
+class _BnTail(Function):
+
+    @staticmethod
+    def forward(ctx, y, s, q, gamma, beta, res, sr, qr, gammar, betar, bufs, bufsr, cfg, split, link):
+        N, C, S, count, eps, momentum, countr, epsr, momentumr = cfg
+        y, res = check(y).contiguous(), check(res).contiguous()
+        vol = y[0, 0].numel()
+        if tuple(res.shape) != tuple(y.shape):
+            raise RuntimeError('bn_tail: residual %s does not match y %s' % (tuple(res.shape), tuple(y.shape)))
+        dev = y.device
+        short = sr is not None
+        s, q, sr, qr = _opt(s), _opt(q), _opt(sr), _opt(qr)
+        out = torch.empty_like(y)
+        mask = torch.empty(query('cfn_bn_add_relu_mask_words', N * C, vol), dtype=torch.int32, device=dev)
+
+        def coef():
+            A = torch.empty(N, C, dtype=torch.float64, device=dev)
+            mean = torch.empty(S, C, dtype=torch.float64, device=dev)
+            return A, torch.empty_like(A), mean, torch.empty_like(mean)
+        A, B, mean, rstd = coef()
+        Ar, Br, meanr, rstdr = coef() if short else (None,) * 4
+        rm, rv, nbt = bufs
+        rmr, rvr, nbtr = bufsr if short else (None,) * 3
+        if not call_try('cfn_bn_tail_fwd', y, res, s, q, gamma, beta, rm, rv, nbt, float(count), float(eps), float(momentum), sr, qr,
+                        gammar, betar, rmr, rvr, nbtr, float(countr), float(epsr), float(momentumr), 1, N, C, S, vol, out, mask,
+                        A, B, mean, rstd, Ar, Br, meanr, rstdr):
+            call('cfn_bn_fold_fwd', s, q, gamma, beta, rm, rv, nbt, 1, N, C, S, float(count), float(eps), float(momentum),
+                 None, None, None, None, 0, float(count), A, B, mean, rstd, None, None, None, None, None)
+            if short:
+                call('cfn_bn_fold_fwd', sr, qr, gammar, betar, rmr, rvr, nbtr, 1, N, C, S, float(countr), float(epsr), float(momentumr),
+                     None, None, None, None, 0, float(countr), Ar, Br, meanr, rstdr, None, None, None, None, None)
+            call('cfn_bn_add_relu_fwd', y, A, B, res, Ar, Br, out, mask, N * C, vol)
+        ctx.link, ctx.cfg, ctx.short = link, (N, C, S, vol, count, countr), short
+        ctx.save_for_backward(y, res if short else None, mask, A, Ar, gamma, mean, rstd, gammar, meanr, rstdr)
+        if not split:
+            return out
+        alias = torch.empty(0, dtype=out.dtype, device=out.device).set_(out.untyped_storage(), out.storage_offset(),
+                                                                         out.shape, out.stride())
+        return out, alias
+
+    @staticmethod
+    @once_differentiable
+    def backward(ctx, gout, gout2=None):
+        y, res, mask, A, Ar, gamma, mean, rstd, gammar, meanr, rstdr = ctx.saved_tensors
+        N, C, S, vol, count, countr = ctx.cfg
+        short, dev = ctx.short, y.device
+        if gout is None:
+            gout, gout2 = gout2, None
+        if gout is None:
+            gout = torch.zeros_like(y)
+        gout = gout.contiguous()
+        gout2 = None if gout2 is None else gout2.contiguous()
+        t3 = _tls.arena.take(3 * N * C, dev).view(3, N, C)
+        gA, gB = t3[0], t3[1]
+        gAr = t3[2] if short else None
+        tickets = _tls.arena.take((C + 1) // 2, dev).view(torch.int32)
+        g = torch.empty_like(y)
+
+        def grads(gam):
+            gs = torch.empty(N, C, dtype=torch.float64, device=dev)
+            gg, gbt = (torch.empty(C, device=dev), torch.empty(C, device=dev)) if gam is not None else (None, None)
+            return gs, torch.empty_like(gs), gg, gbt
+        gs, gq, gg, gbt = grads(gamma)
+        gsr, gqr, ggr, gbtr = grads(gammar) if short else (None,) * 4
+        if not call_try('cfn_bn_tail_bwd', gout, gout2, mask, y, res, g, gA, gB, gAr, tickets, gamma, mean, rstd, float(count),
+                        gs, gq, gg, gbt, gammar, meanr, rstdr, float(countr), gsr, gqr, ggr, gbtr, N, C, S, vol):
+            call('cfn_bn_add_relu_bwd_g', gout, gout2, None, mask, y, res, g, gA, gB, gAr, N * C, vol)
+            call('cfn_bn_fold_bwd', gA, gB, None, gamma, mean, rstd, None, None, None, None, None, None, None, 1, N, C, S, 0,
+                 float(count), float(count), gs, gq, gg, gbt, None, None, None, None, None, None)
+            if short:
+                call('cfn_bn_fold_bwd', gAr, gB, None, gammar, meanr, rstdr, None, None, None, None, None, None, None, 1, N, C, S, 0,
+                     float(countr), float(countr), gsr, gqr, ggr, gbtr, None, None, None, None, None, None)
+        link = ctx.link
+        link.y_scale, link.res_scale, link.done = A.detach(), (None if Ar is None else Ar.detach()), True
+        g2 = torch.empty(0, dtype=g.dtype, device=g.device).set_(g.untyped_storage(), g.storage_offset(), g.shape, g.stride())
+        return g, gs, gq, gg, gbt, g2, gsr, gqr, ggr, gbtr, None, None, None, None, None
+
+
+def bn_tail(y, res, training, N, C, bn, short=None, split=False, link=None):
+    s, q, gamma, beta, bufs, S, count, eps, momentum = bn
+    fused = (FUSED_BN_TAIL and training and link is not None and y.dtype == torch.float32 and res.dtype == torch.float32
+             and y[0, 0].numel() % 4 == 0 and (short is None or short[5] == S))
+    if fused:
+        sr, qr, gammar, betar, bufsr, _, countr, epsr, momentumr = short if short is not None else (None,) * 5 + (S, count, eps, momentum)
+        return _BnTail.apply(y, s, q, gamma, beta, res, sr, qr, gammar, betar, bufs, bufsr,
+                             (N, C, S, count, eps, momentum, countr, epsr, momentumr), split, link)
+    A, B = bn_fold(s, q, gamma, beta, bufs, training, N, C, S, count, eps, momentum, pool_count=count)
+    Ar = Br = None
+    if short is not None:
+        sr, qr, gammar, betar, bufsr, Sr, countr, epsr, momentumr = short
+        Ar, Br = bn_fold(sr, qr, gammar, betar, bufsr, training, N, C, Sr, countr, epsr, momentumr, pool_count=countr)
+    return bn_add_relu(y, A, B, res, Ar, Br, split=split, link=link)
+
+
 class _AffineAct(Function):
     @staticmethod
     def forward(ctx, x, A, B, act):
diff --git a/coarse-fine-networks_amd/csrc/bnfold.hip b/coarse-fine-networks_amd/csrc/bnfold.hip
--- a/coarse-fine-networks_amd/csrc/bnfold.hip
+++ b/coarse-fine-networks_amd/csrc/bnfold.hip
@@ -1,4 +1,5 @@
 #include "cfn_common.h"
+#include "bnfold_math.h"
 #include <stdlib.h>
 
 struct BnFoldArgs {
@@ -18,7 +19,18 @@
 #define BNF_NB 8
 
 __device__ __forceinline__ void bnf_stage_se(const float* w1, const float* w2, float* w1s, float* w2s, int C, int Wd) {
-    for (int e = threadIdx.x; e < C * Wd; e += blockDim.x) {
+    const int n = C * Wd;
+    if ((Wd & 3) == 0 && ((((uintptr_t)w1) | ((uintptr_t)w2)) & 15) == 0) {
+        for (int e = threadIdx.x * 4; e < n; e += blockDim.x * 4) {
+            const float4 u = *reinterpret_cast<const float4*>(w1 + e), v = *reinterpret_cast<const float4*>(w2 + e);
+            *reinterpret_cast<float4*>(w1s + e) = u;
+            const int c = e / Wd, j = e - c * Wd;
+            float* d = w2s + c * (Wd + 1) + j;
+            d[0] = v.x; d[1] = v.y; d[2] = v.z; d[3] = v.w;
+        }
+        return;
+    }
+    for (int e = threadIdx.x; e < n; e += blockDim.x) {
         w1s[e] = w1[e];
         const int c = e / Wd, j = e - c * Wd;
         w2s[c * (Wd + 1) + j] = w2[e];
@@ -27,7 +39,7 @@
 
 __global__ __launch_bounds__(1024) void bn_fold_fwd_kernel(const BnFoldArgs a) {
     const int tid = threadIdx.x, nthr = blockDim.x, N = a.N, C = a.C, S = a.training ? a.S : 1, G = N / S, Wd = a.Wd;
-    extern __shared__ float sh[];
+    extern __shared__ __attribute__((aligned(16))) float sh[];
     const bool st = Wd > 0 && a.stage;
     float* sp = sh + (st ? Wd * C + C * (Wd + 1) : 0);
     float* shh = sp + BNF_NB * C;
@@ -41,27 +53,11 @@
     for (int e = ps ? gown * C + tid : gtid; e < (ps ? (gown + 1) * C : S * C); e += gn) {
         const bool wr = !ps || (int)blockIdx.x == gown;
         const int g = e / C, c = e - g * C;
-        double mean, var;
-        if (a.training) {
-            double ss = 0.0, qq = 0.0;
-            for (int i = 0; i < G; ++i) { ss += a.s[(long)(i * S + g) * C + c]; qq += a.q[(long)(i * S + g) * C + c]; }
-            const double cnt = a.count * G;
-            mean = ss / cnt;
-            var = qq / cnt - mean * mean;
-            if (var < 0.0) var = 0.0;
-            const double unb = var * (cnt / (cnt > 1.0 ? cnt - 1.0 : 1.0));
-            if (wr) {
-                a.run_mean[e] = (float)((1.0 - a.momentum) * (double)a.run_mean[e] + a.momentum * mean);
-                a.run_var[e] = (float)((1.0 - a.momentum) * (double)a.run_var[e] + a.momentum * unb);
-            }
-        } else {
-            mean = (double)a.run_mean[c];
-            var = (double)a.run_var[c];
-        }
-        const double rstd = 1.0 / sqrt(var + a.eps);
+        double mean, unb, rstd;
+        float av, bv;
+        bnf_stats(a.training, a.s, a.q, a.run_mean, a.run_var, a.gamma, a.beta, S, G, C, g, c, a.count, a.eps, mean, unb, rstd, av, bv);
+        if (a.training && wr) bnf_running_update(a.run_mean, a.run_var, e, a.momentum, mean, unb);
         if (wr) { a.mean[e] = mean; a.rstd[e] = rstd; }
-        const double ga = a.gamma ? (double)a.gamma[c] : 1.0, be = a.beta ? (double)a.beta[c] : 0.0;
-        const float av = (float)(ga * rstd), bv = (float)(be - mean * ga * rstd);
         for (int i = 0; i < G; ++i) {
             if (ps && i * S + g != (int)blockIdx.x) continue;
             const long o = (long)(i * S + g) * C + c;
@@ -123,9 +119,17 @@
     double* tA; double* tB;
 };
 
+__device__ __forceinline__ double bnf_mul_then_add(double x, double y, double z) {
+#pragma clang fp contract(off)
+    const double p = x * y;
+    return p + z;
+}
+
 __global__ __launch_bounds__(1024) void bn_fold_bwd_kernel(const BnFoldBwdArgs a) {
     const int tid = threadIdx.x, nthr = blockDim.x, N = a.N, C = a.C, S = a.training ? a.S : 1, G = N / S, Wd = a.Wd;
-    extern __shared__ float sh[];
+    extern __shared__ __attribute__((aligned(16))) float sh[];
+    const int cw = Wd > 0 ? (C + (int)gridDim.x - 1) / (int)gridDim.x : C;
+    const int c0 = Wd > 0 ? min(C, (int)blockIdx.x * cw) : 0, c1 = Wd > 0 ? min(C, c0 + cw) : C, ncw = c1 - c0;
     if (Wd > 0) {
         const bool st = a.stage != 0;
         const float* w1s = st ? sh : a.w1;
@@ -147,17 +151,15 @@
                 const float ggate = a.gA[o] * a.A0[o] + a.gB[o] * a.B0[o];
                 gz2[e] = ggate * gt * (1.0f - gt);
                 pl[e] = a.pooled[o];
-                a.tA[o] = a.gA[o] * gt;
-                a.tB[o] = a.gB[o] * gt;
             }
             __syncthreads();
-            for (int e = tid; e < C * Wd; e += nthr) {
+            for (int e = c0 * Wd + tid; e < c1 * Wd; e += nthr) {
                 const int c = e / Wd, j = e - c * Wd;
                 float acc = 0.0f;
                 for (int nl = 0; nl < nb; ++nl) acc = fmaf(gz2[nl * C + c], shh[nl * Wd + j], acc);
                 a.gw2[e] = first ? acc : a.gw2[e] + acc;
             }
-            for (int c = tid; c < C; c += nthr) {
+            for (int c = c0 + tid; c < c1; c += nthr) {
                 float acc = 0.0f;
                 for (int nl = 0; nl < nb; ++nl) acc += gz2[nl * C + c];
                 a.gb2[c] = first ? acc : a.gb2[c] + acc;
@@ -170,25 +172,27 @@
                 if (lane == 0) gz1[p] = shh[p] > 0.0f ? acc : 0.0f;
             }
             __syncthreads();
-            for (int e = tid; e < Wd * C; e += nthr) {
-                const int j = e / C, c = e - j * C;
+            for (int e = tid; e < Wd * ncw; e += nthr) {
+                const int j = e / ncw, c = c0 + (e - j * ncw);
                 float acc = 0.0f;
                 for (int nl = 0; nl < nb; ++nl) acc = fmaf(gz1[nl * Wd + j], pl[nl * C + c], acc);
-                a.gw1[e] = first ? acc : a.gw1[e] + acc;
-            }
-            for (int j = tid; j < Wd; j += nthr) {
-                float acc = 0.0f;
-                for (int nl = 0; nl < nb; ++nl) acc += gz1[nl * Wd + j];
-                a.gb1[j] = first ? acc : a.gb1[j] + acc;
-            }
-            for (int e = tid; e < nb * C; e += nthr) {
-                const int nl = e / C, c = e - nl * C;
+                a.gw1[j * C + c] = first ? acc : a.gw1[j * C + c] + acc;
+            }
+            if (blockIdx.x == 0)
+                for (int j = tid; j < Wd; j += nthr) {
+                    float acc = 0.0f;
+                    for (int nl = 0; nl < nb; ++nl) acc += gz1[nl * Wd + j];
+                    a.gb1[j] = first ? acc : a.gb1[j] + acc;
+                }
+            for (int e = tid; e < nb * ncw; e += nthr) {
+                const int nl = e / ncw, c = c0 + (e - nl * ncw);
                 float gp = 0.0f;
                 for (int j = 0; j < Wd; ++j) gp = fmaf(gz1[nl * Wd + j], w1s[j * C + c], gp);
-                const long o = (long)n0 * C + e;
+                const long o = (long)(n0 + nl) * C + c;
                 const float sm = (float)(a.s[o] / a.pool_count);
-                a.tA[o] += gp * sm;
-                a.tB[o] += gp;
+                const float gt = a.gate[o];
+                a.tA[o] = bnf_mul_then_add(a.gA[o], (double)gt, (double)(gp * sm));
+                a.tB[o] = bnf_mul_then_add(a.gB[o], (double)gt, (double)gp);
                 if (a.gs) a.gs[o] = (double)(gp * a.A0[o]) / a.pool_count;
             }
             __syncthreads();
@@ -196,30 +200,9 @@
     }
     const double* dA = Wd > 0 ? a.tA : a.gA;
     const double* dB = Wd > 0 ? a.tB : a.gB;
-    const int gtid = Wd > 0 ? tid : (int)(blockIdx.x * blockDim.x) + tid, gn = Wd > 0 ? nthr : (int)(gridDim.x * blockDim.x);
-    for (int c = gtid; c < C; c += gn) {
-        double ggam = 0.0, gbet = 0.0;
-        for (int g = 0; g < S; ++g) {
-            double ga = 0.0, gb = 0.0;
-            for (int i = 0; i < G; ++i) { ga += dA[(long)(i * S + g) * C + c]; gb += dB[(long)(i * S + g) * C + c]; }
-            const double mean = a.mean[g * C + c], rstd = a.rstd[g * C + c];
-            const double gam = a.gamma ? (double)a.gamma[c] : 1.0;
-            ggam += (ga - gb * mean) * rstd;
-            gbet += gb;
-            if (a.training && a.gs) {
-                const double cnt = a.count * G;
-                const double g_rstd = (ga - gb * mean) * gam;
-                const double g_var = g_rstd * (-0.5 * rstd * rstd * rstd);
-                const double g_mean = -gb * gam * rstd - 2.0 * mean * g_var;
-                for (int i = 0; i < G; ++i) {
-                    const long o = (long)(i * S + g) * C + c;
-                    a.gs[o] = (Wd > 0 ? a.gs[o] : 0.0) + g_mean / cnt;
-                    a.gq[o] = g_var / cnt;
-                }
-            }
-        }
-        if (a.ggamma) { a.ggamma[c] = (float)ggam; a.gbeta[c] = (float)gbet; }
-    }
+    const int gtid = Wd > 0 ? c0 + tid : (int)(blockIdx.x * blockDim.x) + tid, gn = Wd > 0 ? nthr : (int)(gridDim.x * blockDim.x);
+    for (int c = gtid; c < c1; c += gn)
+        bnf_channel_adjoint(BnfLoadPlain(), dA, dB, a.mean, a.rstd, a.gamma, a.training, S, G, C, c, a.count, Wd > 0, a.gs, a.gq, a.ggamma, a.gbeta);
 }
 
 extern "C" int cfn_bn_fold_fwd(const double* s, const double* q, const float* gamma, const float* beta, float* run_mean,
@@ -263,6 +246,7 @@
                        pool_count, gs, gq, ggamma, gbeta, gw1, gb1, gw2, gb2, tA, tB};
     CFN_REQUIRE(lds <= 150 * 1024, "cfn_bn_fold_bwd: per-sample SE tables (C=%d, width=%d) exceed LDS", C, Wd);
     if (lds > 48 * 1024) (void)hipFuncSetAttribute((const void*)bn_fold_bwd_kernel, hipFuncAttributeMaxDynamicSharedMemorySize, (int)lds);
-    hipLaunchKernelGGL(bn_fold_bwd_kernel, dim3(Wd > 0 ? 1 : cfn_cdiv(C, 64)), dim3(Wd > 0 ? 1024 : 64), lds, (hipStream_t)stream, a);
+    const int Wg = C / 32 < 1 ? 1 : (C / 32 > 8 ? 8 : C / 32);
+    hipLaunchKernelGGL(bn_fold_bwd_kernel, dim3(Wd > 0 ? Wg : cfn_cdiv(C, 64)), dim3(Wd > 0 ? 1024 : 64), lds, (hipStream_t)stream, a);
     return cfn_check_launch("bn_fold_bwd");
 }
diff --git a/coarse-fine-networks_amd/csrc/bnfold_math.h b/coarse-fine-networks_amd/csrc/bnfold_math.h
--- /dev/null
+++ b/coarse-fine-networks_amd/csrc/bnfold_math.h
@@ -0,0 +1,68 @@
+#pragma once
+
+__device__ __forceinline__ void bnf_stats(int training, const double* s, const double* q, const float* run_mean, const float* run_var,
+                                          const float* gamma, const float* beta, int S, int G, int C, int g, int c, double count, double eps,
+                                          double& mean, double& unb, double& rstd, float& av, float& bv) {
+    double var;
+    unb = 0.0;
+    if (training) {
+        double ss = 0.0, qq = 0.0;
+        for (int i = 0; i < G; ++i) { ss += s[(long)(i * S + g) * C + c]; qq += q[(long)(i * S + g) * C + c]; }
+        const double cnt = count * G;
+        mean = ss / cnt;
+        var = qq / cnt - mean * mean;
+        if (var < 0.0) var = 0.0;
+        unb = var * (cnt / (cnt > 1.0 ? cnt - 1.0 : 1.0));
+    } else {
+        mean = (double)run_mean[c];
+        var = (double)run_var[c];
+    }
+    rstd = 1.0 / sqrt(var + eps);
+    const double ga = gamma ? (double)gamma[c] : 1.0, be = beta ? (double)beta[c] : 0.0;
+    av = (float)(ga * rstd);
+    bv = (float)(be - mean * ga * rstd);
+}
+
+__device__ __forceinline__ void bnf_running_update(float* run_mean, float* run_var, int e, double momentum, double mean, double unb) {
+    run_mean[e] = (float)((1.0 - momentum) * (double)run_mean[e] + momentum * mean);
+    run_var[e] = (float)((1.0 - momentum) * (double)run_var[e] + momentum * unb);
+}
+
+struct BnfLoadPlain { __device__ __forceinline__ double operator()(const double* p) const { return *p; } };
+struct BnfLoadAgent {
+    __device__ __forceinline__ double operator()(const double* p) const { return __hip_atomic_load(p, __ATOMIC_RELAXED, __HIP_MEMORY_SCOPE_AGENT); }
+};
+
+template <class LD>
+__device__ __forceinline__ void bnf_channel_adjoint(LD ld, const double* dA, const double* dB, const double* mean_, const double* rstd_,
+                                                    const float* gamma, int training, int S, int G, int C, int c, double count, bool gs_acc,
+                                                    double* gs, double* gq, float* ggamma, float* gbeta) {
+    double ggam = 0.0, gbet = 0.0;
+    for (int g = 0; g < S; ++g) {
+        double ga = 0.0, gb = 0.0;
+        for (int i = 0; i < G; ++i) { ga += ld(dA + (long)(i * S + g) * C + c); gb += ld(dB + (long)(i * S + g) * C + c); }
+        const double mean = mean_[g * C + c], rstd = rstd_[g * C + c];
+        const double gam = gamma ? (double)gamma[c] : 1.0;
+        ggam += (ga - gb * mean) * rstd;
+        gbet += gb;
+        if (training && gs) {
+            const double cnt = count * G;
+            const double g_rstd = (ga - gb * mean) * gam;
+            const double g_var = g_rstd * (-0.5 * rstd * rstd * rstd);
+            const double g_mean = -gb * gam * rstd - 2.0 * mean * g_var;
+            for (int i0 = 0; i0 < G; i0 += 4) {
+                double old[4];
+#pragma unroll
+                for (int k = 0; k < 4; ++k) old[k] = (gs_acc && i0 + k < G) ? gs[(long)((i0 + k) * S + g) * C + c] : 0.0;
+#pragma unroll
+                for (int k = 0; k < 4; ++k)
+                    if (i0 + k < G) {
+                        const long o = (long)((i0 + k) * S + g) * C + c;
+                        gs[o] = old[k] + g_mean / cnt;
+                        gq[o] = g_var / cnt;
+                    }
+            }
+        }
+    }
+    if (ggamma) { ggamma[c] = (float)ggam; gbeta[c] = (float)gbet; }
+}
diff --git a/coarse-fine-networks_amd/csrc/cfn_common.h b/coarse-fine-networks_amd/csrc/cfn_common.h
--- a/coarse-fine-networks_amd/csrc/cfn_common.h
+++ b/coarse-fine-networks_amd/csrc/cfn_common.h
@@ -12,6 +12,7 @@
 enum { CFN_ACT_NONE = 0, CFN_ACT_RELU = 1, CFN_ACT_SWISH = 2, CFN_ACT_SIGMOID = 3 };
 
 extern "C" const char* cfn_last_error(void);
+extern "C" int cfn_deterministic(int on);
 int cfn_fail(int code, const char* fmt, ...);
 int cfn_check_launch(const char* what);
 
diff --git a/coarse-fine-networks_amd/csrc/elementwise.hip b/coarse-fine-networks_amd/csrc/elementwise.hip
--- a/coarse-fine-networks_amd/csrc/elementwise.hip
+++ b/coarse-fine-networks_amd/csrc/elementwise.hip
@@ -1,4 +1,5 @@
 #include "cfn_common.h"
+#include "bnfold_math.h"
 #include <stdlib.h>
 
 typedef float __attribute__((ext_vector_type(4))) f4v;
@@ -184,6 +185,128 @@
     }
 }
 
+struct BnTailFwdBn {
+    const double* s; const double* q; const float* gamma; const float* beta; float* run_mean; float* run_var; long* nbt;
+    double* A; double* B; double* mean; double* rstd;
+    double count, eps, momentum;
+};
+struct BnTailFwdArgs { EwFlatArgs e; BnTailFwdBn m, r; int N, C, S, hasr; };
+
+__device__ __forceinline__ void bn_tail_coef(const BnTailFwdBn& b, int N, int C, int S, int g, int c, bool lead, float& av, float& bv) {
+    const int G = N / S;
+    double mean, unb, rstd;
+    bnf_stats(1, b.s, b.q, b.run_mean, b.run_var, b.gamma, b.beta, S, G, C, g, c, b.count, b.eps, mean, unb, rstd, av, bv);
+    if (lead) {
+        const int e = g * C + c;
+        bnf_running_update(b.run_mean, b.run_var, e, b.momentum, mean, unb);
+        b.mean[e] = mean; b.rstd[e] = rstd;
+        for (int i = 0; i < G; ++i) { const long o = (long)(i * S + g) * C + c; b.A[o] = av; b.B[o] = bv; }
+        if (b.nbt && e == 0) b.nbt[0] += 1;
+    }
+}
+
+__global__ __launch_bounds__(256) void bn_tail_fwd_flat_kernel(const BnTailFwdArgs t) {
+    constexpr int OOB = 0x7ffffff0;
+    const EwFlatArgs& a = t.e;
+    const unsigned L = cfn_xcd_remap(blockIdx.x, gridDim.x);
+    const long nc = cfn_uni((int)(L / a.nchunks));
+    const unsigned chunk = cfn_uni(L - (unsigned)nc * a.nchunks);
+    const unsigned bytes = (unsigned)(a.vol * 4);
+    __amdgpu_buffer_rsrc_t ry = cfn_rsrc(a.y + nc * a.vol, bytes), rr = cfn_rsrc(a.res + nc * a.vol, bytes), ro = cfn_rsrc(a.out + nc * a.vol, bytes);
+    const long i0 = ((long)chunk * 256 * EW_ITEMS + threadIdx.x) * 4;
+    f4v yv[EW_ITEMS], rv[EW_ITEMS];
+    int off[EW_ITEMS];
+#pragma unroll
+    for (int k = 0; k < EW_ITEMS; ++k) {
+        const long i = i0 + (long)k * 1024;
+        off[k] = i < a.vol ? (int)(i * 4) : OOB;
+        yv[k] = __builtin_bit_cast(f4v, __builtin_amdgcn_raw_buffer_load_b128(ry, off[k], 0, 0));
+        rv[k] = __builtin_bit_cast(f4v, __builtin_amdgcn_raw_buffer_load_b128(rr, off[k], 0, 0));
+    }
+    const int n = (int)nc / t.C, c = (int)nc - n * t.C, g = n % t.S;
+    const bool lead = chunk == 0 && n == g && threadIdx.x == 0;
+    float av, bv, avr = 1.0f, bvr = 0.0f;
+    bn_tail_coef(t.m, t.N, t.C, t.S, g, c, lead, av, bv);
+    if (t.hasr) bn_tail_coef(t.r, t.N, t.C, t.S, g, c, lead, avr, bvr);
+    const float ca = av, cb = (float)((double)bv + (double)bvr), car = avr;
+    unsigned mw = 0;
+#pragma unroll
+    for (int k = 0; k < EW_ITEMS; ++k) {
+        f4v o;
+        o.x = fmaxf(fmaf(yv[k].x, ca, fmaf(rv[k].x, car, cb)), 0.f); o.y = fmaxf(fmaf(yv[k].y, ca, fmaf(rv[k].y, car, cb)), 0.f);
+        o.z = fmaxf(fmaf(yv[k].z, ca, fmaf(rv[k].z, car, cb)), 0.f); o.w = fmaxf(fmaf(yv[k].w, ca, fmaf(rv[k].w, car, cb)), 0.f);
+        cfn_bst128(__builtin_bit_cast(unsigned __attribute__((ext_vector_type(4))), o), ro, off[k], 0);
+        if (off[k] != OOB) mw |= ((o.x > 0.f ? 1u : 0u) | (o.y > 0.f ? 2u : 0u) | (o.z > 0.f ? 4u : 0u) | (o.w > 0.f ? 8u : 0u)) << (4 * k);
+    }
+    a.mask[((unsigned long)nc * a.nchunks + chunk) * 256 + threadIdx.x] = mw;
+}
+
+struct BnTailBwdBn {
+    const float* gamma; const double* mean; const double* rstd; double count;
+    double* gs; double* gq; float* ggamma; float* gbeta;
+};
+struct BnTailBwdArgs { EwFlatArgs e; BnTailBwdBn m, r; unsigned* tickets; int N, C, S; };
+
+__global__ __launch_bounds__(256) void bn_tail_bwd_flat_kernel(const BnTailBwdArgs t) {
+    constexpr int OOB = 0x7ffffff0;
+    __shared__ float sh[12];
+    const EwFlatArgs& a = t.e;
+    const unsigned L = cfn_xcd_remap(blockIdx.x, gridDim.x);
+    const long nc = cfn_uni((int)(L / a.nchunks));
+    const unsigned chunk = cfn_uni(L - (unsigned)nc * a.nchunks);
+    const unsigned bytes = (unsigned)(a.vol * 4);
+    const bool has2 = a.gout2 != nullptr, hasr = a.gAr != nullptr;
+    __amdgpu_buffer_rsrc_t rg = cfn_rsrc(a.gout + nc * a.vol, bytes), rg2 = cfn_rsrc((has2 ? a.gout2 : a.gout) + nc * a.vol, has2 ? bytes : 0u);
+    __amdgpu_buffer_rsrc_t ry = cfn_rsrc(a.y + nc * a.vol, bytes);
+    __amdgpu_buffer_rsrc_t rr = cfn_rsrc((hasr ? a.res : a.gout) + nc * a.vol, bytes), rd = cfn_rsrc(a.g + nc * a.vol, bytes);
+    const long i0 = ((long)chunk * 256 * EW_ITEMS + threadIdx.x) * 4;
+    const unsigned mw = a.maskr[((unsigned long)nc * a.nchunks + chunk) * 256 + threadIdx.x];
+    f4v go[EW_ITEMS], g2v[EW_ITEMS], yv[EW_ITEMS];
+    int off[EW_ITEMS];
+#pragma unroll
+    for (int k = 0; k < EW_ITEMS; ++k) {
+        const long i = i0 + (long)k * 1024;
+        off[k] = i < a.vol ? (int)(i * 4) : OOB;
+        go[k] = __builtin_bit_cast(f4v, __builtin_amdgcn_raw_buffer_load_b128(rg, off[k], 0, 0));
+        g2v[k] = __builtin_bit_cast(f4v, __builtin_amdgcn_raw_buffer_load_b128(rg2, off[k], 0, 0));
+        yv[k] = __builtin_bit_cast(f4v, __builtin_amdgcn_raw_buffer_load_b128(ry, off[k], 0, 0));
+    }
+    float acc[3] = {0.f, 0.f, 0.f};
+#pragma unroll
+    for (int k = 0; k < EW_ITEMS; ++k) {
+        f4v rv;
+        const f4v g2 = g2v[k];
+        if (hasr) rv = __builtin_bit_cast(f4v, __builtin_amdgcn_raw_buffer_load_b128(rr, off[k], 0, 0));
+        const f4v gs = go[k] + g2;
+        const unsigned m4 = (mw >> (4 * k)) & 15u;
+        f4v g;
+        g.x = (m4 & 1u) ? gs.x : 0.f; g.y = (m4 & 2u) ? gs.y : 0.f;
+        g.z = (m4 & 4u) ? gs.z : 0.f; g.w = (m4 & 8u) ? gs.w : 0.f;
+        acc[0] += g.x * yv[k].x + g.y * yv[k].y + g.z * yv[k].z + g.w * yv[k].w;
+        acc[1] += g.x + g.y + g.z + g.w;
+        if (hasr) acc[2] += g.x * rv.x + g.y * rv.y + g.z * rv.z + g.w * rv.w;
+        cfn_bst128(__builtin_bit_cast(unsigned __attribute__((ext_vector_type(4))), g), rd, off[k], 0);
+    }
+    block_sum<3>(acc, sh);
+    if (threadIdx.x == 0) {
+        atomicAdd(&a.gA[nc], (double)acc[0]);
+        atomicAdd(&a.gB[nc], (double)acc[1]);
+        if (hasr) atomicAdd(&a.gAr[nc], (double)acc[2]);
+        const int c = (int)(nc % t.C);
+        asm volatile("s_waitcnt vmcnt(0)" ::: "memory");
+        const unsigned old = __hip_atomic_fetch_add(&t.tickets[c], 1u, __ATOMIC_RELAXED, __HIP_MEMORY_SCOPE_AGENT);
+        if (old == (unsigned)t.N * a.nchunks - 1u) {
+            __builtin_amdgcn_fence(__ATOMIC_ACQUIRE, "agent");
+            const int G = t.N / t.S;
+            bnf_channel_adjoint(BnfLoadAgent(), a.gA, a.gB, t.m.mean, t.m.rstd, t.m.gamma, 1, t.S, G, t.C, c, t.m.count, false,
+                                t.m.gs, t.m.gq, t.m.ggamma, t.m.gbeta);
+            if (hasr)
+                bnf_channel_adjoint(BnfLoadAgent(), a.gAr, a.gB, t.r.mean, t.r.rstd, t.r.gamma, 1, t.S, G, t.C, c, t.r.count, false,
+                                    t.r.gs, t.r.gq, t.r.ggamma, t.r.gbeta);
+        }
+    }
+}
+
 template <int VEC>
 __global__ __launch_bounds__(256) void bn_add_relu_bwd_kernel(const float* __restrict__ gout, const float* __restrict__ gout2,
                                                               const float* __restrict__ out,
@@ -507,6 +630,58 @@
     return cfn_check_launch("bn_add_relu_bwd_g");
 }
 
+extern "C" int cfn_bn_tail_fwd(const float* y, const float* res, const double* s, const double* q, const float* gamma, const float* beta,
+                               float* run_mean, float* run_var, long* nbt, double count, double eps, double momentum, const double* sr,
+                               const double* qr, const float* gammar, const float* betar, float* run_meanr, float* run_varr, long* nbtr,
+                               double countr, double epsr, double momentumr, int training, int N, int C, int S, long vol, float* out,
+                               int* mask, double* A, double* B, double* mean, double* rstd, double* Ar, double* Br, double* meanr,
+                               double* rstdr, void* stream) {
+    CFN_REQUIRE(y && res && out && mask && s && q && run_mean && run_var && A && B && mean && rstd, "cfn_bn_tail_fwd: null tensor");
+    CFN_REQUIRE((gamma == nullptr) == (beta == nullptr) && (gammar == nullptr) == (betar == nullptr), "cfn_bn_tail_fwd: gamma/beta mismatch");
+    CFN_REQUIRE(sr == nullptr || (qr && run_meanr && run_varr && Ar && Br && meanr && rstdr), "cfn_bn_tail_fwd: the shortcut BN needs its tensors");
+    CFN_REQUIRE(N > 0 && C > 0 && S > 0 && N % S == 0 && vol > 0, "cfn_bn_tail_fwd: bad sizes (batch %d, %d splits)", N, S);
+    const long NC = (long)N * C;
+    CFN_NC_CHECK(NC);
+    if (!training || cfn_deterministic(-1) > 0) return -1;
+    if (!ew_vec4(vol, y, res, out) || !ew_flat_ok(vol, NC)) return -1;
+    hipStream_t st = (hipStream_t)stream;
+    CfnProfScope prof(CFN_K_ELEMWISE, st, 12.0 * NC * vol);
+    BnTailFwdArgs t = {};
+    t.e.y = y; t.e.res = res; t.e.out = out; t.e.mask = (unsigned*)mask; t.e.vol = vol;
+    t.e.nchunks = (unsigned)cfn_cdiv(vol, 256L * EW_ITEMS * 4);
+    t.m = {s, q, gamma, beta, run_mean, run_var, nbt, A, B, mean, rstd, count, eps, momentum};
+    t.r = {sr, qr, gammar, betar, run_meanr, run_varr, nbtr, Ar, Br, meanr, rstdr, countr, epsr, momentumr};
+    t.N = N; t.C = C; t.S = S; t.hasr = sr != nullptr;
+    hipLaunchKernelGGL(bn_tail_fwd_flat_kernel, dim3((unsigned)(NC * t.e.nchunks)), dim3(256), 0, st, t);
+    return cfn_check_launch("bn_tail_fwd");
+}
+
+extern "C" int cfn_bn_tail_bwd(const float* gout, const float* gout2, const int* mask, const float* y, const float* res, float* g,
+                               double* gA, double* gB, double* gAr, int* tickets, const float* gamma, const double* mean,
+                               const double* rstd, double count, double* gs, double* gq, float* ggamma, float* gbeta,
+                               const float* gammar, const double* meanr, const double* rstdr, double countr, double* gsr, double* gqr,
+                               float* ggammar, float* gbetar, int N, int C, int S, long vol, void* stream) {
+    CFN_REQUIRE(gout && mask && y && g && gA && gB && tickets && mean && rstd && gs && gq, "cfn_bn_tail_bwd: null tensor");
+    CFN_REQUIRE((gamma == nullptr) == (ggamma == nullptr) && (ggamma == nullptr) == (gbeta == nullptr), "cfn_bn_tail_bwd: gamma / ggamma / gbeta mismatch");
+    CFN_REQUIRE(gAr == nullptr || (res && meanr && rstdr && gsr && gqr && (gammar == nullptr) == (ggammar == nullptr) && (ggammar == nullptr) == (gbetar == nullptr)),
+                "cfn_bn_tail_bwd: the shortcut BN needs its tensors");
+    CFN_REQUIRE(N > 0 && C > 0 && S > 0 && N % S == 0 && vol > 0, "cfn_bn_tail_bwd: bad sizes (batch %d, %d splits)", N, S);
+    const long NC = (long)N * C;
+    CFN_NC_CHECK(NC);
+    if (cfn_deterministic(-1) > 0) return -1;
+    if (!(ew_vec4(vol, gout, y, gAr ? res : nullptr, g) && (((uintptr_t)gout2) & 15) == 0) || !ew_flat_ok(vol, NC)) return -1;
+    hipStream_t st = (hipStream_t)stream;
+    CfnProfScope prof(CFN_K_ELEMWISE, st, (12.125 + (gout2 ? 4.0 : 0.0) + (gAr ? 4.0 : 0.0)) * NC * vol);
+    BnTailBwdArgs t = {};
+    t.e.gout = gout; t.e.gout2 = gout2; t.e.maskr = (const unsigned*)mask; t.e.y = y; t.e.res = res; t.e.g = g;
+    t.e.gA = gA; t.e.gB = gB; t.e.gAr = gAr; t.e.vol = vol; t.e.nchunks = (unsigned)cfn_cdiv(vol, 256L * EW_ITEMS * 4);
+    t.m = {gamma, mean, rstd, count, gs, gq, ggamma, gbeta};
+    t.r = {gammar, meanr, rstdr, countr, gsr, gqr, ggammar, gbetar};
+    t.tickets = (unsigned*)tickets; t.N = N; t.C = C; t.S = S;
+    hipLaunchKernelGGL(bn_tail_bwd_flat_kernel, dim3((unsigned)(NC * t.e.nchunks)), dim3(256), 0, st, t);
+    return cfn_check_launch("bn_tail_bwd");
+}
+
 extern "C" int cfn_bn_add_relu_bwd(const float* gout, const float* gout2, const float* out, const float* y, const double* A, const float* res,
                                    const double* Ar, float* gy, float* gres, double* gA, double* gB, double* gAr, long NC,
                                    long vol, void* stream) {
diff --git a/coarse-fine-networks_amd/x3d_fine.py b/coarse-fine-networks_amd/x3d_fine.py
--- a/coarse-fine-networks_amd/x3d_fine.py
+++ b/coarse-fine-networks_amd/x3d_fine.py
@@ -65,6 +65,12 @@
         gamma, beta = (self.weight, self.bias) if self.affine else (None, None)
         return ops.bn_fold(s, q, gamma, beta, bufs, self.training, n, self.num_features, self.num_splits, count, self.eps,
                            self.momentum, se=se, pool_count=count)
+
+    def fold_args(self, s, q, count):
+        bn = self.split_bn if self.training else self.bn
+        gamma, beta = (self.weight, self.bias) if self.affine else (None, None)
+        return (s, q, gamma, beta, (bn.running_mean, bn.running_var, bn.num_batches_tracked), self.num_splits, count, self.eps,
+                self.momentum)
 
     def fold_op(self, s, q, count, n, se=None):
         tr = self.training
@@ -196,7 +202,8 @@
         A2, B2 = self.bn2.fold(s2, q2, _count(y2), n, se=se)
         link = ops.TailLink() if torch.is_grad_enabled() else None
         y3, s3, q3 = ops.pwconv(y2, self.conv3.weight, A2, B2, ACT_SWISH, 1, stats=tr, tail=link, tail_role='y')
-        A3, B3 = self.bn3.fold(s3, q3, _count(y3), n)
+        bn3 = self.bn3.fold_args(s3, q3, _count(y3))
+        C3 = self.bn3.num_features
 
         if self.downsample is not None:
             if not isinstance(self.downsample, nn.Sequential):
@@ -205,13 +212,13 @@
                 res = xm.detach()[:, :, ::s_, ::s_, ::s_]
                 if planes_out > res.shape[1]:
                     res = torch.cat([res, res.new_zeros((res.shape[0], planes_out - res.shape[1]) + tuple(res.shape[2:]))], dim=1)
-                return ops.bn_add_relu(y3, A3, B3, res.contiguous(), split=self.split_out, link=link)
+                return ops.bn_tail(y3, res.contiguous(), tr, n, C3, bn3, split=self.split_out, link=link)
             yd, sd, qd = ops.pwconv(_every(xr, ts), self.downsample[0].weight, xa, xb, xact, self.stride, stats=tr, token=tok, role='short',
                                     tail=link, tail_role='res')
-            Ad, Bd = self.downsample[1].fold(sd, qd, _count(yd), n)
-            return ops.bn_add_relu(y3, A3, B3, yd, Ad, Bd, split=self.split_out, link=link)
+            return ops.bn_tail(y3, yd, tr, n, C3, bn3, short=self.downsample[1].fold_args(sd, qd, _count(yd)), split=self.split_out,
+                               link=link)
         res = x_res.materialize() if isinstance(x_res, Deferred) else x_res
-        return ops.bn_add_relu(y3, A3, B3, res, split=self.split_out, link=link)
+        return ops.bn_tail(y3, res, tr, n, C3, bn3, split=self.split_out, link=link)
 
 
 class ResNet(nn.Module):
diff --git a/include/cfn_hip.h b/include/cfn_hip.h
--- a/include/cfn_hip.h
+++ b/include/cfn_hip.h
@@ -111,6 +111,17 @@
 long cfn_bn_add_relu_mask_words(long NC, long vol);
 int cfn_bn_add_relu_bwd_g(const float* gout, const float* gout2, const float* out, const int* mask, const float* y,
                           const float* res, float* g, double* gA, double* gB, double* gAr, long NC, long vol, void* stream);
+int cfn_bn_tail_fwd(const float* y, const float* res, const double* s, const double* q, const float* gamma, const float* beta,
+                    float* run_mean, float* run_var, long* nbt, double count, double eps, double momentum, const double* sr,
+                    const double* qr, const float* gammar, const float* betar, float* run_meanr, float* run_varr, long* nbtr,
+                    double countr, double epsr, double momentumr, int training, int N, int C, int S, long vol, float* out,
+                    int* mask, double* A, double* B, double* mean, double* rstd, double* Ar, double* Br, double* meanr,
+                    double* rstdr, void* stream);
+int cfn_bn_tail_bwd(const float* gout, const float* gout2, const int* mask, const float* y, const float* res, float* g,
+                    double* gA, double* gB, double* gAr, int* tickets, const float* gamma, const double* mean,
+                    const double* rstd, double count, double* gs, double* gq, float* ggamma, float* gbeta,
+                    const float* gammar, const double* meanr, const double* rstdr, double countr, double* gsr, double* gqr,
+                    float* ggammar, float* gbetar, int N, int C, int S, long vol, void* stream);
 
 int cfn_affine_act_fwd(const float* x, const double* A, const double* B, int act, float* out, long NC, long vol, void* stream);
 int cfn_affine_act_bwd(const float* gout, const float* x, const double* A, const double* B, int act, float* gx, double* gA,
```

Result: no change. 107.2 clips/s, median of 6 (+0.3%).
